# HydraRadio/hydra-pspec

Measured on NVIDIA B200. Metric: baseline-Gibbs-iterations/sec at Nfreq=384, Ntimes=1024, Nfg=32 on 1/8 B200, higher is better.
Workload: dtype f64 (complex128)

## Files before the change

### hydra_pspec_b200/_lib.py

```python
import ctypes as C
import os
from pathlib import Path

import numpy as np

_HERE = Path(__file__).resolve().parent
LIB_PATH = Path(os.environ.get("HP_LIB_PATH", _HERE / "csrc" / "libhydra_pspec_b200.so"))

HP_RNG_INJECTED, HP_RNG_PHILOX = 0, 1
HP_KEEP_CR, HP_KEEP_FG, HP_KEEP_CHISQ = 1, 2, 4
(HP_BUF_PS, HP_BUF_LNPOST, HP_BUF_CR, HP_BUF_FG, HP_BUF_CHISQ, HP_BUF_LAST_CR, HP_BUF_LAST_FG,
 HP_BUF_PS_CUR) = range(8)
HP_NUM_KERNEL_CLASSES = 6


class HPConfig(C.Structure):
    _fields_ = [
        ("device", C.c_int), ("nchains", C.c_int), ("ntimes", C.c_int), ("nfreqs", C.c_int),
        ("nmodes", C.c_int), ("rng_mode", C.c_int), ("cg_compat", C.c_int), ("refresh_omega", C.c_int),
        ("keep", C.c_int), ("max_iters", C.c_int), ("general_basis0", C.c_int), ("profile", C.c_int), ("substreams", C.c_int), ("dense_noise", C.c_int),
        ("force_dense_transforms", C.c_int), ("force_dense_solve", C.c_int), ("time_flags", C.c_int),
        ("ring_iters", C.c_int), ("seed", C.c_uint64), ("stream", C.c_void_p),
    ]


class HPHostSink(C.Structure):
    _fields_ = [("signal_ps", C.c_void_p), ("ln_post", C.c_void_p), ("signal_cr", C.c_void_p),
                ("fg_amps", C.c_void_p), ("chisq", C.c_void_p), ("iters", C.c_int), ("first_iter", C.c_int),
                ("iter_major", C.c_int), ("read_ahead", C.c_int)]


class HydraLibError(RuntimeError):
    pass


_lib = None

_dp = C.POINTER(C.c_double)
_SIGNATURES = {
    "hp_engine_create": (C.c_int, [C.POINTER(HPConfig), C.POINTER(C.c_void_p)]),
    "hp_engine_destroy": (C.c_int, [C.c_void_p]),
    "hp_engine_load_chain": (C.c_int, [C.c_void_p, C.c_int, C.c_void_p, C.c_void_p, C.c_void_p, C.c_void_p,
                                       C.c_void_p, C.c_void_p, C.c_void_p]),
    "hp_engine_load_chain_dense": (C.c_int, [C.c_void_p, C.c_int] + [C.c_void_p] * 9),
    "hp_engine_set_draws": (C.c_int, [C.c_void_p, C.c_int, C.c_void_p, C.c_void_p, C.c_void_p, C.c_int]),
    "hp_engine_run": (C.c_int, [C.c_void_p, C.c_int]),
    "hp_engine_run_to_host": (C.c_int, [C.c_void_p, C.c_int, C.POINTER(HPHostSink)]),
    "hp_engine_gcr": (C.c_int, [C.c_void_p]),
    "hp_engine_sync": (C.c_int, [C.c_void_p]),
    "hp_engine_iterations_done": (C.c_int, [C.c_void_p]),
    "hp_engine_rewind": (C.c_int, [C.c_void_p]),
    "hp_engine_read": (C.c_int, [C.c_void_p, C.c_int, C.c_int, C.c_int, C.c_int, C.c_void_p, C.c_size_t]),
    "hp_engine_read_signal_S": (C.c_int, [C.c_void_p, C.c_int, C.c_void_p]),
    "hp_engine_info": (C.c_int, [C.c_void_p, C.c_void_p]),
    "hp_engine_kernel_ms": (C.c_int, [C.c_void_p, C.c_void_p, C.c_void_p, C.c_int]),
    "hp_engine_set_substreams": (C.c_int, [C.c_void_p, C.c_int]),
    "hp_engine_set_chain_ids": (C.c_int, [C.c_void_p, C.c_void_p]),
    "hp_engine_set_profile": (C.c_int, [C.c_void_p, C.c_int]),
    "hp_engine_launch_count": (C.c_longlong, [C.c_void_p]),
    "hp_engine_pt_form": (C.c_int, [C.c_void_p, C.POINTER(C.c_int), C.POINTER(C.c_int)]),
    "hp_kernel_class_name": (C.c_char_p, [C.c_int]),
    "hp_sample_S": (C.c_int, [C.c_int, C.c_int, C.c_int, C.c_void_p, C.c_void_p, C.c_void_p, C.c_void_p]),
    "hp_fourier_operator": (C.c_int, [C.c_int, C.c_int, C.c_void_p]),
    "hp_eigh_batch": (C.c_int, [C.c_int, C.c_int, C.c_int, C.c_void_p, C.c_void_p, C.c_void_p, C.c_void_p]),
    "hp_test_zgemm": (C.c_int, [C.c_int, C.c_int, C.c_int, C.c_void_p, C.c_int, C.c_int, C.c_void_p, C.c_int,
                                C.c_int, C.c_void_p, C.c_void_p]),
    "hp_test_chol_solve": (C.c_int, [C.c_int, C.c_int, C.c_int, C.c_void_p, C.c_void_p, C.c_void_p, C.c_void_p,
                                     C.c_int, C.c_void_p, C.c_void_p, C.c_void_p]),
    "hp_test_solve2": (C.c_int, [C.c_int, C.c_int, C.c_int, C.c_int, C.c_void_p, C.c_void_p, C.c_void_p, C.c_void_p,
                                 C.c_int, C.c_int, C.c_int, C.c_void_p, C.c_void_p]),
    "hp_test_solve3_schedule": (C.c_int, [C.c_int, C.c_void_p, C.c_void_p, C.POINTER(C.c_int), C.POINTER(C.c_int)]),
    "hp_fp64_peak_tflops": (C.c_double, [C.c_int, C.c_double]),
    "hp_release_cached_memory": (None, []),
    "hp_pinned_alloc": (C.c_void_p, [C.c_size_t]),
    "hp_pinned_free": (None, [C.c_void_p]),
    "hp_last_error": (C.c_char_p, []),
    "hp_version": (C.c_char_p, []),
}
EXPORTED_SYMBOLS = tuple(_SIGNATURES)


def lib():
    global _lib
    if _lib is None:
        if not LIB_PATH.exists():
            raise HydraLibError(
                f"{LIB_PATH} not found: build it with hydra_pspec_b200/csrc/build.sh "
                "(hydra_pspec_b200 has no CPU fallback)")
        L = C.CDLL(os.fspath(LIB_PATH))
        for name, (res, args) in _SIGNATURES.items():
            fn = getattr(L, name)
            fn.restype = res
            fn.argtypes = args
        _lib = L
    return _lib


def check(rc):
    if rc != 0:
        raise HydraLibError(f"hydra_pspec_b200 error {rc}: {lib().hp_last_error().decode()}")


def ptr(a):
    if a is None:
        return None
    assert a.flags["C_CONTIGUOUS"]
    return a.ctypes.data_as(C.c_void_p)


def c128(a):
    return np.ascontiguousarray(a, dtype=np.complex128)


def f64(a):
    return np.ascontiguousarray(a, dtype=np.float64)


def pinned_empty(shape, dtype):
    dtype = np.dtype(dtype)
    nbytes = int(np.prod(shape)) * dtype.itemsize
    p = lib().hp_pinned_alloc(max(nbytes, 1))
    if not p:
        raise HydraLibError("cudaHostAlloc failed")
    buf = (C.c_char * max(nbytes, 1)).from_address(p)
    arr = np.frombuffer(buf, dtype=dtype, count=int(np.prod(shape))).reshape(shape)
    import weakref
    weakref.finalize(buf, lib().hp_pinned_free, p)
    return arr


def bind_to_device_numa(device, verbose=False):
    import os
    import subprocess
    if os.environ.get("HP_NO_NUMA_BIND") == "1":
        return None
    try:
        out = subprocess.run(["nvidia-smi", "--query-gpu=pci.bus_id", "--format=csv,noheader", "-i", str(int(device))],
                             capture_output=True, text=True, timeout=20).stdout.strip().splitlines()[0].strip().lower()
        dom, rest = out.split(":", 1)
        bus = f"{dom[-4:]}:{rest}"
        node = int(open(f"/sys/bus/pci/devices/{bus}/numa_node").read())
        if node < 0:
            return None
        cpus = set()
        for part in open(f"/sys/devices/system/node/node{node}/cpulist").read().strip().split(","):
            lo, _, hi = part.partition("-")
            cpus.update(range(int(lo), int(hi or lo) + 1))
        allowed = os.sched_getaffinity(0)
        use = cpus & allowed
        if verbose:
            import sys
            print(f"[numa] device {device} bus {bus} node {node}: {len(use)} of {len(allowed)} allowed CPUs on that node",
                  file=sys.stderr)
        if not use:
            return None
        os.sched_setaffinity(0, use)
        return node
    except Exception:
        return None
```

### hydra_pspec_b200/csrc/hp_diag.cuh

```cuda
#pragma once
#include "hp_kernels.cuh"
#include "hp_mma.cuh"

namespace hp {

__device__ __forceinline__ bool diag_chol_inverse8(double* Ar, double* Ai, double* Vr, double* Vi) {
    const int lane = threadIdx.x & 31;
    const int r = lane & 7;
    const bool act = lane < 8;
    bool bad = false;
    {
        double ar[8], ai[8];
#pragma unroll
        for (int c = 0; c < 8; ++c) { ar[c] = Ar[r * kLdBlk + c]; ai[c] = Ai[r * kLdBlk + c]; }
#pragma unroll
        for (int c = 0; c < 8; ++c) {
            const double piv = __shfl_sync(0xffffffffu, ar[c], c);
            if (!(piv > 0.0)) bad = true;
            const double inv = rsqrt(piv);
            double lr = ar[c] * inv, li = ai[c] * inv;
            if (r == c) { lr = piv * inv; li = 0.0; }
            if (r < c) { lr = 0.0; li = 0.0; }
            if (act) {
                Ar[r * kLdBlk + c] = lr; Ai[r * kLdBlk + c] = li;
                if (r == c) Vr[c * kLdBlk + c] = inv;
            }
#pragma unroll
            for (int c2 = c + 1; c2 < 8; ++c2) {
                const double yr = __shfl_sync(0xffffffffu, lr, c2), yi = __shfl_sync(0xffffffffu, li, c2);
                ar[c2] -= lr * yr + li * yi;
                ai[c2] -= li * yr - lr * yi;
            }
        }
    }
    __syncwarp();
    {
        double vr[8], vi[8];
#pragma unroll
        for (int q = 0; q < 8; ++q) {
            double sr = 0.0, si = 0.0;
#pragma unroll
            for (int p = 0; p < q; ++p) {
                const double lr = Ar[q * kLdBlk + p], li = Ai[q * kLdBlk + p];
                sr += lr * vr[p] - li * vi[p];
                si += lr * vi[p] + li * vr[p];
            }
            const double dinv = Vr[q * kLdBlk + q];
            vr[q] = r < q ? -sr * dinv : (r == q ? dinv : 0.0);
            vi[q] = r < q ? -si * dinv : 0.0;
        }
        __syncwarp();
        if (act) {
#pragma unroll
            for (int q = 0; q < 8; ++q) { Vr[q * kLdBlk + r] = vr[q]; Vi[q * kLdBlk + r] = vi[q]; }
        }
    }
    __syncwarp();
    return bad;
}

__device__ __forceinline__ bool diag_chol_inverse_block(double* Ar, double* Ai, double* Vr, double* Vi, int tid, int nthreads) {
    const int warp = tid >> 5, lane = tid & 31;
    const int g = lane >> 2, q = lane & 3;
    bool bad = false;
    auto sub = [](double* base, int R, int C) { return base + (8 * R) * kLdBlk + 8 * C; };
    for (int e = tid; e < kLBlkDoubles; e += nthreads) Vr[e] = 0.0;
    if (warp < 6) {
        const int R = warp < 3 ? 0 : (warp < 5 ? 1 : 2), C = warp < 3 ? warp + 1 : (warp < 5 ? warp - 1 : 3);
        for (int e = lane; e < 64; e += 32) { sub(Ar, R, C)[(e >> 3) * kLdBlk + (e & 7)] = 0.0; sub(Ai, R, C)[(e >> 3) * kLdBlk + (e & 7)] = 0.0; }
    }
    __syncthreads();
    for (int kk = 0; kk < 4; ++kk) {
        if (warp == 0) bad |= diag_chol_inverse8(sub(Ar, kk, kk), sub(Ai, kk, kk), sub(Vr, kk, kk), sub(Vi, kk, kk));
        if (kk == 3) break;
        __syncthreads();
        if (warp < 3 - kk) {
            const int R = kk + 1 + warp;
            double P[3][1][1][2], cr[1][1][2], ci[1][1][2];
            warp_zero3m<1, 1>(P);
            warp_zgemm3m<1, 1, false, false, true, true>(P, sub(Ar, R, kk), sub(Ai, R, kk), kLdBlk, sub(Vr, kk, kk), sub(Vi, kk, kk),
                                                         kLdBlk, 8);
            warp_zgemm3m_finish<1, 1, false, true>(P, cr, ci);
            __syncwarp();
            *reinterpret_cast<double2*>(sub(Ar, R, kk) + g * kLdBlk + 2 * q) = make_double2(cr[0][0][0], cr[0][0][1]);
            *reinterpret_cast<double2*>(sub(Ai, R, kk) + g * kLdBlk + 2 * q) = make_double2(ci[0][0][0], ci[0][0][1]);
        }
        __syncthreads();
        const int ntr = (3 - kk) * (4 - kk) / 2;
        if (warp < ntr) {
            int R = kk + 1, C = kk + 1, w = warp;
            while (w > R - (kk + 1)) { w -= R - kk; ++R; }
            C = kk + 1 + w;
            double P[3][1][1][2], cr[1][1][2], ci[1][1][2];
            warp_zero3m<1, 1>(P);
            warp_zgemm3m<1, 1, false, false, true, true>(P, sub(Ar, R, kk), sub(Ai, R, kk), kLdBlk, sub(Ar, C, kk), sub(Ai, C, kk),
                                                         kLdBlk, 8);
            warp_zgemm3m_finish<1, 1, false, true>(P, cr, ci);
            double2* dr = reinterpret_cast<double2*>(sub(Ar, R, C) + g * kLdBlk + 2 * q);
            double2* di = reinterpret_cast<double2*>(sub(Ai, R, C) + g * kLdBlk + 2 * q);
            double2 xr = *dr, xi = *di;
            xr.x -= cr[0][0][0]; xr.y -= cr[0][0][1]; xi.x -= ci[0][0][0]; xi.y -= ci[0][0][1];
            *dr = xr; *di = xi;
        }
        __syncthreads();
    }
    __syncthreads();
    for (int d = 1; d < 4; ++d) {
        if (warp < 4 - d) {
            const int C = warp, R = C + d;
            double P[3][1][1][2], cr[1][1][2], ci[1][1][2];
            warp_zero3m<1, 1>(P);
            warp_zgemm3m<1, 1, false, false, false, false>(P, sub(Ar, R, C), sub(Ai, R, C), kLdBlk, sub(Vr, C, C), sub(Vi, C, C),
                                                           kLdBlk, 8 * d);
            warp_zgemm3m_finish<1, 1, false, false>(P, cr, ci);
            *reinterpret_cast<double2*>(sub(Vr, R, C) + g * kLdBlk + 2 * q) = make_double2(cr[0][0][0], cr[0][0][1]);
            *reinterpret_cast<double2*>(sub(Vi, R, C) + g * kLdBlk + 2 * q) = make_double2(ci[0][0][0], ci[0][0][1]);
            __syncwarp();
            warp_zero3m<1, 1>(P);
            warp_zgemm3m<1, 1, false, false, false, false>(P, sub(Vr, R, R), sub(Vi, R, R), kLdBlk, sub(Vr, R, C), sub(Vi, R, C),
                                                           kLdBlk, 8);
            warp_zgemm3m_finish<1, 1, false, false>(P, cr, ci);
            __syncwarp();
            *reinterpret_cast<double2*>(sub(Vr, R, C) + g * kLdBlk + 2 * q) = make_double2(-cr[0][0][0], -cr[0][0][1]);
            *reinterpret_cast<double2*>(sub(Vi, R, C) + g * kLdBlk + 2 * q) = make_double2(-ci[0][0][0], -ci[0][0][1]);
        }
        __syncthreads();
    }
    return bad;
}

}
```

### hydra_pspec_b200/csrc/hp_engine.cu

```cuda
#include "../../include/hydra_pspec_b200.h"
#include "hp_kernels.cuh"
#include "hp_math.h"

#include <cmath>
#include <cstdio>
#include <cstdlib>
#include <cstring>
#include <mutex>
#include <string>
#include <vector>

namespace {

thread_local std::string g_err;

int fail(int code, const std::string& msg) {
    g_err = msg;
    return code;
}

#define CU_TRY(expr)                                                                              \
    do {                                                                                          \
        cudaError_t _e = (expr);                                                                  \
        if (_e != cudaSuccess)                                                                    \
// ... 78 lines not shown
    double* y = Y + 2 * (sys * (size_t)Tp * Np + (size_t)e);
    y[0] += n0 * 0.70710678118654752440; y[1] += n1 * 0.70710678118654752440;
}
__global__ void k_make_ssc(double* Ssc, const double* X, const double* lam, int n, int Np, int T, int Tp) {
    const size_t sys = blockIdx.y;
    long long e = blockIdx.x * (long long)blockDim.x + threadIdx.x;
    if (e >= (long long)T * n) return;
    const int t = (int)(e / n), k = (int)(e % n);
    const double l = lam[sys * Np + k];
    const double* x = X + 2 * ((sys * (size_t)Tp + t) * Np + k);
    double* o = Ssc + 2 * ((sys * (size_t)Tp + t) * n + k);
    o[0] = l * x[0]; o[1] = l * x[1];
}
__global__ void k_sqrt_vec(double* out, const double* in, int n) {
    int k = blockIdx.x * blockDim.x + threadIdx.x;
    if (k < n) out[k] = sqrt(in[k]);
}

__global__ void k_basis_fourier(double* Bmat, const double* U, int n, int Np) {
    long long e = blockIdx.x * (long long)blockDim.x + threadIdx.x;
    if (e >= (long long)n * n) return;
    int x = (int)(e / n), k = (int)(e % n);
    Bmat[2 * ((size_t)x * Np + k)] = U[2 * ((size_t)k * n + x)];
    Bmat[2 * ((size_t)x * Np + k) + 1] = -U[2 * ((size_t)k * n + x) + 1];
}
__global__ void k_basis_general(double* Bmat, const double* Q, int n, int Np) {
    long long e = blockIdx.x * (long long)blockDim.x + threadIdx.x;
    if (e >= (long long)n * n) return;
    int x = (int)(e / n), k = (int)(e % n);
    Bmat[2 * ((size_t)x * Np + k)] = Q[2 * e];
    Bmat[2 * ((size_t)x * Np + k) + 1] = Q[2 * e + 1];
}
__global__ void k_basis_fg(double* Bmat, double* Ft, const double* F, int n, int m, int Np) {
    long long e = blockIdx.x * (long long)blockDim.x + threadIdx.x;
    if (e >= (long long)n * m) return;
    int x = (int)(e / m), j = (int)(e % m);
    double fr = F[2 * e], fi = F[2 * e + 1];
    Bmat[2 * ((size_t)x * Np + n + j)] = fr;
    Bmat[2 * ((size_t)x * Np + n + j) + 1] = fi;
    if (Ft) { Ft[2 * ((size_t)j * n + x)] = fr; Ft[2 * ((size_t)j * n + x) + 1] = fi; }
}
__global__ void k_noise_vectors(const double* w, const double* ninv, double* ni, double* nu, int n) {
    int x = blockIdx.x * blockDim.x + threadIdx.x;
    if (x >= n) return;
    double v = w[x] * ninv[x];
    ni[x] = v;
    nu[x] = sqrt(v);
}
__global__ void k_init_lam(double* lam, double* ps, const double* lamsq, int n, int N, int Np) {
    int k = blockIdx.x * blockDim.x + threadIdx.x;
    if (k >= Np) return;
    if (k < n) { lam[k] = sqrt(lamsq[k]); if (ps) ps[k] = (double)n * lamsq[k]; }
    else lam[k] = k < N ? 1.0 : 0.0;
}
__global__ void k_scale_vec(double* out, const double* in, double s, int n) {
    int k = blockIdx.x * blockDim.x + threadIdx.x;
    if (k < n) out[k] = in[k] * s;
}

__global__ void k_mask_dense(double* NiD, const double* Ninv, const double* w, int n) {
    long long e = blockIdx.x * (long long)blockDim.x + threadIdx.x;
    if (e >= (long long)n * n) return;
    int x = (int)(e / n), y = (int)(e % n);
    double s = w[x] * w[y];
    NiD[2 * e] = s * Ninv[2 * e];
    NiD[2 * e + 1] = s * Ninv[2 * e + 1];
}
__global__ void k_lower_half(double* NiL, const double* NiD, int n) {
    long long e = blockIdx.x * (long long)blockDim.x + threadIdx.x;
    if (e >= (long long)n * n) return;
    int x = (int)(e / n), y = (int)(e % n);
    double re = 0.0, im = 0.0;
    if (y < x) {
        const long long f = (long long)y * n + x;
        re = 0.5 * (NiD[2 * e] + NiD[2 * f]);
        im = 0.5 * (NiD[2 * e + 1] - NiD[2 * f + 1]);
    } else if (y == x) {
        re = 0.5 * NiD[2 * e];
    }
    NiL[2 * e] = re; NiL[2 * e + 1] = im;
}
__global__ void k_rowdot(const double* A, const double* B, double* out, int T, int Tp, int n, double scale) {
    const int sys = blockIdx.y, t = blockIdx.x;
    const double* a = A + 2 * (((size_t)sys * Tp + t) * n);
    const double* b = B + 2 * (((size_t)sys * Tp + t) * n);
    double acc = 0.0;
    if (t < T)
        for (int x = threadIdx.x; x < n; x += blockDim.x) acc += a[2 * x] * b[2 * x] + a[2 * x + 1] * b[2 * x + 1];
    __shared__ double red[8];
    for (int o = 16; o > 0; o >>= 1) acc += __shfl_down_sync(0xffffffffu, acc, o);
    if ((threadIdx.x & 31) == 0) red[threadIdx.x >> 5] = acc;
    __syncthreads();
    if (threadIdx.x == 0) {
        double s2 = 0.0;
        for (int i = 0; i < (int)(blockDim.x >> 5); ++i) s2 += red[i];
        out[(size_t)sys * Tp + t] = scale * s2;
    }
}

inline unsigned nblocks(long long tot, int bs = 256) { return (unsigned)((tot + bs - 1) / bs); }

struct Basis {
    double* Bmat = nullptr;
    double* Gp = nullptr;
    double* Rfix = nullptr;
    double* wa = nullptr;
    double* Rt = nullptr;
};

enum { CLS_CHOL = 0, CLS_SOLVE = 1, CLS_TRANSFORM = 2, CLS_POST = 3, CLS_SAMPLE = 4, CLS_LOWRANK = 5 };

}

struct hp_engine {
    hp_config cfg;
    int C, T, n, m, N, nblk, Np, Tp, ntiles;
    cudaStream_t st = nullptr;
    cudaStream_t copy_st = nullptr;
    std::vector<cudaStream_t> sub_st;
    cudaEvent_t fork_ev = nullptr;
    int active_subs = 1 << 30;
    std::vector<cudaEvent_t> join_ev;
    bool own_stream = false;
    double *Fop = nullptr, *U = nullptr;
    Basis bF, b0;
    double *lam = nullptr, *ps = nullptr;
    double *wd = nullptr, *w = nullptr, *ninvd = nullptr, *ni = nullptr, *nu = nullptr, *Ft = nullptr, *prior = nullptr;
    double *Lp = nullptr, *Linvp = nullptr, *Wp = nullptr;
    double *wT = nullptr, *Hpt = nullptr, *niT = nullptr, *Bsel = nullptr, *ptScratch = nullptr;
    int* ptSame = nullptr;
    int pt_ctas = 0;
    bool pt_low = false;
    int Tp0 = 0;
    int pt_kcap = 0;
    double* Pm = nullptr;
    uint16_t* ptFidx = nullptr;
    int* ptFcnt = nullptr;
    std::vector<int> pt_kmax;
    std::vector<uint8_t> hpt_built;
    std::vector<uint8_t> pt_loaded;
    int gd_slots = 1;
    std::vector<uint8_t> pending;
    bool big_solve = false;
    bool solve2 = false;
    bool solve3 = false;
    double *Wf1 = nullptr, *Wf2 = nullptr;
    hp::Solve3Sched sched3{};
    int pp_tiles = 0;
    double* Wp1 = nullptr;
    double *Wd = nullptr, *Yb = nullptr;
    double *NiL = nullptr;
    double *NiD = nullptr, *NihD = nullptr, *Td = nullptr, *Rm = nullptr, *Yd = nullptr;
    int* info = nullptr;
    int* chain_ids = nullptr;
    double *X = nullptr, *Ssc = nullptr, *Ppart = nullptr, *Sf = nullptr, *Wm = nullptr, *Tmp = nullptr;
    double *Em = nullptr, *Eu = nullptr, *lnp1 = nullptr;
    double* sdraws = nullptr;
    double *ps_out = nullptr, *lnpost_out = nullptr, *cr_out = nullptr, *fg_out = nullptr, *chisq_out = nullptr;
    double *Gd = nullptr, *stage = nullptr, *vecn = nullptr;
    void* arena = nullptr;
    size_t arena_bytes = 0;
    hp::FftPlan plan{};
    hp::FftPlan plan2f{}, plan2r{};
    bool fft2_ok = false;
    bool fft_ok = false;
    int ntilesE = 0, ktp = 8;
    double *tw = nullptr, *tw2 = nullptr, *Empart = nullptr, *Eupart = nullptr;
    std::vector<uint8_t> flagged;
    std::vector<uint8_t> have_omega;
    bool any_flagged = false;
    int ring = 1;
    std::vector<cudaEvent_t> copy_done;
    std::vector<cudaEvent_t> sub_done;
    int iter = 0;
    int out_pos = 0;
    int ahead = 0;
    std::vector<cudaEvent_t> it_done;
    uint32_t draw_counter = 0;
    const double* last_sf = nullptr;
    long long last_sf_bs = 0;
    long long launches = 0;
    std::vector<cudaEvent_t> ev;
    std::vector<int> ev_cls;
    double ms_acc[HP_NUM_KERNEL_CLASSES] = {0};
    int launch_acc[HP_NUM_KERNEL_CLASSES] = {0};

    void prof_begin(int cls, cudaStream_t s) {
        if (!cfg.profile || ev_cls.size() >= 8192) return;
        cudaEvent_t a, b;
        cudaEventCreate(&a); cudaEventCreate(&b);
        cudaEventRecord(a, s);
        ev.push_back(a); ev.push_back(b); ev_cls.push_back(cls);
    }
    void prof_end(int cls, int nlaunch, cudaStream_t s) {
        launches += nlaunch;
        launch_acc[cls] += nlaunch;
        if (!cfg.profile || ev_cls.empty() || ev_cls.back() != cls) return;
        cudaEventRecord(ev.back(), s);
    }
};

namespace {
constexpr int kMaxDevices = 64;
struct CachedArena { void* p = nullptr; size_t bytes = 0; };
CachedArena g_arena_cache[kMaxDevices];
std::mutex g_arena_mutex;
bool arena_cache_enabled() {
    static int on = -1;
    if (on < 0) { const char* e = getenv("HP_NO_ARENA_CACHE"); on = (e && e[0] == '1') ? 0 : 1; }
    return on == 1;
}
cudaError_t arena_acquire(void** base, size_t* bytes, int device) {
    if (arena_cache_enabled() && device >= 0 && device < kMaxDevices) {
        std::lock_guard<std::mutex> lk(g_arena_mutex);
        CachedArena& c = g_arena_cache[device];
        if (c.p && c.bytes >= *bytes) { *base = c.p; *bytes = c.bytes; c.p = nullptr; c.bytes = 0; return cudaSuccess; }
        if (c.p) { cudaFree(c.p); c.p = nullptr; c.bytes = 0; }
    }
    return cudaMalloc(base, *bytes);
}
void arena_release(void* p, size_t bytes, int device) {
    if (!p) return;
    if (arena_cache_enabled() && device >= 0 && device < kMaxDevices) {
        std::lock_guard<std::mutex> lk(g_arena_mutex);
        CachedArena& c = g_arena_cache[device];
        if (!c.p || c.bytes < bytes) {
            if (c.p) cudaFree(c.p);
            c.p = p; c.bytes = bytes;
            return;
        }
    }
    cudaFree(p);
}

struct ArenaPlan {
    struct Req { void** p; size_t bytes; };
    std::vector<Req> reqs;
    template <typename T>
    void want(T** p, size_t count) { *p = nullptr; if (count) reqs.push_back({reinterpret_cast<void**>(p), count * sizeof(T)}); }
    cudaError_t commit(void** base, size_t* bytes_out, int device, cudaStream_t st) {
        size_t total = 0;
        for (auto& r : reqs) total += (r.bytes + 255) & ~size_t(255);
        if (!total) total = 256;
        *bytes_out = total;
        cudaError_t e = arena_acquire(base, bytes_out, device);
        if (e != cudaSuccess) return e;
        e = cudaMemsetAsync(*base, 0, total, st);
        if (e != cudaSuccess) return e;
        size_t off = 0;
        for (auto& r : reqs) { *r.p = static_cast<char*>(*base) + off; off += (r.bytes + 255) & ~size_t(255); }
        return cudaSuccess;
    }
};

void want_basis(hp_engine* e, ArenaPlan& ap, Basis& b) {
    size_t C = e->C;
    ap.want(&b.Bmat, 2 * C * e->n * e->Np);
    ap.want(&b.Gp, C * hp::tri_blocks(e->nblk) * hp::kBlkDoubles);
    ap.want(&b.Rfix, 2 * C * e->Tp * e->Np);
    if (e->cfg.rng_mode == HP_RNG_INJECTED) ap.want(&b.wa, 2 * C * e->Tp * e->Np);
    if (e->solve2 || e->solve3) ap.want(&b.Rt, 2 * C * e->Tp * e->Np);
}
}

static const char* kAheadMsg = "read-ahead iterations are pending (hp_host_sink.read_ahead): deliver them with hp_engine_run_to_host or "
                               "drop them with hp_engine_rewind first";

extern "C" {

const char* hp_last_error(void) { return g_err.c_str(); }
const char* hp_version(void) { return "hydra_pspec_b200 0.1 (sm_100a)"; }
void hp_release_cached_memory(void) {
    std::lock_guard<std::mutex> lk(g_arena_mutex);
    int cur = 0;
    cudaGetDevice(&cur);
    for (int d = 0; d < kMaxDevices; ++d)
        if (g_arena_cache[d].p) {
            cudaSetDevice(d);
            cudaFree(g_arena_cache[d].p);
            g_arena_cache[d] = CachedArena();
        }
    cudaSetDevice(cur);
}
const char* hp_kernel_class_name(int cls) {
    static const char* names[HP_NUM_KERNEL_CLASSES] = {"chol", "solve", "transform", "post", "sample", "lowrank"};
    return (cls >= 0 && cls < HP_NUM_KERNEL_CLASSES) ? names[cls] : "?";
}

int hp_engine_destroy(hp_engine* e) {
    if (!e) return HP_OK;
    cudaSetDevice(e->cfg.device);
    if (e->st) cudaStreamSynchronize(e->st);
    for (auto& x : e->ev) cudaEventDestroy(x);
    arena_release(e->arena, e->arena_bytes, e->cfg.device);
    if (e->copy_st) cudaStreamDestroy(e->copy_st);
    for (auto x : e->sub_st) cudaStreamDestroy(x);
    if (e->fork_ev) cudaEventDestroy(e->fork_ev);
    for (auto x : e->join_ev) cudaEventDestroy(x);
    for (auto x : e->copy_done) cudaEventDestroy(x);
    for (auto x : e->it_done) cudaEventDestroy(x);
    for (auto x : e->sub_done) cudaEventDestroy(x);
    if (e->own_stream) cudaStreamDestroy(e->st);
    delete e;
    return HP_OK;
}

int hp_engine_create(const hp_config* cfg, hp_engine** out) {
    if (!cfg || !out) return fail(HP_ERR_ARG, "null argument");
    if (cfg->nchains < 1 || cfg->ntimes < 2 || cfg->nfreqs < 2 || cfg->nmodes < 0 || cfg->max_iters < 1)
        return fail(HP_ERR_ARG, "hp_engine_create: bad dimensions");
    int ndev = 0;
    if (cudaGetDeviceCount(&ndev) != cudaSuccess || ndev == 0)
        return fail(HP_ERR_CUDA, "no CUDA device: hydra_pspec_b200 has no CPU fallback");
    CU_TRY(cudaSetDevice(cfg->device));
    hp_engine* e = new hp_engine();
    e->cfg = *cfg;
    e->C = cfg->nchains; e->T = cfg->ntimes; e->n = cfg->nfreqs; e->m = cfg->nmodes;
    e->N = e->n + e->m;
    e->nblk = (e->N + hp::kNB - 1) / hp::kNB;
    e->Np = e->nblk * hp::kNB;
    e->ntiles = (e->T + hp::kTT - 1) / hp::kTT;
    e->Tp = e->ntiles * hp::kTT;
    e->Tp0 = e->Tp;
    int max_smem = 0;
    cudaDeviceGetAttribute(&max_smem, cudaDevAttrMaxSharedMemoryPerBlockOptin, cfg->device);
    e->big_solve = cfg->force_dense_solve || !hp::solve_resident_ok(e->nblk, (size_t)max_smem);
    {
        const char* kv = getenv("HP_SOLVE_KERNEL");
        const int want = kv ? atoi(kv) : 3;
        const bool resident = !e->big_solve && !cfg->time_flags;
        e->solve3 = resident && want >= 3 && hp::solve3_ok(e->nblk, (size_t)max_smem);
        const char* pd = getenv("HP_PT_DIRECT");
        if (cfg->time_flags && !(pd && pd[0] == '1') && !cfg->force_dense_solve && hp::solve3_ok(e->nblk, (size_t)max_smem) &&
            e->n < 65536) {
            e->pt_low = true;
            e->solve3 = true;
            e->Tp0 = e->Tp;
            e->Tp += hp::kTT * ((e->n + hp::kTT - 1) / hp::kTT);
            e->ntiles = e->Tp / hp::kTT;
        }
        e->solve2 = resident && !e->solve3 && want >= 2 && hp::solve2_stages(e->nblk, (size_t)max_smem) >= 2;
        if (e->solve3) hp::solve3_make_schedule(e->nblk, &e->sched3, (e->N + 15) / 16);
    }
    if (cfg->time_flags && (cfg->dense_noise || cfg->cg_compat || cfg->force_dense_transforms || (cfg->general_basis0 && !e->pt_low))) {
        delete e;
        return fail(HP_ERR_ARG, "per-time flags need diagonal noise, the exact solver and an FFT-able Nfreqs (and a delay-diagonal "
                                "S_initial unless Nfreqs + Nmodes <= 448)");
    }
    if (cfg->time_flags && (hp::pt_smem_bytes(e->nblk, e->n) > (size_t)max_smem || !hp::make_fft_plan(e->n, &e->plan) ||
                            hp::postfft_ktp(e->n, e->m, (size_t)max_smem) == 0)) {
        delete e;
        return fail(HP_ERR_SIZE, "per-time flags: Nfreqs too large for the shared-memory working set, or without an FFT plan");
    }
    if (cfg->stream) e->st = (cudaStream_t)cfg->stream;
    else { CU_TRY(cudaStreamCreateWithFlags(&e->st, cudaStreamNonBlocking)); e->own_stream = true; }
    const size_t C = e->C, n = e->n, m = e->m, Np = e->Np, Tp = e->Tp, T = e->T, I = cfg->max_iters;
    e->ring = (cfg->ring_iters > 0 && cfg->ring_iters < cfg->max_iters) ? cfg->ring_iters : cfg->max_iters;
    const size_t R = e->ring;
    e->ktp = hp::postfft_ktp(e->n, e->m, (size_t)max_smem);
    e->fft_ok = hp::make_fft_plan(e->n, &e->plan) && e->ktp > 0 &&
                !cfg->force_dense_transforms;
    {
        const char* v1 = getenv("HP_POST_FFT_V1");
        e->fft2_ok = e->fft_ok && !(v1 && v1[0] == '1') && hp::make_fft2_plan(e->n, &e->plan2f, &e->plan2r) &&
                     hp::postfft2_smem_bytes(e->n, e->m) <= (size_t)max_smem / (e->n >= 512 ? 1 : 2);
        if (e->fft2_ok) e->ktp = 8;
    }
    e->ntilesE = hp::postfft_tiles(e->T, e->ktp > 0 ? e->ktp : 8);
    const bool dense = !e->fft_ok;
    const bool need_ssc = dense || cfg->general_basis0;
    ArenaPlan ap;
    ap.want(&e->Fop, 2 * n * n); ap.want(&e->U, 2 * n * n);
    want_basis(e, ap, e->bF);
    if (cfg->general_basis0) want_basis(e, ap, e->b0);
    ap.want(&e->lam, C * Np); ap.want(&e->ps, C * n);
    ap.want(&e->wd, 2 * C * Tp * n); ap.want(&e->w, C * n); ap.want(&e->ninvd, C * n);
    ap.want(&e->ni, C * n); ap.want(&e->nu, C * n); ap.want(&e->Ft, 2 * C * (m ? m : 1) * n);
    ap.want(&e->prior, C * 2 * n);
    ap.want(&e->Lp, C * hp::tri_blocks(e->nblk) * hp::kLBlkDoubles);
    ap.want(&e->Linvp, C * e->nblk * hp::kLBlkDoubles);
    ap.want(&e->Wp, C * hp::tri_blocks(e->nblk) * hp::kLBlkDoubles);
    if (e->solve2 && cfg->rng_mode == HP_RNG_PHILOX) ap.want(&e->Wp1, C * hp::tri_blocks(e->nblk) * hp::kLBlkDoubles);
    if (e->solve3) { ap.want(&e->Wf1, C * hp::solve3_frag_doubles(e->nblk)); ap.want(&e->Wf2, C * hp::solve3_frag_doubles(e->nblk)); }
    ap.want(&e->info, C);
    ap.want(&e->chain_ids, C);
    ap.want(&e->X, 2 * C * Tp * Np);
    if (need_ssc) ap.want(&e->Ssc, 2 * C * Tp * n);
    e->pp_tiles = (e->solve2 ? 2 : 1) * e->ntiles;
    ap.want(&e->Ppart, C * e->pp_tiles * n); ap.want(&e->Sf, 2 * C * Tp * n);
    if (dense) { ap.want(&e->Wm, 2 * C * Tp * n); ap.want(&e->Tmp, 2 * C * Tp * n); ap.want(&e->Em, C * n); ap.want(&e->Eu, C * n); }
    ap.want(&e->lnp1, C * Tp);
    if (e->big_solve && !cfg->time_flags) { ap.want(&e->Wd, 2 * C * Np * Np); ap.want(&e->Yb, 2 * C * Tp * Np); }
    if (cfg->time_flags) {
        e->pt_ctas = hp::pt_grid(e->C, e->T);
        ap.want(&e->wT, C * Tp * n);
        ap.want(&e->ptSame, C * Tp);
        ap.want(&e->Hpt, 2 * C * Tp * (1 + m) * Np);
        ap.want(&e->niT, Tp * n);
        ap.want(&e->Bsel, 2 * n * (1 + m));
        ap.want(&e->ptScratch, (size_t)e->pt_ctas * hp::pt_scratch_doubles_per_cta(e->nblk));
        if (e->pt_low) {
            ap.want(&e->Pm, 2 * C * n * n);
            ap.want(&e->ptFidx, C * T * hp::kPtLowMaxRank);
            ap.want(&e->ptFcnt, C * T);
        }
    }
    if (cfg->dense_noise) {
        ap.want(&e->NiD, 2 * C * n * n);
        ap.want(&e->NiL, 2 * C * n * n);
        if (cfg->rng_mode == HP_RNG_INJECTED) ap.want(&e->NihD, 2 * C * n * n);
        ap.want(&e->Td, 2 * n * Np); ap.want(&e->Rm, 2 * C * Tp * n); ap.want(&e->Yd, 2 * C * Tp * n);
    }
    if (cfg->rng_mode != HP_RNG_PHILOX) ap.want(&e->sdraws, C * I * n);
    ap.want(&e->ps_out, C * I * n); ap.want(&e->lnpost_out, C * I);
    if (cfg->keep & HP_KEEP_CR) ap.want(&e->cr_out, 2 * C * R * T * n);
    if (cfg->keep & HP_KEEP_FG) ap.want(&e->fg_out, 2 * C * R * T * (m ? m : 1));
    if (cfg->keep & HP_KEEP_CHISQ) ap.want(&e->chisq_out, C * R * T * n);
    e->gd_slots = (int)(C < 16 ? C : 16);
    ap.want(&e->Gd, 2 * (size_t)e->gd_slots * e->N * e->N);
    ap.want(&e->stage, 2 * (T * n > n * n ? T * n : n * n));
    ap.want(&e->vecn, 4 * n);
    ap.want(&e->tw, 2 * n);
    if (e->fft2_ok) ap.want(&e->tw2, 4 * n);
    ap.want(&e->Empart, C * e->ntilesE * n); ap.want(&e->Eupart, C * e->ntilesE * n);
    {
        cudaError_t ce = ap.commit(&e->arena, &e->arena_bytes, cfg->device, e->st);
        if (ce != cudaSuccess) {
            std::string msg = std::string("device allocation failed: ") + cudaGetErrorString(ce);
            hp_engine_destroy(e);
            return fail(HP_ERR_CUDA, msg);
        }
    }
    e->flagged.assign(C, 0);
    e->pt_kmax.assign(C, 0);
    e->hpt_built.assign(C, 0);
    e->pt_loaded.assign(C, 0);
    e->pending.assign(C, 0);
    e->have_omega.assign(C, 0);
    {
        int ns = cfg->substreams > 1 ? (cfg->substreams < (int)C ? cfg->substreams : (int)C) : 1;
        if (ns > 1) {
            for (int i = 0; i < ns; ++i) {
                cudaStream_t x; cudaEvent_t ev;
                cudaStreamCreateWithFlags(&x, cudaStreamNonBlocking); e->sub_st.push_back(x);
                cudaEventCreateWithFlags(&ev, cudaEventDisableTiming); e->join_ev.push_back(ev);
            }
            cudaEventCreateWithFlags(&e->fork_ev, cudaEventDisableTiming);
        }
    }
    {
        std::vector<int> ids(C);
        for (size_t c = 0; c < C; ++c) ids[c] = (int)c;
        cudaMemcpyAsync(e->chain_ids, ids.data(), C * sizeof(int), cudaMemcpyHostToDevice, e->st);
    }
    hp::launch_fourier_operator(e->Fop, e->n, 1.0, e->st);
    hp::launch_fourier_operator(e->U, e->n, 1.0 / std::sqrt((double)e->n), e->st);
    hp::launch_twiddles(e->tw, e->n, e->st);
    if (e->tw2 && !hp::launch_fft2_tables(e->tw2, e->tw, e->n, e->st)) e->tw2 = nullptr;
    if (cudaStreamSynchronize(e->st) != cudaSuccess || cudaGetLastError() != cudaSuccess) {
        hp_engine_destroy(e);
        return fail(HP_ERR_CUDA, "engine initialisation kernels failed");
    }
    *out = e;
    return HP_OK;
}

static int build_hpt(hp_engine* e, int c) {
    const int n = e->n, m = e->m, N = e->N, Np = e->Np, T = e->T;
    const double* Bm = e->bF.Bmat + 2 * (size_t)c * n * Np;
    k_rowscale<<<nblocks((long long)T * n), 256, 0, e->st>>>(e->niT, e->wT + (size_t)c * e->Tp * n, e->ninvd + (size_t)c * n, T, n);
    k_select_cols<<<nblocks((long long)n * (1 + m)), 256, 0, e->st>>>(e->Bsel, Bm, n, m, Np);
    hp::ZgemmArgs h{};
    h.A = Bm; h.sAi = 1; h.sAk = Np; h.bsA = 0; h.conjA = 1;
    h.B = e->Bsel; h.sBk = 1 + m; h.sBj = 1; h.bsB = 0;
    h.C = e->Hpt + 2 * (size_t)c * e->Tp * (1 + m) * Np; h.sCi = 1; h.sCj = Np; h.bsC = (long long)(1 + m) * Np;
    h.dk = e->niT; h.bsD = n;
    h.M = N; h.N = 1 + m; h.K = n; h.accumulate = 0; h.alpha = 1.0; h.batch = T;
    hp::launch_zgemm(h, e->st);
    CU_TRY(cudaGetLastError());
    e->hpt_built[c] = 1;
    return HP_OK;
}

static int build_basis_products(hp_engine* e, Basis& b, int c) {
    const int n = e->n, N = e->N, Np = e->Np, T = e->T;
    double* Bm = b.Bmat + 2 * (size_t)c * n * Np;
    const bool dn = e->cfg.dense_noise != 0;
    const double* NiD = dn ? e->NiD + 2 * (size_t)c * n * n : nullptr;
    hp::ZgemmArgs g{};
    g.A = Bm; g.sAi = 1; g.sAk = Np; g.bsA = 0; g.conjA = 1;
    g.C = e->Gd; g.sCi = N; g.sCj = 1; g.bsC = 0;
    g.M = N; g.N = N; g.K = n; g.accumulate = 0; g.alpha = 1.0; g.batch = 1;
    if (dn) {
        hp::ZgemmArgs t1{};
        t1.A = NiD; t1.sAi = n; t1.sAk = 1;
        t1.B = Bm; t1.sBk = Np; t1.sBj = 1;
        t1.C = e->Td; t1.sCi = Np; t1.sCj = 1;
        t1.M = n; t1.N = N; t1.K = n; t1.alpha = 1.0; t1.batch = 1;
        hp::launch_zgemm(t1, e->st);
        g.B = e->Td; g.sBk = Np; g.sBj = 1;
    } else {
        g.B = Bm; g.sBk = Np; g.sBj = 1; g.bsB = 0; g.conjB = 0;
        g.dk = e->ni + (size_t)c * n; g.bsD = 0;
    }
    hp::launch_zgemm(g, e->st);
    hp::launch_pack_lower(e->Gd, N, 0, b.Gp + (size_t)c * hp::tri_blocks(e->nblk) * hp::kBlkDoubles, N, e->nblk, 1, e->st);
    hp::ZgemmArgs r{};
    r.B = Bm; r.sBk = Np; r.sBj = 1; r.conjB = 1;
    r.C = b.Rfix + 2 * (size_t)c * e->Tp * Np; r.sCi = Np; r.sCj = 1;
    r.M = T; r.N = N; r.K = n; r.accumulate = 0; r.alpha = 1.0; r.batch = 1;
    if (dn) {
        hp::ZgemmArgs y{};
        y.A = e->wd + 2 * (size_t)c * e->Tp * n; y.sAi = n; y.sAk = 1;
        y.B = NiD; y.sBk = 1; y.sBj = n;
        y.C = e->Yd + 2 * (size_t)c * e->Tp * n; y.sCi = n; y.sCj = 1;
        y.M = T; y.N = n; y.K = n; y.alpha = 1.0; y.batch = 1;
        hp::launch_zgemm(y, e->st);
        r.A = e->Yd + 2 * (size_t)c * e->Tp * n; r.sAi = n; r.sAk = 1;
    } else {
        r.A = e->wd + 2 * (size_t)c * e->Tp * n; r.sAi = n; r.sAk = 1; r.conjA = 0;
        r.dk = e->cfg.time_flags ? e->ninvd + (size_t)c * n : e->ni + (size_t)c * n;
    }
    hp::launch_zgemm(r, e->st);
    if (e->ptFidx) hp::launch_pt_arows(b.Rfix + 2 * (size_t)c * e->Tp * Np, Bm, e->ni + (size_t)c * n, n, Np, e->Tp0, e->st);
    if (b.Rt && e->cfg.rng_mode == HP_RNG_PHILOX)
        hp::launch_rhs_tile(b.Rt + 2 * (size_t)c * e->Tp * Np, b.Rfix + 2 * (size_t)c * e->Tp * Np, nullptr, nullptr, e->nblk, e->n, e->N,
                            e->ptFidx ? e->Tp : e->T, e->Tp, e->ntiles, 1, e->st);
    if (e->cfg.time_flags && &b == &e->bF) {
        e->hpt_built[c] = 0;
        if (!e->pt_low) { const int rc = build_hpt(e, c); if (rc != HP_OK) return rc; }
    }
    CU_TRY(cudaGetLastError());
    return HP_OK;
}

static int build_basis_products_batch(hp_engine* e, Basis& b, int c0, int nc) {
    const int n = e->n, N = e->N, Np = e->Np, T = e->T;
    const size_t tri = hp::tri_blocks(e->nblk);
    for (int cc0 = c0; cc0 < c0 + nc; cc0 += e->gd_slots) {
        const int ncc = (c0 + nc - cc0) < e->gd_slots ? (c0 + nc - cc0) : e->gd_slots;
        double* Bm = b.Bmat + 2 * (size_t)cc0 * n * Np;
        hp::ZgemmArgs g{};
        g.A = Bm; g.sAi = 1; g.sAk = Np; g.bsA = (long long)n * Np; g.conjA = 1;
        g.B = Bm; g.sBk = Np; g.sBj = 1; g.bsB = (long long)n * Np;
        g.dk = e->ni + (size_t)cc0 * n; g.bsD = n;
        g.C = e->Gd; g.sCi = N; g.sCj = 1; g.bsC = (long long)N * N;
        g.M = N; g.N = N; g.K = n; g.accumulate = 0; g.alpha = 1.0; g.batch = ncc;
        hp::launch_zgemm(g, e->st);
        hp::launch_pack_lower(e->Gd, N, (long long)N * N, b.Gp + (size_t)cc0 * tri * hp::kBlkDoubles, N, e->nblk, ncc, e->st);
        hp::ZgemmArgs r{};
        r.A = e->wd + 2 * (size_t)cc0 * e->Tp * n; r.sAi = n; r.sAk = 1; r.bsA = (long long)e->Tp * n;
        r.dk = e->ni + (size_t)cc0 * n; r.bsD = n;
        r.B = Bm; r.sBk = Np; r.sBj = 1; r.bsB = (long long)n * Np; r.conjB = 1;
        r.C = b.Rfix + 2 * (size_t)cc0 * e->Tp * Np; r.sCi = Np; r.sCj = 1; r.bsC = (long long)e->Tp * Np;
        r.M = T; r.N = N; r.K = n; r.accumulate = 0; r.alpha = 1.0; r.batch = ncc;
        hp::launch_zgemm(r, e->st);
        if (b.Rt && e->cfg.rng_mode == HP_RNG_PHILOX)
            hp::launch_rhs_tile(b.Rt + 2 * (size_t)cc0 * e->Tp * Np, b.Rfix + 2 * (size_t)cc0 * e->Tp * Np, nullptr, nullptr, e->nblk,
                                e->n, e->N, e->T, e->Tp, e->ntiles, ncc, e->st);
    }
    CU_TRY(cudaGetLastError());
    return HP_OK;
}

static int flush_pending(hp_engine* e) {
    const int C = e->C;
    if (e->cfg.time_flags && !e->pt_low)
        for (int c = 0; c < C; ++c)
            if (e->pt_loaded[c] && !e->hpt_built[c]) { const int rc = build_hpt(e, c); if (rc != HP_OK) return rc; }
    for (int c = 0; c < C;) {
        if (!e->pending[c]) { ++c; continue; }
        int c1 = c;
        while (c1 < C && e->pending[c1]) ++c1;
        int rc;
        if ((rc = build_basis_products_batch(e, e->bF, c, c1 - c)) != HP_OK) return rc;
        if (e->cfg.general_basis0 && (rc = build_basis_products_batch(e, e->b0, c, c1 - c)) != HP_OK) return rc;
        for (int k = c; k < c1; ++k) e->pending[k] = 0;
// ... 105 lines not shown
    }
    CU_TRY(cudaMemcpyAsync(e->vecn, lam0sq, n * sizeof(double), cudaMemcpyHostToDevice, st));
    k_init_lam<<<nblocks(Np), 256, 0, st>>>(e->lam + (size_t)c * Np, e->ps + (size_t)c * n, e->vecn, n, N, Np);
    CU_TRY(cudaStreamSynchronize(st));
    CU_TRY(cudaGetLastError());
    e->iter = 0;
    e->out_pos = 0;
    e->draw_counter = 0;
    return HP_OK;
}

int hp_engine_load_chain(hp_engine* e, int c, const double* vis, const uint8_t* flags, const double* fgmodes,
                         const double* ninv_diag, const double* basis0, const double* lam0sq, const double* ps_prior) {
    return load_chain_impl(e, c, vis, flags, fgmodes, ninv_diag, nullptr, nullptr, basis0, lam0sq, ps_prior);
}

int hp_engine_load_chain_dense(hp_engine* e, int c, const double* vis, const uint8_t* flags, const double* fgmodes,
                               const double* ninv_diag, const double* ninv_dense, const double* nih_dense,
                               const double* basis0, const double* lam0sq, const double* ps_prior) {
    if (!ninv_dense) return fail(HP_ERR_ARG, "hp_engine_load_chain_dense: ninv_dense is NULL");
    return load_chain_impl(e, c, vis, flags, fgmodes, ninv_diag, ninv_dense, nih_dense, basis0, lam0sq, ps_prior);
}

int hp_engine_set_draws(hp_engine* e, int c, const double* omega_a, const double* omega_b, const double* s_draws,
                        int n_draw_iters) {
    if (!e) return fail(HP_ERR_ARG, "null engine");
    if (e->cfg.rng_mode != HP_RNG_INJECTED) return fail(HP_ERR_ARG, "hp_engine_set_draws: engine is not in injected-draw mode");
    if (e->ahead > 0) return fail(HP_ERR_ARG, kAheadMsg);
    if (c < 0 || c >= e->C) return fail(HP_ERR_ARG, "chain index out of range");
    if ((omega_a == nullptr) != (omega_b == nullptr)) return fail(HP_ERR_ARG, "omega_a and omega_b must both be given or both NULL");
    if (n_draw_iters > e->cfg.max_iters) return fail(HP_ERR_ARG, "more draw iterations than max_iters");
    CU_TRY(cudaSetDevice(e->cfg.device));
    { int rcf = flush_pending(e); if (rcf != HP_OK) return rcf; }
    const int n = e->n, Np = e->Np, T = e->T, Tp = e->Tp;
    cudaStream_t st = e->st;
    if (s_draws && n_draw_iters > 0)
        CU_TRY(cudaMemcpyAsync(e->sdraws + (size_t)c * e->cfg.max_iters * n, s_draws, (size_t)n_draw_iters * n * sizeof(double),
                               cudaMemcpyHostToDevice, st));
    if (omega_a) {
        for (int which = 0; which < (e->cfg.general_basis0 ? 2 : 1); ++which) {
            Basis& b = which ? e->b0 : e->bF;
            double* Bm = b.Bmat + 2 * (size_t)c * n * Np;
            CU_TRY(cudaMemcpyAsync(e->stage, omega_b, 2 * (size_t)T * n * sizeof(double), cudaMemcpyHostToDevice, st));
            hp::ZgemmArgs r{};
            r.A = e->stage; r.sAi = n; r.sAk = 1;
            r.B = Bm; r.sBk = Np; r.sBj = 1; r.conjB = 1;
            r.C = b.Rfix + 2 * (size_t)c * Tp * Np; r.sCi = Np; r.sCj = 1;
            if (e->cfg.dense_noise) {
                hp::ZgemmArgs y{};
                y.A = e->stage; y.sAi = n; y.sAk = 1;
                y.B = e->NihD + 2 * (size_t)c * n * n; y.sBk = 1; y.sBj = n;
                y.C = e->Yd + 2 * (size_t)c * Tp * n; y.sCi = n; y.sCj = 1;
                y.M = T; y.N = n; y.K = n; y.alpha = 1.0; y.batch = 1;
                hp::launch_zgemm(y, st);
                r.A = e->Yd + 2 * (size_t)c * Tp * n;
            } else if (e->cfg.time_flags) {
                k_mask_elem<<<nblocks((long long)T * n), 256, 0, st>>>(e->stage, e->wT + (size_t)c * Tp * n, (long long)T * n);
                k_sqrt_vec<<<nblocks(n), 256, 0, st>>>(e->vecn, e->ninvd + (size_t)c * n, n);
                r.dk = e->vecn;
            } else {
                r.dk = e->nu + (size_t)c * n;
            }
            r.M = T; r.N = e->N; r.K = n; r.accumulate = 1; r.alpha = 1.0; r.batch = 1;
            hp::launch_zgemm(r, st);
            CU_TRY(cudaStreamSynchronize(st));
            CU_TRY(cudaMemcpyAsync(e->stage, omega_a, 2 * (size_t)T * n * sizeof(double), cudaMemcpyHostToDevice, st));
            hp::ZgemmArgs a{};
            a.A = e->stage; a.sAi = n; a.sAk = 1;
            a.B = Bm; a.sBk = Np; a.sBj = 1; a.conjB = 1;
            a.C = b.wa + 2 * (size_t)c * Tp * Np; a.sCi = Np; a.sCj = 1;
            a.M = T; a.N = n; a.K = n; a.accumulate = 0; a.alpha = 1.0; a.batch = 1;
            hp::launch_zgemm(a, st);
            CU_TRY(cudaStreamSynchronize(st));
        }
        e->have_omega[c] = 1;
    }
    CU_TRY(cudaStreamSynchronize(st));
    CU_TRY(cudaGetLastError());
    return HP_OK;
}

static cudaError_t copy_rows_d2h(void* dst, size_t dpitch, const void* src, size_t spitch, size_t width, size_t rows,
                                 cudaStream_t st) {
    if (rows == 0 || width == 0) return cudaSuccess;
    if (dpitch < (size_t)0x7fffffff && spitch < (size_t)0x7fffffff)
        return cudaMemcpy2DAsync(dst, dpitch, src, spitch, width, rows, cudaMemcpyDeviceToHost, st);
    cudaError_t e = cudaSuccess;
    for (size_t r = 0; r < rows && e == cudaSuccess; ++r)
        e = cudaMemcpyAsync((char*)dst + r * dpitch, (const char*)src + r * spitch, width, cudaMemcpyDeviceToHost, st);
    return e;
}

struct IterOut {
    double* sf; long long sf_bs;
    double* fg; long long fg_bs;
    double* chisq; long long chisq_bs;
};

struct Sub { int c0, nc; cudaStream_t st; };
#define OFFS(ptr, per_chain) ((ptr) ? (ptr) + (size_t)sb.c0 * (size_t)(per_chain) : nullptr)

static void enqueue_dense_lnp1(hp_engine* e, const Sub& sb) {
    const size_t n = e->n, Tp = e->Tp;
    e->prof_begin(CLS_TRANSFORM, sb.st);
    hp::ZgemmArgs y{};
    y.A = OFFS(e->Rm, 2 * Tp * n); y.sAi = e->n; y.sAk = 1; y.bsA = (long long)e->Tp * e->n;
    y.B = OFFS(e->NiL, 2 * n * n); y.sBk = e->n; y.sBj = 1; y.conjB = 1; y.bsB = (long long)e->n * e->n;
    y.C = OFFS(e->Yd, 2 * Tp * n); y.sCi = e->n; y.sCj = 1; y.bsC = (long long)e->Tp * e->n;
    y.M = e->T; y.N = e->n; y.K = e->n; y.alpha = 1.0; y.batch = sb.nc;
    y.tri = 2;
    hp::launch_zgemm(y, sb.st);
    k_rowdot<<<dim3(e->Tp, sb.nc), 128, 0, sb.st>>>(OFFS(e->Rm, 2 * Tp * n), OFFS(e->Yd, 2 * Tp * n), OFFS(e->lnp1, Tp), e->T,
                                                   e->Tp, e->n, 2.0);
    e->prof_end(CLS_TRANSFORM, 2, sb.st);
}

static void enqueue_gcr(hp_engine* e, Basis& b, const IterOut& o, const Sub& sb, uint32_t draw_iter) {
    const bool philox = e->cfg.rng_mode == HP_RNG_PHILOX;
    const bool general = &b == &e->b0;
    const size_t n = e->n, m = e->m, Np = e->Np, Tp = e->Tp;
    const size_t tri = hp::tri_blocks(e->nblk);
    const bool fused_inverse = e->fft_ok && !general;
    const bool pt = e->cfg.time_flags != 0;
    bool any_omega = false;
    for (auto h : e->have_omega) any_omega |= (h != 0);
    const bool pt_low = pt && e->pt_low;
    if (pt && !pt_low) {
        const int nsub = e->C > 0 ? (e->C + sb.nc - 1) / sb.nc : 1;
        int grid = e->pt_ctas / (nsub > 0 ? nsub : 1);
        if (grid < 1) grid = 1;
        const int slot0 = (int)(((long long)sb.c0 * e->pt_ctas) / e->C);
        if (slot0 + grid > e->pt_ctas) grid = e->pt_ctas - slot0;
        e->prof_begin(CLS_SOLVE, sb.st);
        cudaMemsetAsync(e->info + sb.c0, 0, sizeof(int) * sb.nc, sb.st);
        hp::PtArgs pa{};
        pa.H = OFFS(e->Hpt, 2 * Tp * (1 + m) * Np); pa.lam = OFFS(e->lam, Np); pa.Rfix = OFFS(b.Rfix, 2 * Tp * Np);
        pa.wa = (!philox && any_omega) ? OFFS(b.wa, 2 * Tp * Np) : nullptr;
        pa.X = OFFS(e->X, 2 * Tp * Np);
        pa.same_prev = OFFS(e->ptSame, Tp);
        pa.scratch = e->ptScratch + (size_t)slot0 * hp::pt_scratch_doubles_per_cta(e->nblk);
        pa.info = e->info + sb.c0;
        pa.nblk = e->nblk; pa.n = e->n; pa.m = e->m; pa.N = e->N; pa.T = e->T; pa.Tp = e->Tp; pa.nsys = sb.nc;
        pa.philox_wa = philox ? 1 : 0;
        pa.key0 = (uint32_t)e->cfg.seed; pa.key1 = (uint32_t)(e->cfg.seed >> 32); pa.iter = draw_iter;
        pa.chain_ids = OFFS(e->chain_ids, 1); pa.chain0 = sb.c0;
        hp::launch_pt_cholsolve(pa, grid, sb.st);
        hp::launch_colsumsq(OFFS(e->X, 2 * Tp * Np), OFFS(e->Ppart, (size_t)e->pp_tiles * n), e->T, e->Tp, e->n, sb.nc, sb.st, e->Np);
        e->prof_end(CLS_SOLVE, 2, sb.st);
    } else {
    e->prof_begin(CLS_CHOL, sb.st);
    hp::CholArgs ca{};
    ca.Gp = OFFS(b.Gp, tri * hp::kBlkDoubles); ca.lam = OFFS(e->lam, Np); ca.Lp = OFFS(e->Lp, tri * hp::kLBlkDoubles);
    ca.Linvp = OFFS(e->Linvp, (size_t)e->nblk * hp::kLBlkDoubles); ca.info = e->info + sb.c0;
    ca.nblk = e->nblk; ca.n = e->n; ca.N = e->N; ca.nsys = sb.nc;
    const hp::TrinvExtra ex{OFFS(e->Wp1, tri * hp::kLBlkDoubles), OFFS(e->Wf1, hp::solve3_frag_doubles(e->nblk)),
                            OFFS(e->Wf2, hp::solve3_frag_doubles(e->nblk)), philox ? OFFS(e->lam, Np) : nullptr};
    const int nchol = hp::launch_chol_trinv(ca, OFFS(e->Wp, tri * hp::kLBlkDoubles), ex, sb.st);
    e->prof_end(CLS_CHOL, nchol, sb.st);

    if (e->big_solve) {
        e->prof_begin(CLS_SOLVE, sb.st);
        const long long NN = (long long)e->Np * e->Np, TN = (long long)e->Tp * e->Np;
        double* Wd = OFFS(e->Wd, 2 * Np * Np);
        double* Yb = OFFS(e->Yb, 2 * Tp * Np);
        double* X = OFFS(e->X, 2 * Tp * Np);
        k_unpack_lower<<<dim3(nblocks(NN), sb.nc), 256, 0, sb.st>>>(OFFS(e->Wp, tri * hp::kLBlkDoubles), Wd, e->nblk,
                                                                   tri * hp::kLBlkDoubles);
        k_build_rhs<<<dim3(nblocks(TN), sb.nc), 256, 0, sb.st>>>(X, OFFS(b.Rfix, 2 * Tp * Np),
                                                                (!philox && any_omega) ? OFFS(b.wa, 2 * Tp * Np) : nullptr,
                                                                OFFS(e->lam, Np), e->n, e->Np, e->T, e->Tp);
        hp::ZgemmArgs y{};
        y.A = X; y.sAi = e->Np; y.sAk = 1; y.bsA = TN;
        y.B = Wd; y.sBk = 1; y.sBj = e->Np; y.bsB = NN;
        y.C = Yb; y.sCi = e->Np; y.sCj = 1; y.bsC = TN;
        y.M = e->T; y.N = e->Np; y.K = e->Np; y.alpha = 1.0; y.batch = sb.nc;
        y.tri = 1;
        hp::launch_zgemm(y, sb.st);
        int nl = 4;
        if (philox) {
            k_add_noise<<<dim3(nblocks((long long)e->T * e->Np), sb.nc), 256, 0, sb.st>>>(
                Yb, e->N, e->Np, e->T, e->Tp, (uint32_t)e->cfg.seed, (uint32_t)(e->cfg.seed >> 32), draw_iter, OFFS(e->chain_ids, 1));
            ++nl;
        }
        hp::ZgemmArgs x{};
        x.A = Yb; x.sAi = e->Np; x.sAk = 1; x.bsA = TN;
        x.B = Wd; x.sBk = e->Np; x.sBj = 1; x.bsB = NN; x.conjB = 1;
        x.C = X; x.sCi = e->Np; x.sCj = 1; x.bsC = TN;
        x.M = e->T; x.N = e->Np; x.K = e->Np; x.alpha = 1.0; x.batch = sb.nc;
        x.tri = 2;
        hp::launch_zgemm(x, sb.st);
        if (e->cfg.cg_compat) {
            hp::launch_cg_scale(X, OFFS(b.Rfix, 2 * Tp * Np), (!philox && any_omega) ? OFFS(b.wa, 2 * Tp * Np) : nullptr, OFFS(e->lam, Np),
                                e->n, e->N, e->Np, e->T, e->Tp, sb.nc, sb.st);
            ++nl;
        }
        hp::launch_colsumsq(X, OFFS(e->Ppart, (size_t)e->pp_tiles * n), e->T, e->Tp, e->n, sb.nc, sb.st, e->Np);
        ++nl;
        if (!fused_inverse) {
            k_make_ssc<<<dim3(nblocks((long long)e->T * e->n), sb.nc), 256, 0, sb.st>>>(OFFS(e->Ssc, 2 * Tp * n), X, OFFS(e->lam, Np),
                                                                                       e->n, e->Np, e->T, e->Tp);
            ++nl;
        }
        e->prof_end(CLS_SOLVE, nl, sb.st);
    } else if (e->solve3) {
        e->prof_begin(CLS_SOLVE, sb.st);
        int nl = 1;
        const double* wa_sb = (!philox && any_omega) ? OFFS(b.wa, 2 * Tp * Np) : nullptr;
        if (!philox) {
            hp::launch_rhs_tile(OFFS(b.Rt, 2 * Tp * Np), OFFS(b.Rfix, 2 * Tp * Np), wa_sb, OFFS(e->lam, Np), e->nblk, e->n, e->N,
                                pt_low ? e->Tp : e->T, e->Tp, e->ntiles, sb.nc, sb.st);
            ++nl;
        }
        hp::Solve3Args sa{};
        sa.Wf1 = OFFS(e->Wf1, hp::solve3_frag_doubles(e->nblk)); sa.Wf2 = OFFS(e->Wf2, hp::solve3_frag_doubles(e->nblk));
        sa.Rt = OFFS(b.Rt, 2 * Tp * Np);
        sa.X = OFFS(e->X, 2 * Tp * Np);
        sa.Ppart = OFFS(e->Ppart, (size_t)e->pp_tiles * n);
        sa.nblk = e->nblk; sa.n = e->n; sa.N = e->N; sa.Tp = e->Tp; sa.ntiles = e->ntiles; sa.nsys = sb.nc; sa.T = e->T;
        sa.philox = philox ? 1 : 0;
        sa.key0 = (uint32_t)e->cfg.seed; sa.key1 = (uint32_t)(e->cfg.seed >> 32); sa.iter = draw_iter;
        sa.chain_ids = OFFS(e->chain_ids, 1); sa.chain0 = sb.c0;
        sa.sched = e->sched3; sa.nstrip = (e->N + 15) / 16;
        hp::launch_solve3(sa, sb.st);
        if (pt_low) {
            e->prof_end(CLS_SOLVE, nl, sb.st);
            nl = 0;
            e->prof_begin(CLS_LOWRANK, sb.st);
            hp::ZgemmArgs pz{};
            pz.A = OFFS(b.Rfix, 2 * Tp * Np) + 2 * (size_t)e->Tp0 * Np; pz.sAi = e->Np; pz.sAk = 1; pz.bsA = (long long)e->Tp * e->Np;
            pz.conjA = 1; pz.dk = OFFS(e->lam, Np); pz.bsD = e->Np;
            pz.B = sa.X + 2 * (size_t)e->Tp0 * Np; pz.sBk = 1; pz.sBj = e->Np; pz.bsB = (long long)e->Tp * e->Np;
            pz.C = OFFS(e->Pm, 2 * n * n); pz.sCi = e->n; pz.sCj = 1; pz.bsC = (long long)e->n * e->n;
            pz.M = e->n; pz.N = e->n; pz.K = e->N; pz.alpha = 1.0; pz.batch = sb.nc;
            pz.lower_out = 1;
            hp::launch_zgemm(pz, sb.st);
            hp::PtLowArgs la{};
            la.Rfix = OFFS(b.Rfix, 2 * Tp * Np); la.wa = wa_sb; la.lam = OFFS(e->lam, Np); la.X = sa.X; la.Pm = OFFS(e->Pm, 2 * n * n);
            la.fidx = e->ptFidx + (size_t)sb.c0 * e->T * hp::kPtLowMaxRank; la.fcnt = e->ptFcnt + (size_t)sb.c0 * e->T;
            la.info = e->info + sb.c0;
            la.n = e->n; la.N = e->N; la.Np = e->Np; la.T = e->T; la.Tp = e->Tp; la.Tp0 = e->Tp0; la.nsys = sb.nc; la.nblk = e->nblk;
            la.kcap = e->pt_kcap; la.philox = philox ? 1 : 0;
            la.key0 = (uint32_t)e->cfg.seed; la.key1 = (uint32_t)(e->cfg.seed >> 32); la.iter = draw_iter;
            la.chain_ids = OFFS(e->chain_ids, 1); la.chain0 = sb.c0;
            hp::launch_pt_lowrank(la, sb.st);
            hp::launch_colsumsq(sa.X, OFFS(e->Ppart, (size_t)e->pp_tiles * n), e->T, e->Tp, e->n, sb.nc, sb.st, e->Np);
            e->prof_end(CLS_LOWRANK, 3, sb.st);
            e->prof_begin(CLS_SOLVE, sb.st);
        }
        if (e->cfg.cg_compat) {
            hp::launch_cg_scale(sa.X, OFFS(b.Rfix, 2 * Tp * Np), wa_sb, OFFS(e->lam, Np), e->n, e->N, e->Np, e->T, e->Tp, sb.nc, sb.st);
            hp::launch_colsumsq(sa.X, OFFS(e->Ppart, (size_t)e->pp_tiles * n), e->T, e->Tp, e->n, sb.nc, sb.st, e->Np);
            nl += 2;
        }
        if (!fused_inverse) {
            k_make_ssc<<<dim3(nblocks((long long)e->T * e->n), sb.nc), 256, 0, sb.st>>>(OFFS(e->Ssc, 2 * Tp * n), sa.X, OFFS(e->lam, Np),
                                                                                       e->n, e->Np, e->T, e->Tp);
            ++nl;
        }
        e->prof_end(CLS_SOLVE, nl, sb.st);
    } else if (e->solve2) {
        e->prof_begin(CLS_SOLVE, sb.st);
        int nl = 1;
        const double* wa_sb = (!philox && any_omega) ? OFFS(b.wa, 2 * Tp * Np) : nullptr;
        if (!philox) {
            hp::launch_rhs_tile(OFFS(b.Rt, 2 * Tp * Np), OFFS(b.Rfix, 2 * Tp * Np), wa_sb, OFFS(e->lam, Np), e->nblk, e->n, e->N, e->T,
                                e->Tp, e->ntiles, sb.nc, sb.st);
            ++nl;
        }
        hp::Solve2Args sa{};
        sa.W1 = philox ? OFFS(e->Wp1, tri * hp::kLBlkDoubles) : OFFS(e->Wp, tri * hp::kLBlkDoubles);
        sa.W2 = OFFS(e->Wp, tri * hp::kLBlkDoubles);
        sa.Rt = OFFS(b.Rt, 2 * Tp * Np);
        sa.X = OFFS(e->X, 2 * Tp * Np);
        sa.Ppart = OFFS(e->Ppart, (size_t)e->pp_tiles * n);
        sa.nblk = e->nblk; sa.n = e->n; sa.N = e->N; sa.Tp = e->Tp; sa.ntiles = e->ntiles; sa.nsys = sb.nc; sa.T = e->T;
        sa.philox = philox ? 1 : 0;
        sa.key0 = (uint32_t)e->cfg.seed; sa.key1 = (uint32_t)(e->cfg.seed >> 32); sa.iter = draw_iter;
        sa.chain_ids = OFFS(e->chain_ids, 1); sa.chain0 = sb.c0;
        hp::launch_solve2(sa, sb.st);
        if (e->cfg.cg_compat) {
            hp::launch_cg_scale(sa.X, OFFS(b.Rfix, 2 * Tp * Np), wa_sb, OFFS(e->lam, Np), e->n, e->N, e->Np, e->T, e->Tp, sb.nc, sb.st);
            hp::launch_colsumsq(sa.X, OFFS(e->Ppart, (size_t)e->pp_tiles * n), e->T, e->Tp, e->n, sb.nc, sb.st, e->Np);
            nl += 2;
        }
        if (!fused_inverse) {
            k_make_ssc<<<dim3(nblocks((long long)e->T * e->n), sb.nc), 256, 0, sb.st>>>(OFFS(e->Ssc, 2 * Tp * n), sa.X, OFFS(e->lam, Np),
                                                                                       e->n, e->Np, e->T, e->Tp);
            ++nl;
        }
        e->prof_end(CLS_SOLVE, nl, sb.st);
    } else {
    e->prof_begin(CLS_SOLVE, sb.st);
    hp::SolveArgs sa{};
    sa.Wp = OFFS(e->Wp, tri * hp::kLBlkDoubles); sa.lam = OFFS(e->lam, Np);
    sa.Rfix = OFFS(b.Rfix, 2 * Tp * Np);
    sa.wa = (!philox && any_omega) ? OFFS(b.wa, 2 * Tp * Np) : nullptr;
    sa.X = OFFS(e->X, 2 * Tp * Np); sa.Ssc = fused_inverse ? nullptr : OFFS(e->Ssc, 2 * Tp * n);
    sa.Ppart = OFFS(e->Ppart, (size_t)e->pp_tiles * n);
    sa.nblk = e->nblk; sa.n = e->n; sa.N = e->N; sa.Tp = e->Tp; sa.ntiles = e->ntiles; sa.nsys = sb.nc; sa.T = e->T;
    sa.philox_wa = philox ? 1 : 0;
    sa.cg_compat = e->cfg.cg_compat;
    sa.key0 = (uint32_t)e->cfg.seed; sa.key1 = (uint32_t)(e->cfg.seed >> 32); sa.iter = draw_iter;
    sa.chain_ids = OFFS(e->chain_ids, 1); sa.chain0 = sb.c0;
    hp::launch_solve(sa, sb.st);
    e->prof_end(CLS_SOLVE, 1, sb.st);
    }
// ... 246 lines not shown
                                     e->copy_st);
        }
        cudaEventRecord(e->copy_done[slot], e->copy_st);
    }
    if (big && cerr == cudaSuccess && sink->read_ahead > 0) {
        int want = sink->read_ahead < (int)R - 1 ? sink->read_ahead : (int)R - 1;
        while (e->ahead < want && e->out_pos + e->ahead < e->cfg.max_iters) {
            compute_next((size_t)(e->out_pos + e->ahead));
            ++e->ahead;
        }
    }
    join_subs(e, subs);
    if (cerr != cudaSuccess) return fail(HP_ERR_CUDA, std::string("hp_engine_run_to_host: ") + cudaGetErrorString(cerr));
    {
        cudaEvent_t ev;
        CU_TRY(cudaEventCreateWithFlags(&ev, cudaEventDisableTiming));
        CU_TRY(cudaEventRecord(ev, e->st));
        CU_TRY(cudaStreamWaitEvent(e->copy_st, ev, 0));
        cudaEventDestroy(ev);
    }
    if (niter > 0) {
        const size_t h0 = (size_t)(first - sink->first_iter);
        if (sink->signal_ps)
            CU_TRY(copy_rows_d2h(sink->signal_ps + h0 * n, HI * n * 8, e->ps_out + first * n, I * n * 8, (size_t)niter * n * 8, C,
                                 e->copy_st));
        if (sink->ln_post)
            CU_TRY(copy_rows_d2h(sink->ln_post + h0, HI * 8, e->lnpost_out + first, I * 8, (size_t)niter * 8, C, e->copy_st));
    }
    CU_TRY(cudaStreamSynchronize(e->copy_st));
    CU_TRY(cudaStreamSynchronize(e->st));
    CU_TRY(cudaGetLastError());
    return HP_OK;
}

int hp_engine_set_chain_ids(hp_engine* e, const int* ids) {
    if (!e || !ids) return fail(HP_ERR_ARG, "null argument");
    CU_TRY(cudaSetDevice(e->cfg.device));
    CU_TRY(cudaMemcpyAsync(e->chain_ids, ids, (size_t)e->C * sizeof(int), cudaMemcpyHostToDevice, e->st));
    CU_TRY(cudaStreamSynchronize(e->st));
    return HP_OK;
}

int hp_engine_set_substreams(hp_engine* e, int n) {
    if (!e) return fail(HP_ERR_ARG, "null engine");
    if (e->ahead > 0) return fail(HP_ERR_ARG, kAheadMsg);
    e->active_subs = n < 1 ? 1 : n;
    return HP_OK;
}

int hp_engine_set_profile(hp_engine* e, int on) {
    if (!e) return fail(HP_ERR_ARG, "null engine");
    e->cfg.profile = on ? 1 : 0;
    return HP_OK;
}

int hp_engine_sync(hp_engine* e) {
    if (!e) return fail(HP_ERR_ARG, "null engine");
    CU_TRY(cudaSetDevice(e->cfg.device));
    CU_TRY(cudaStreamSynchronize(e->st));
    CU_TRY(cudaGetLastError());
    return HP_OK;
}
int hp_engine_iterations_done(const hp_engine* e) { return e ? e->iter : -1; }
int hp_engine_rewind(hp_engine* e) {
    if (!e) return fail(HP_ERR_ARG, "null engine");
    e->out_pos = 0;
    e->ahead = 0;
    return HP_OK;
}
long long hp_engine_launch_count(const hp_engine* e) { return e ? e->launches : -1; }
int hp_engine_pt_form(const hp_engine* e, int* low_rank, int* max_rank) {
    if (!e) return fail(HP_ERR_ARG, "null engine");
    if (low_rank) *low_rank = (e->cfg.time_flags && e->pt_low) ? 1 : 0;
    if (max_rank) *max_rank = e->pt_kcap;
    return HP_OK;
}

int hp_engine_read(hp_engine* e, int c, int buffer, int iter0, int niter, void* dst, size_t dst_bytes) {
    if (!e || !dst) return fail(HP_ERR_ARG, "null argument");
    if (c < 0 || c >= e->C) return fail(HP_ERR_ARG, "chain index out of range");
    CU_TRY(cudaSetDevice(e->cfg.device));
    CU_TRY(cudaStreamSynchronize(e->st));
    const size_t n = e->n, m = e->m, T = e->T, Tp = e->Tp, Np = e->Np, I = e->cfg.max_iters;
    const bool per_iter = buffer <= HP_BUF_CHISQ;
    if (per_iter && (iter0 < 0 || niter < 0 || (size_t)(iter0 + niter) > I)) return fail(HP_ERR_ARG, "iteration range out of bounds");
    const double* src = nullptr;
    size_t bytes = 0;
    switch (buffer) {
        case HP_BUF_PS: src = e->ps_out + ((size_t)c * I + iter0) * n; bytes = (size_t)niter * n * 8; break;
        case HP_BUF_LNPOST: src = e->lnpost_out + (size_t)c * I + iter0; bytes = (size_t)niter * 8; break;
        case HP_BUF_CR:
        case HP_BUF_FG:
        case HP_BUF_CHISQ: {
            const double* base = buffer == HP_BUF_CR ? e->cr_out : (buffer == HP_BUF_FG ? e->fg_out : e->chisq_out);
            if (!base) return fail(HP_ERR_ARG, "this output was not kept (cfg.keep)");
            const size_t R = e->ring;
            const size_t per = buffer == HP_BUF_CR ? 2 * T * n : (buffer == HP_BUF_FG ? 2 * T * m : T * n);
            bytes = (size_t)niter * per * 8;
            if (dst_bytes < bytes) return fail(HP_ERR_ARG, "destination too small");
            if (niter > 0 && (size_t)iter0 + R < (size_t)(e->out_pos + e->ahead))
                return fail(HP_ERR_ARG, "iteration no longer in the device ring (cfg.ring_iters): stream it with hp_engine_run_to_host");
            for (int k = 0; k < niter; ++k) {
                const size_t slot = (size_t)(iter0 + k) % R;
                if (per) CU_TRY(cudaMemcpy((char*)dst + (size_t)k * per * 8, base + (slot * (size_t)e->C + (size_t)c) * per, per * 8, cudaMemcpyDeviceToHost));
            }
            return HP_OK;
        }
        case HP_BUF_LAST_CR:
            if (e->ahead > 0) return fail(HP_ERR_ARG, kAheadMsg);
            if (!e->last_sf) return fail(HP_ERR_ARG, "no GCR solve has run yet");
            src = e->last_sf + 2 * (size_t)c * e->last_sf_bs; bytes = T * n * 16; break;
        case HP_BUF_PS_CUR:
            if (e->ahead > 0) return fail(HP_ERR_ARG, kAheadMsg);
            src = e->ps + (size_t)c * n; bytes = n * 8; break;
        case HP_BUF_LAST_FG: {
            if (e->ahead > 0) return fail(HP_ERR_ARG, kAheadMsg);
            bytes = T * m * 16;
            if (dst_bytes < bytes) return fail(HP_ERR_ARG, "destination too small");
            if (m == 0) return HP_OK;
            CU_TRY(cudaMemcpy2D(dst, m * 16, e->X + 2 * ((size_t)c * Tp * Np + n), Np * 16, m * 16, T, cudaMemcpyDeviceToHost));
            return HP_OK;
        }
        default: return fail(HP_ERR_ARG, "unknown buffer id");
    }
    if (dst_bytes < bytes) return fail(HP_ERR_ARG, "destination too small");
    if (bytes) CU_TRY(cudaMemcpy(dst, src, bytes, cudaMemcpyDeviceToHost));
    return HP_OK;
}

int hp_engine_read_signal_S(hp_engine* e, int c, double* dst) {
    if (!e || !dst) return fail(HP_ERR_ARG, "null argument");
    if (c < 0 || c >= e->C) return fail(HP_ERR_ARG, "chain index out of range");
    if (e->ahead > 0) return fail(HP_ERR_ARG, kAheadMsg);
    CU_TRY(cudaSetDevice(e->cfg.device));
    const int n = e->n;
    k_scale_vec<<<nblocks(n), 256, 0, e->st>>>(e->vecn + n, e->ps + (size_t)c * n, 1.0 / ((double)n * n), n);
    hp::ZgemmArgs g{};
    g.A = e->Fop; g.sAi = 1; g.sAk = n; g.conjA = 1;
    g.B = e->Fop; g.sBk = n; g.sBj = 1;
    g.C = e->stage; g.sCi = n; g.sCj = 1;
    g.dk = e->vecn + n;
    g.M = n; g.N = n; g.K = n; g.alpha = 1.0; g.batch = 1;
    hp::launch_zgemm(g, e->st);
    CU_TRY(cudaStreamSynchronize(e->st));
    CU_TRY(cudaMemcpy(dst, e->stage, 2 * (size_t)n * n * sizeof(double), cudaMemcpyDeviceToHost));
    return HP_OK;
}

int hp_engine_info(hp_engine* e, int* info_host) {
    if (!e || !info_host) return fail(HP_ERR_ARG, "null argument");
    CU_TRY(cudaSetDevice(e->cfg.device));
    CU_TRY(cudaStreamSynchronize(e->st));
    CU_TRY(cudaMemcpy(info_host, e->info, e->C * sizeof(int), cudaMemcpyDeviceToHost));
    return HP_OK;
}

int hp_engine_kernel_ms(hp_engine* e, double* ms, int* launches, int reset) {
    if (!e) return fail(HP_ERR_ARG, "null engine");
    CU_TRY(cudaSetDevice(e->cfg.device));
    CU_TRY(cudaStreamSynchronize(e->st));
    for (size_t i = 0; i < e->ev_cls.size(); ++i) {
        float t = 0.f;
        if (cudaEventElapsedTime(&t, e->ev[2 * i], e->ev[2 * i + 1]) == cudaSuccess) e->ms_acc[e->ev_cls[i]] += t;
        cudaEventDestroy(e->ev[2 * i]); cudaEventDestroy(e->ev[2 * i + 1]);
    }
    e->ev.clear(); e->ev_cls.clear();
    for (int i = 0; i < HP_NUM_KERNEL_CLASSES; ++i) {
        if (ms) ms[i] = e->ms_acc[i];
        if (launches) launches[i] = e->launch_acc[i];
        if (reset) { e->ms_acc[i] = 0; e->launch_acc[i] = 0; }
    }
    return HP_OK;
}

int hp_sample_S(int device, int T, int n, const double* s, const double* prior, const double* draws, double* out) {
    if (!s || !draws || !out || T < 2 || n < 1) return fail(HP_ERR_ARG, "hp_sample_S: bad argument");
    int ndev = 0;
    if (cudaGetDeviceCount(&ndev) != cudaSuccess || ndev == 0) return fail(HP_ERR_CUDA, "no CUDA device: hydra_pspec_b200 has no CPU fallback");
    CU_TRY(cudaSetDevice(device));
    double *U, *S, *Sk, *Eu, *pr, *dr, *ps, *lam, *lnp1, *psout, *lnp;
    CU_TRY(dalloc(&U, 2 * (size_t)n * n)); CU_TRY(dalloc(&S, 2 * (size_t)T * n)); CU_TRY(dalloc(&Sk, 2 * (size_t)T * n));
    CU_TRY(dalloc(&Eu, n)); CU_TRY(dalloc(&pr, 2 * (size_t)n)); CU_TRY(dalloc(&dr, n)); CU_TRY(dalloc(&ps, n));
    CU_TRY(dalloc(&lam, n + 64)); CU_TRY(dalloc(&lnp1, T)); CU_TRY(dalloc(&psout, n)); CU_TRY(dalloc(&lnp, 1));
    hp::launch_fourier_operator(U, n, 1.0 / std::sqrt((double)n), 0);
    CU_TRY(cudaMemcpy(S, s, 2 * (size_t)T * n * sizeof(double), cudaMemcpyHostToDevice));
    if (prior) CU_TRY(cudaMemcpy(pr, prior, 2 * (size_t)n * sizeof(double), cudaMemcpyHostToDevice));
    CU_TRY(cudaMemcpy(dr, draws, n * sizeof(double), cudaMemcpyHostToDevice));
    hp::ZgemmArgs t{};
    t.A = S; t.sAi = n; t.sAk = 1;
    t.B = U; t.sBk = 1; t.sBj = n;
    t.C = Sk; t.sCi = n; t.sCj = 1;
    t.M = T; t.N = n; t.K = n; t.alpha = 1.0; t.batch = 1;
    hp::launch_zgemm(t, 0);
    hp::launch_colsumsq(Sk, Eu, T, T, n, 1, 0);
    hp::SampleArgs sp{};
    sp.Eu = Eu; sp.lnp1 = lnp1; sp.prior = pr; sp.draws = dr; sp.draws_bs = n;
    sp.ps = ps; sp.lam = lam; sp.ps_out = psout; sp.ps_bs = n; sp.lnpost_out = lnp; sp.lnpost_bs = 1;
    sp.n = n; sp.Np = n; sp.T = T; sp.Tp = T; sp.ntiles = 0; sp.nsys = 1; sp.beta_mode = 1; sp.philox = 0;
    hp::launch_sample(sp, 0);
    CU_TRY(cudaDeviceSynchronize());
    CU_TRY(cudaGetLastError());
    CU_TRY(cudaMemcpy(out, psout, n * sizeof(double), cudaMemcpyDeviceToHost));
    double* ptrs[] = {U, S, Sk, Eu, pr, dr, ps, lam, lnp1, psout, lnp};
    for (double* p : ptrs) cudaFree(p);
    return HP_OK;
}

int hp_fourier_operator(int device, int n, double* out) {
    if (!out || n < 1) return fail(HP_ERR_ARG, "hp_fourier_operator: bad argument");
    int ndev = 0;
    if (cudaGetDeviceCount(&ndev) != cudaSuccess || ndev == 0) return fail(HP_ERR_CUDA, "no CUDA device: hydra_pspec_b200 has no CPU fallback");
    CU_TRY(cudaSetDevice(device));
    double* d;
    CU_TRY(dalloc(&d, 2 * (size_t)n * n));
    hp::launch_fourier_operator(d, n, 1.0, 0);
    CU_TRY(cudaDeviceSynchronize());
    CU_TRY(cudaMemcpy(out, d, 2 * (size_t)n * n * sizeof(double), cudaMemcpyDeviceToHost));
    cudaFree(d);
    return HP_OK;
}

}
```

### hydra_pspec_b200/csrc/hp_kernels.cu

```cuda
#include "hp_kernels.cuh"
#include "hp_math.h"
#include "hp_mma.cuh"
#include "hp_diag.cuh"

namespace hp {

__device__ __forceinline__ void cp_async16(void* smem_dst, const void* gmem_src) {
    unsigned s = (unsigned)__cvta_generic_to_shared(smem_dst);
    asm volatile("cp.async.cg.shared.global [%0], [%1], 16;" ::"r"(s), "l"(gmem_src) : "memory");
}
__device__ __forceinline__ void cp_async_commit() { asm volatile("cp.async.commit_group;" ::: "memory"); }
template <int N>
__device__ __forceinline__ void cp_async_wait() { asm volatile("cp.async.wait_group %0;" ::"n"(N) : "memory"); }

__global__ void k_fourier_operator(double* out, int n, double scale) {
    long long e = blockIdx.x * (long long)blockDim.x + threadIdx.x;
    if (e >= (long long)n * n) return;
    int k = (int)(e / n), x = (int)(e % n);
    long long a = (long long)(k - n / 2) * (long long)(x - n / 2);
    long long r = a % n;
    if (r < 0) r += n;
    double s, c;
    sincospi(-2.0 * (double)r / (double)n, &s, &c);
    out[2 * e] = c * scale;
    out[2 * e + 1] = s * scale;
}
void launch_fourier_operator(double* out, int n, double scale, cudaStream_t st) {
    long long tot = (long long)n * n;
    k_fourier_operator<<<(unsigned)((tot + 255) / 256), 256, 0, st>>>(out, n, scale);
}

__global__ void k_pack_lower(const double* dense, long long ld, long long bs, double* packed, int N, int nblk) {
    const int bi = blockIdx.y, bj = blockIdx.x;
    if (bj > bi) return;
    const double* D = dense + 2 * bs * blockIdx.z;
    double* P = packed + ((size_t)blockIdx.z * tri_blocks(nblk) + blk_index(bi, bj)) * kBlkDoubles;
    for (int e = threadIdx.x; e < 1024; e += blockDim.x) {
        int r = e >> 5, c = e & 31;
        int gi = bi * 32 + r, gj = bj * 32 + c;
        double xr = 0.0, xi = 0.0;
        if (gi < N && gj < N) { xr = D[2 * (gi * ld + gj)]; xi = D[2 * (gi * ld + gj) + 1]; }
        P[e] = xr; P[1024 + e] = xi;
    }
}
void launch_pack_lower(const double* dense, long long ld, long long bs, double* packed, int N, int nblk, int batch,
                       cudaStream_t st) {
    k_pack_lower<<<dim3(nblk, nblk, batch), 256, 0, st>>>(dense, ld, bs, packed, N, nblk);
}

constexpr int kCT = 512;

__device__ __forceinline__ void load_block_async_ct(double* s, const double* g) {
    for (int c = threadIdx.x; c < kLBlkDoubles / 2; c += kCT) cp_async16(s + 2 * c, g + 2 * c);
}

struct CholWSmem {
    double A[2][kLBlkDoubles];
    double B[2][kLBlkDoubles];
    double V[kLBlkDoubles];
};
__device__ __forceinline__ void store_frag1(double* Wf1, int R, int C, double re, double im) {
    const int s = R >> 4, t = C >> 2;
    double* d = Wf1 + ((size_t)(2 * s * (s + 1) + t) * 128 + 64 * ((R >> 3) & 1) + (4 * (R & 7) + (C & 3)) * 2);
    *reinterpret_cast<double2*>(d) = make_double2(re, im);
}
__device__ __forceinline__ void store_frag2(double* Wf2, int nblk, int R, int C, double re, double im) {
    const int s = C >> 4, t = R >> 2;
    double* d = Wf2 + ((size_t)(8 * nblk * s - 2 * s * (s - 1) + t - 4 * s) * 128 + 64 * ((C >> 3) & 1) + (4 * (C & 7) + (R & 3)) * 2);
    *reinterpret_cast<double2*>(d) = make_double2(re, im);
}

__global__ void __launch_bounds__(kCT, 2) k_chol_w(CholArgs a, TrinvExtra ex, double* Wp_all, int k, int first) {
    extern __shared__ __align__(16) unsigned char smem_raw[];
    CholWSmem& s = *reinterpret_cast<CholWSmem*>(smem_raw);
    const int sys = blockIdx.x;
    const int nblk = a.nblk, Np = nblk * 32;
    const int npanel = nblk - k - 1;
    const bool wrow = !first && (int)blockIdx.y >= npanel;
    const int jp = wrow ? (int)blockIdx.y - npanel : 0;
    const double* Gp = a.Gp + (size_t)sys * tri_blocks(nblk) * kBlkDoubles;
    double* Lp = a.Lp + (size_t)sys * tri_blocks(nblk) * kLBlkDoubles;
    double* Linvp = a.Linvp + (size_t)sys * nblk * kLBlkDoubles;
    double* Wp = Wp_all + (size_t)sys * tri_blocks(nblk) * kLBlkDoubles;
    const double* lam = a.lam + (size_t)sys * Np;
    double* Wp1 = (ex.Wp1 && ex.lam) ? ex.Wp1 + (size_t)sys * tri_blocks(nblk) * kLBlkDoubles : nullptr;
    const size_t wf = (size_t)4 * nblk * (2 * nblk + 1) * 128;
    double* Wf1 = ex.Wf1 ? ex.Wf1 + (size_t)sys * wf : nullptr;
    double* Wf2 = ex.Wf2 ? ex.Wf2 + (size_t)sys * wf : nullptr;
    const int tid = threadIdx.x, warp = tid >> 5, lane = tid & 31;
    const int g = lane >> 2, q = lane & 3;
    const int ti = warp >> 2, tj = warp & 3;
    double* Ar = s.A[0];
    double* Ai = s.A[0] + kLPlane;
    double* Vr = s.V;
    double* Vi = s.V + kLPlane;

    if (wrow) {
        const double* lamj = ex.lam ? ex.lam + (size_t)sys * Np + 32 * jp : nullptr;
        double P3m[3][1][1][2], cr[1][1][2], ci[1][1][2];
        warp_zero3m<1, 1>(P3m);
        load_block_async_ct(s.V, Linvp + (size_t)k * kLBlkDoubles);
        load_block_async_ct(s.A[0], Lp + blk_index(k, jp) * kLBlkDoubles);
        load_block_async_ct(s.B[0], Wp + blk_index(jp, jp) * kLBlkDoubles);
        cp_async_commit();
        for (int j = jp; j < k; ++j) {
            const int st = (j - jp) & 1;
            cp_async_wait<0>();
            __syncthreads();
            if (j + 1 < k) {
                load_block_async_ct(s.A[st ^ 1], Lp + blk_index(k, j + 1) * kLBlkDoubles);
                load_block_async_ct(s.B[st ^ 1], Wp + blk_index(j + 1, jp) * kLBlkDoubles);
                cp_async_commit();
            }
            warp_zgemm3m<1, 1, false, false, false, false>(P3m, s.A[st] + 8 * ti * kLdBlk, s.A[st] + kLPlane + 8 * ti * kLdBlk, kLdBlk,
                                                           s.B[st] + 8 * tj, s.B[st] + kLPlane + 8 * tj, kLdBlk, 32);
        }
        __syncthreads();
        warp_zgemm3m_finish<1, 1, false, false>(P3m, cr, ci);
#pragma unroll
        for (int e = 0; e < 2; ++e) {
            const int r = 8 * ti + g, c = 8 * tj + 2 * q + e;
            s.A[0][r * kLdBlk + c] = -cr[0][0][e];
            s.A[0][kLPlane + r * kLdBlk + c] = -ci[0][0][e];
        }
        __syncthreads();
        double dr[1][1][2], di[1][1][2], Q3m[3][1][1][2];
        warp_zero3m<1, 1>(Q3m);
        warp_zgemm3m<1, 1, false, false, false, false>(Q3m, s.V + 8 * ti * kLdBlk, s.V + kLPlane + 8 * ti * kLdBlk, kLdBlk,
                                                       s.A[0] + 8 * tj, s.A[0] + kLPlane + 8 * tj, kLdBlk, 8 * (ti + 1));
        warp_zgemm3m_finish<1, 1, false, false>(Q3m, dr, di);
        double* Wb = Wp + blk_index(k, jp) * kLBlkDoubles;
        const int r = 8 * ti + g, c = 8 * tj + 2 * q;
        *reinterpret_cast<double2*>(Wb + r * kLdBlk + c) = make_double2(dr[0][0][0], dr[0][0][1]);
        *reinterpret_cast<double2*>(Wb + kLPlane + r * kLdBlk + c) = make_double2(di[0][0][0], di[0][0][1]);
        if (Wp1) {
            double* Wb1 = Wp1 + blk_index(k, jp) * kLBlkDoubles;
            const double l0 = lamj[c], l1 = lamj[c + 1];
            *reinterpret_cast<double2*>(Wb1 + r * kLdBlk + c) = make_double2(l0 * dr[0][0][0], l1 * dr[0][0][1]);
            *reinterpret_cast<double2*>(Wb1 + kLPlane + r * kLdBlk + c) = make_double2(l0 * di[0][0][0], l1 * di[0][0][1]);
        }
        if (Wf1 || Wf2) {
#pragma unroll
            for (int e = 0; e < 2; ++e) {
                const int R = 32 * k + r, C = 32 * jp + c + e;
                if (Wf1) {
                    const double l = lamj ? lamj[c + e] : 1.0;
                    store_frag1(Wf1, R, C, l * dr[0][0][e], l * di[0][0][e]);
                }
                if (Wf2) store_frag2(Wf2, nblk, R, C, dr[0][0][e], di[0][0][e]);
            }
        }
        return;
    }

    auto chol_block = [&](int i, int kc, bool diag) {
        double cr[1][1][2], ci[1][1][2], P3m[3][1][1][2];
        warp_zero<1, 1>(cr, ci);
        warp_zero3m<1, 1>(P3m);
        double mr_[2], mi_[2];
        {
            const double* Gb = Gp + blk_index(i, kc) * kBlkDoubles;
#pragma unroll
            for (int e = 0; e < 2; ++e) {
                const int r = 8 * ti + g, c = 8 * tj + 2 * q + e;
                const int gi = 32 * i + r, gj = 32 * kc + c;
                const double sc = lam[gi] * lam[gj];
                mr_[e] = sc * Gb[r * 32 + c];
                mi_[e] = sc * Gb[1024 + r * 32 + c];
                if (gi == gj && (gi < a.n || gi >= a.N)) mr_[e] += 1.0;
            }
        }
        if (!diag) load_block_async_ct(s.V, Linvp + (size_t)kc * kLBlkDoubles);
        if (kc > 0) {
            load_block_async_ct(s.A[0], Lp + blk_index(i, 0) * kLBlkDoubles);
            if (!diag) load_block_async_ct(s.B[0], Lp + blk_index(kc, 0) * kLBlkDoubles);
        }
        cp_async_commit();
        for (int j = 0; j < kc; ++j) {
            const int st = j & 1;
            cp_async_wait<0>();
            __syncthreads();
            if (j + 1 < kc) {
                load_block_async_ct(s.A[st ^ 1], Lp + blk_index(i, j + 1) * kLBlkDoubles);
                if (!diag) load_block_async_ct(s.B[st ^ 1], Lp + blk_index(kc, j + 1) * kLBlkDoubles);
                cp_async_commit();
            }
            const double* ar = s.A[st];
            const double* br = diag ? s.A[st] : s.B[st];
            warp_zgemm3m<1, 1, false, false, true, true>(P3m, ar + 8 * ti * kLdBlk, ar + kLPlane + 8 * ti * kLdBlk, kLdBlk,
                                                         br + 8 * tj * kLdBlk, br + kLPlane + 8 * tj * kLdBlk, kLdBlk, 32);
        }
        cp_async_wait<0>();
        __syncthreads();
        warp_zgemm3m_finish<1, 1, false, true>(P3m, cr, ci);
#pragma unroll
        for (int e = 0; e < 2; ++e) {
            int r = 8 * ti + g, c = 8 * tj + 2 * q + e;
            Ar[r * kLdBlk + c] = mr_[e] - cr[0][0][e];
            Ai[r * kLdBlk + c] = mi_[e] - ci[0][0][e];
        }
        __syncthreads();
        if (diag) {
            const bool bad = diag_chol_inverse_block(Ar, Ai, Vr, Vi, tid, kCT);
            __syncthreads();
            double* Lb = Lp + blk_index(kc, kc) * kLBlkDoubles;
            double* Vb = Linvp + (size_t)kc * kLBlkDoubles;
            double* Wb = Wp + blk_index(kc, kc) * kLBlkDoubles;
            const double* lamk = ex.lam ? ex.lam + (size_t)sys * Np + 32 * kc : nullptr;
            for (int e = tid; e < kLBlkDoubles; e += kCT) {
                const double v = s.V[e];
                Lb[e] = s.A[0][e];
                Vb[e] = v;
                Wb[e] = v;
                if (Wp1) {
                    const int c = (e % kLPlane) % kLdBlk;
                    Wp1[blk_index(kc, kc) * kLBlkDoubles + e] = c < 32 ? v * lamk[c] : 0.0;
                }
            }
            if (Wf1 || Wf2) {
                for (int e = tid; e < 1024; e += kCT) {
                    const int r = e >> 5, c = e & 31;
                    const double re = Vr[r * kLdBlk + c], im = Vi[r * kLdBlk + c];
                    if (Wf1 && c < 16 * ((r >> 4) + 1)) {
                        const double l = lamk ? lamk[c] : 1.0;
                        store_frag1(Wf1, 32 * kc + r, 32 * kc + c, l * re, l * im);
                    }
                    if (Wf2 && r >= 16 * (c >> 4)) store_frag2(Wf2, nblk, 32 * kc + r, 32 * kc + c, re, im);
                }
            }
            if (bad && tid == 0 && a.info) atomicMax(a.info + sys, kc + 1);
        } else {
            double dr[1][1][2], di[1][1][2], Q3m[3][1][1][2];
            warp_zero3m<1, 1>(Q3m);
            warp_zgemm3m<1, 1, false, false, true, true>(Q3m, Ar + 8 * ti * kLdBlk, Ai + 8 * ti * kLdBlk, kLdBlk, Vr + 8 * tj * kLdBlk,
                                                         Vi + 8 * tj * kLdBlk, kLdBlk, 32);
            warp_zgemm3m_finish<1, 1, false, true>(Q3m, dr, di);
            double* Lb = Lp + blk_index(i, kc) * kLBlkDoubles;
            int r = 8 * ti + g, c = 8 * tj + 2 * q;
            *reinterpret_cast<double2*>(Lb + r * kLdBlk + c) = make_double2(dr[0][0][0], dr[0][0][1]);
            *reinterpret_cast<double2*>(Lb + kLPlane + r * kLdBlk + c) = make_double2(di[0][0][0], di[0][0][1]);
        }
    };
    if (first) { chol_block(0, 0, true); return; }
    chol_block(k + 1 + (int)blockIdx.y, k, false);
    if (blockIdx.y == 0) {
        __syncthreads();
        chol_block(k + 1, k + 1, true);
    }
}

int launch_chol_trinv(const CholArgs& a, double* Wp, const TrinvExtra& ex, cudaStream_t st) {
    static bool attr_dev[kMaxDev] = {false};
    bool& attr_set = attr_dev[current_device_slot()];
    if (!attr_set) {
        cudaFuncSetAttribute(k_chol_w, cudaFuncAttributeMaxDynamicSharedMemorySize, (int)sizeof(CholWSmem));
        attr_set = true;
    }
    if (a.info) cudaMemsetAsync(a.info, 0, sizeof(int) * a.nsys, st);
    k_chol_w<<<dim3(a.nsys, 1), kCT, sizeof(CholWSmem), st>>>(a, ex, Wp, 0, 1);
    if (a.nblk == 1) return 1;
    for (int k = 0; k < a.nblk; ++k) k_chol_w<<<dim3(a.nsys, a.nblk - 1), kCT, sizeof(CholWSmem), st>>>(a, ex, Wp, k, 0);
    return a.nblk + 1;
}

__global__ void __launch_bounds__(128) k_post(PostArgs a) {
    extern __shared__ double fsh[];
    const int sys = blockIdx.y, t = blockIdx.x;
    const double* X = a.X + 2 * ((size_t)sys * a.Tp + t) * a.Np;
    for (int j = threadIdx.x; j < 2 * a.m; j += blockDim.x) fsh[j] = X[2 * a.n + j];
    __syncthreads();
    if (a.fg_out && t < a.T)
        for (int j = threadIdx.x; j < 2 * a.m; j += blockDim.x) a.fg_out[(size_t)sys * a.fg_bs + (size_t)t * 2 * a.m + j] = fsh[j];
    const double* Sf = a.Sf + 2 * ((size_t)sys * a.sf_bs + (size_t)t * a.n);
    const double* wd = a.wd + 2 * ((size_t)sys * a.Tp + t) * a.n;
    const double* Ft = a.Ft + 2 * (size_t)sys * a.m * a.n;
    const double* w = a.w + (size_t)sys * a.n;
    const double* nd = a.ninvd + (size_t)sys * a.n;
    double part = 0.0;
    for (int x = threadIdx.x; x < a.n; x += blockDim.x) {
        double sr = 0.0, si = 0.0;
        if (t < a.T) { sr = Sf[2 * x]; si = Sf[2 * x + 1]; }
        double mr = sr, mi = si;
        for (int j = 0; j < a.m; ++j) {
            double fr = Ft[2 * ((size_t)j * a.n + x)], fi = Ft[2 * ((size_t)j * a.n + x) + 1];
            double ar = fsh[2 * j], ai = fsh[2 * j + 1];
            mr += ar * fr - ai * fi;
            mi += ar * fi + ai * fr;
        }
        double rr = wd[2 * x] - mr, ri = wd[2 * x + 1] - mi;
        double r2 = rr * rr + ri * ri;
        if (t < a.T) {
            if (a.chisq_out) a.chisq_out[(size_t)sys * a.chisq_bs + (size_t)t * a.n + x] = r2 * nd[x];
            part += w[x] * nd[x] * r2;
            if (a.Rm) {
                double* p = a.Rm + 2 * (((size_t)sys * a.Tp + t) * a.n + x);
                p[0] = w[x] * rr; p[1] = w[x] * ri;
            }
        }
        if (a.Wm) {
            double* p = a.Wm + 2 * (((size_t)sys * a.Tp + t) * a.n + x);
            p[0] = w[x] * sr; p[1] = w[x] * si;
        }
    }
    __shared__ double redp[4];
    for (int o = 16; o > 0; o >>= 1) part += __shfl_down_sync(0xffffffffu, part, o);
    if ((threadIdx.x & 31) == 0) redp[threadIdx.x >> 5] = part;
    __syncthreads();
    if (threadIdx.x == 0) {
        double s = 0.0;
        for (int i = 0; i < (int)(blockDim.x >> 5); ++i) s += redp[i];
        a.lnp1[(size_t)sys * a.Tp + t] = t < a.T ? s : 0.0;
    }
}
void launch_post(const PostArgs& a, cudaStream_t st) {
    k_post<<<dim3(a.Tp, a.nsys), 128, 2 * a.m * sizeof(double), st>>>(a);
}

__global__ void __launch_bounds__(256) k_colsumsq(const double* A, double* out, int T, int Tp, int n, int ld) {
    __shared__ double red[8][33];
    const int sys = blockIdx.y;
    const int k = blockIdx.x * 32 + (threadIdx.x & 31), tg = threadIdx.x >> 5;
    double acc = 0.0;
    if (k < n)
        for (int t = tg; t < T; t += 8) {
            const double* p = A + 2 * (((size_t)sys * Tp + t) * ld + k);
            acc += p[0] * p[0] + p[1] * p[1];
        }
    red[tg][threadIdx.x & 31] = acc;
    __syncthreads();
    if (tg == 0 && k < n) {
        double s = 0.0;
#pragma unroll
        for (int i = 0; i < 8; ++i) s += red[i][threadIdx.x & 31];
        out[(size_t)sys * n + k] = s;
    }
}
void launch_colsumsq(const double* A, double* out, int T, int Tp, int n, int nsys, cudaStream_t st, int ld) {
    k_colsumsq<<<dim3((n + 31) / 32, nsys), 256, 0, st>>>(A, out, T, Tp, n, ld > 0 ? ld : n);
}

__device__ __forceinline__ double block_reduce(double v, double* sh, int op) {
    for (int o = 16; o > 0; o >>= 1) {
        double w = __shfl_xor_sync(0xffffffffu, v, o);
        v = op == 0 ? v + w : (op == 1 ? fmin(v, w) : fmax(v, w));
    }
    __syncthreads();
    if ((threadIdx.x & 31) == 0) sh[threadIdx.x >> 5] = v;
    __syncthreads();
    if (threadIdx.x < 32) {
        double x = sh[threadIdx.x];
        for (int o = 16; o > 0; o >>= 1) {
            double w = __shfl_xor_sync(0xffffffffu, x, o);
            x = op == 0 ? x + w : (op == 1 ? fmin(x, w) : fmax(x, w));
        }
        if (threadIdx.x == 0) sh[32] = x;
    }
    __syncthreads();
    return sh[32];
}

__global__ void __launch_bounds__(1024) k_sample(SampleArgs a) {
    __shared__ double sh[40];
    __shared__ double cdf[kInvGrid + 24];
    __shared__ double pmx[kInvGrid + 24];
    __shared__ double wmax[33];
    __shared__ double beta_s;
    const int sys = blockIdx.x, tid = threadIdx.x;
    const int n = a.n;
    double* ps = a.ps + (size_t)sys * n;
    double* lam = a.lam + (size_t)sys * a.Np;
    const double* prior = a.prior + (size_t)sys * 2 * n;
    const double* draws = a.draws ? a.draws + (size_t)sys * a.draws_bs : nullptr;
    const double alpha = (double)a.T - 1.0;
    const uint32_t chain = a.chain_ids ? (uint32_t)a.chain_ids[sys] : (uint32_t)(a.chain0 + sys);

    double lp2 = 0.0;
    for (int k0 = 0; k0 < n; k0 += 1024) {
        int k = k0 + tid;
        double beta = 0.0, newps = 0.0;
        bool has_prior = false;
        if (k < n) {
            if (a.beta_mode == 0) {
                double s = 0.0;
                for (int tl = 0; tl < a.ntiles; ++tl) s += a.Ppart[((size_t)sys * a.ntiles + tl) * n + k];
                beta = ps[k] * s;
            } else if (a.ntilesE > 0) {
                double s = 0.0;
                for (int tl = 0; tl < a.ntilesE; ++tl) s += a.Eu[((size_t)sys * a.ntilesE + tl) * n + k];
                beta = (double)n * s;
            } else {
                beta = (double)n * a.Eu[(size_t)sys * n + k];
            }
            has_prior = prior[k] > 0.0 || prior[n + k] > 0.0;
            if (!has_prior) {
                if (!a.philox) newps = draws[k] * beta;
                else newps = beta / gamma_mt(alpha, (uint32_t)k, a.iter, chain, a.key0, a.key1 ^ 0x5A5A5A5Au);
            }
        }
        for (int kk = k0; kk < min(k0 + 1024, n); ++kk) {
            bool hp_ = prior[kk] > 0.0 || prior[n + kk] > 0.0;
            if (!hp_) continue;
            if (tid == kk - k0) beta_s = beta;
            __syncthreads();
            const double b = beta_s;
            const double l0 = log10(prior[n + kk]), l1 = log10(prior[kk]);
            double xj = 0.0, cj = 0.0;
            if (tid < kInvGrid) {
                xj = invsamp_grid_x(l0, l1, tid, kInvGrid);
                cj = igamc(alpha + 1.0, b / xj);
            }
            double mn = block_reduce(tid < kInvGrid ? cj : INFINITY, sh, 1);
            cj -= mn;
            double mx = block_reduce(tid < kInvGrid ? cj : -INFINITY, sh, 2);
            cj /= mx;
// ... 70 lines not shown
```

### hydra_pspec_b200/csrc/hp_kernels.cuh

```cuda
#pragma once
#include <cuda_runtime.h>
#include <stdint.h>

namespace hp {

constexpr int kNB = 32;
constexpr int kBlkDoubles = 2 * 32 * 32;
constexpr int kLdBlk = 36;
constexpr int kLPlane = 32 * kLdBlk;
constexpr int kLBlkDoubles = 2 * kLPlane;
constexpr int kTT = 16;
constexpr int kInvGrid = 1000;

constexpr int kMaxDev = 64;
inline int current_device_slot() {
    int d = 0;
    cudaGetDevice(&d);
    return (d < 0 || d >= kMaxDev) ? 0 : d;
}

__host__ __device__ inline size_t tri_blocks(int nblk) { return (size_t)nblk * (nblk + 1) / 2; }
__host__ __device__ inline size_t blk_index(int i, int j) { return (size_t)i * (i + 1) / 2 + j; }

struct ZgemmArgs {
    const double* A; long long sAi, sAk, bsA;
    const double* B; long long sBk, sBj, bsB;
    double* C;       long long sCi, sCj, bsC;
    const double* dk; long long bsD;
    int M, N, K;
    int conjA, conjB, accumulate;
    double alpha;
    int batch;
    int tri;
    int lower_out;
};
void launch_zgemm(const ZgemmArgs& a, cudaStream_t st);

void launch_fourier_operator(double* out, int n, double scale, cudaStream_t st);

void launch_pack_lower(const double* dense, long long ld, long long bs, double* packed, int N, int nblk,
                       int batch, cudaStream_t st);

struct CholArgs {
    const double* Gp;
    const double* lam;
    double* Lp;
    double* Linvp;
    int* info;
    int nblk, n, N, nsys;
};
struct TrinvExtra { double* Wp1; double* Wf1; double* Wf2; const double* lam; };
int launch_chol_trinv(const CholArgs& a, double* Wp, const TrinvExtra& ex, cudaStream_t st);

struct SolveArgs {
    const double* Wp;
    const double* lam;
    const double* Rfix;
    const double* wa;
    double* X;
    double* Ssc;
    double* Ppart;
    int nblk, n, N, Tp, ntiles, nsys;
    int T;
    int philox_wa;
    int stages;
    int rows_per_round;
    int cg_compat;
    uint32_t key0, key1, iter;
    const int* chain_ids;
    int chain0;
};
void launch_solve(const SolveArgs& a, cudaStream_t st);
size_t solve_smem_bytes(int nblk);
bool solve_resident_ok(int nblk, size_t max_smem);

struct Solve2Args {
    const double* W1;
    const double* W2;
    const double* Rt;
    double* X;
    double* Ppart;
    int nblk, n, N, Tp, ntiles, nsys, T;
    int philox;
    uint32_t key0, key1, iter;
    const int* chain_ids;
    int chain0;
    int stages;
    int grid_limit;
};
void launch_solve2(const Solve2Args& a, cudaStream_t st);
int solve2_stages(int nblk, size_t max_smem);
void launch_rhs_tile(double* Rt, const double* Rfix, const double* wa, const double* lam, int nblk, int n, int N, int T, int Tp,
                     int ntiles, int nsys, cudaStream_t st);
void launch_cg_scale(double* X, const double* Rfix, const double* wa, const double* lam, int n, int N, int Np, int T, int Tp,
                     int nsys, cudaStream_t st);

constexpr int kS3Warps = 16;
constexpr int kS3MaxStrips = 28;
constexpr int kS3MaxPerWarp = 8;
struct Solve3Sched {
    uint8_t n[2][kS3Warps];
    uint8_t strip[2][kS3Warps][kS3MaxPerWarp];
};
struct Solve3Args {
    const double* Wf1;
    const double* Wf2;
    const double* Rt;
    double* X;
    double* Ppart;
    int nblk, n, N, Tp, ntiles, nsys, T;
    int philox;
    uint32_t key0, key1, iter;
    const int* chain_ids;
    int chain0;
    int grid_limit;
    int nstrip;
    Solve3Sched sched;
};
void launch_solve3(const Solve3Args& a, cudaStream_t st);
bool solve3_ok(int nblk, size_t max_smem);
size_t solve3_frag_doubles(int nblk);
void solve3_make_schedule(int nblk, Solve3Sched* sc, int nstrip = 0);

struct PostArgs {
    const double* Sf;
    long long sf_bs;
    const double* X;
    const double* Ft;
    const double* wd;
    const double* w;
    const double* ninvd;
    double* fg_out;
    double* chisq_out;
    double* Wm;
    double* Rm;
    double* lnp1;
    int n, m, Np, T, Tp, nsys;
    long long fg_bs, chisq_bs;
};
void launch_post(const PostArgs& a, cudaStream_t st);

void launch_colsumsq(const double* A, double* out, int T, int Tp, int n, int nsys, cudaStream_t st, int ld = 0);

struct PtArgs {
    const double* H;
    const double* lam;
    const double* Rfix;
    const double* wa;
    double* X;
    double* scratch;
    const int* same_prev;
    int* info;
    int nblk, n, m, N, T, Tp, nsys;
    int philox_wa;
    uint32_t key0, key1, iter;
    const int* chain_ids;
    int chain0;
};
size_t pt_smem_bytes(int nblk, int n);
size_t pt_scratch_doubles_per_cta(int nblk);
int pt_grid(int nsys, int T);
void launch_pt_cholsolve(const PtArgs& a, int grid, cudaStream_t st);

constexpr int kPtLowMaxRank = 64;
struct PtLowArgs {
    const double* Rfix;
    const double* wa;
    const double* lam;
    double* X;
    const double* Pm;
    const uint16_t* fidx;
    const int* fcnt;
    int* info;
    int n, N, Np, T, Tp, Tp0, nsys, nblk, kcap;
    int philox;
    uint32_t key0, key1, iter;
    const int* chain_ids;
    int chain0;
};
size_t pt_lowrank_smem_bytes(int kcap, int warps);
void launch_pt_lowrank(const PtLowArgs& a, cudaStream_t st);
void launch_pt_arows(double* Rfix_sys, const double* Bmat_sys, const double* ni_sys, int n, int Np, int Tp0, cudaStream_t st);

struct SampleArgs {
    const double* Ppart;
    const double* Eu;
    const double* Em;
    const double* lnp1;
    const double* lnp1_dense;
    const double* prior;
    const double* draws;
    double* ps;
    double* lam;
    double* ps_out;
    double* lnpost_out;
    int n, Np, T, Tp, ntiles, nsys;
    int beta_mode, philox;
    int ntilesE;
    uint32_t key0, key1, iter;
    const int* chain_ids;
    int chain0;
    long long ps_bs, lnpost_bs, draws_bs;
};
void launch_sample(const SampleArgs& a, cudaStream_t st);
// ... 35 lines not shown
```

### hydra_pspec_b200/csrc/hp_pertime.cu

```cuda
#include "hp_kernels.cuh"
#include "hp_math.h"
#include "hp_mma.cuh"
#include "hp_diag.cuh"

namespace hp {
#ifdef HP_PT_TIMERS
__device__ unsigned long long g_pt_cycles[8];
#define PT_T(idx) do { if (tid == 0) { long long _n = clock64(); tacc[idx] += _n - tlast; tlast = _n; } } while (0)
#else
#define PT_T(idx) do { } while (0)
#endif
namespace {

constexpr int kPT = 512;

__device__ __forceinline__ void pt_cp_async16(void* smem_dst, const void* gmem_src) {
    unsigned s = (unsigned)__cvta_generic_to_shared(smem_dst);
    asm volatile("cp.async.cg.shared.global [%0], [%1], 16;" ::"r"(s), "l"(gmem_src) : "memory");
}
__device__ __forceinline__ void pt_commit() { asm volatile("cp.async.commit_group;" ::: "memory"); }
template <int N>
__device__ __forceinline__ void pt_wait() { asm volatile("cp.async.wait_group %0;" ::"n"(N) : "memory"); }
__device__ __forceinline__ void pt_load_block(double* s, const double* g) {
    for (int c = threadIdx.x; c < kLBlkDoubles / 2; c += kPT) pt_cp_async16(s + 2 * c, g + 2 * c);
// ... 15 lines not shown
    double* lamS = yi + Np;
    double* chr = lamS + Np;
    double* chi = chr + n;
    const int tid = threadIdx.x, warp = tid >> 5, lane = tid & 31;
    const int g = lane >> 2, q = lane & 3;
    const int ti = warp >> 2, tj = warp & 3;
    const int mr = tid >> 4, ms = tid & 15;
    double* Ar = s.A[0];
    double* Ai = s.A[0] + kLPlane;
    double* Vr = s.V;
    double* Vi = s.V + kLPlane;
    double* redr = s.B[0];
    double* redi = s.B[0] + 16 * 32;
    const size_t tri = tri_blocks(nblk);
    double* Lp = a.scratch + (size_t)blockIdx.x * (tri + nblk) * kLBlkDoubles;
    double* Vp = Lp + tri * kLBlkDoubles;
    const long long nitems = (long long)a.nsys * a.T;
#ifdef HP_PT_TIMERS
    long long tacc[8] = {0, 0, 0, 0, 0, 0, 0, 0}, tlast = clock64();
#endif

    const long long chunk = (nitems + gridDim.x - 1) / gridDim.x;
    const long long item_begin = (long long)blockIdx.x * chunk;
    const long long item_end = item_begin + chunk < nitems ? item_begin + chunk : nitems;
    for (long long item = item_begin; item < item_end; ++item) {
        const int sys = (int)(item / a.T), t = (int)(item % a.T);
        const bool reuse = item > item_begin && t > 0 && a.same_prev && a.same_prev[(size_t)sys * a.Tp + t] != 0;
        const double2* H = reinterpret_cast<const double2*>(a.H) + ((size_t)sys * a.Tp + t) * (size_t)(1 + m) * Np;
        const double* lam = a.lam + (size_t)sys * Np;
        const double2* R = reinterpret_cast<const double2*>(a.Rfix) + ((size_t)sys * a.Tp + t) * Np;
        const double2* WA = a.wa ? reinterpret_cast<const double2*>(a.wa) + ((size_t)sys * a.Tp + t) * Np : nullptr;
        __syncthreads();
        for (int e = tid; e < Np; e += kPT) {
            const double l = lam[e];
            double2 r = R[e];
            r.x *= l; r.y *= l;
            if (WA) { double2 w = WA[e]; r.x += w.x; r.y += w.y; }
            lamS[e] = l; yr[e] = r.x; yi[e] = r.y;
        }
        for (int e = tid; e < n; e += kPT) { double2 c = H[e]; chr[e] = c.x; chi[e] = c.y; }
        __syncthreads();
        int bad = 0;
        PT_T(0);

        if (reuse) {
            {
                const char* base = reinterpret_cast<const char*>(Lp);
                const size_t bytes = (tri + nblk) * (size_t)kLBlkDoubles * 8;
                for (size_t off = (size_t)tid * 128; off < bytes; off += (size_t)kPT * 128)
                    asm volatile("prefetch.global.L2 [%0];" ::"l"(base + off));
            }
            for (int k = 0; k < nblk; ++k) {
                double f0r = 0.0, f0i = 0.0, f1r = 0.0, f1i = 0.0;
                for (int j = 0; j < k; ++j) {
                    const double* Lb = Lp + blk_index(k, j) * kLBlkDoubles + mr * kLdBlk + 2 * ms;
                    const double lr0 = __ldcg(Lb), lr1 = __ldcg(Lb + 1), li0 = __ldcg(Lb + kLPlane), li1 = __ldcg(Lb + kLPlane + 1);
                    const double2 vr = *reinterpret_cast<const double2*>(yr + 32 * j + 2 * ms);
                    const double2 vi = *reinterpret_cast<const double2*>(yi + 32 * j + 2 * ms);
                    f0r += lr0 * vr.x - li0 * vi.x; f0i += lr0 * vi.x + li0 * vr.x;
                    f1r += lr1 * vr.y - li1 * vi.y; f1i += lr1 * vi.y + li1 * vr.y;
                }
                double fr = f0r + f1r, fi = f0i + f1i;
                for (int o = 8; o > 0; o >>= 1) {
                    fr += __shfl_xor_sync(0xffffffffu, fr, o);
                    fi += __shfl_xor_sync(0xffffffffu, fi, o);
                }
                if (ms == 0) { s.tv[mr] = yr[32 * k + mr] - fr; s.tv[32 + mr] = yi[32 * k + mr] - fi; }
                __syncthreads();
                {
                    const double* Vb = Vp + (size_t)k * kLBlkDoubles + mr * kLdBlk + 2 * ms;
                    const double vr0 = __ldcg(Vb), vr1 = __ldcg(Vb + 1), vi0 = __ldcg(Vb + kLPlane), vi1 = __ldcg(Vb + kLPlane + 1);
                    const double2 xr = *reinterpret_cast<const double2*>(s.tv + 2 * ms);
                    const double2 xi = *reinterpret_cast<const double2*>(s.tv + 32 + 2 * ms);
                    double pr = vr0 * xr.x - vi0 * xi.x + vr1 * xr.y - vi1 * xi.y;
                    double pi = vr0 * xi.x + vi0 * xr.x + vr1 * xi.y + vi1 * xr.y;
                    for (int o = 8; o > 0; o >>= 1) {
                        pr += __shfl_xor_sync(0xffffffffu, pr, o);
                        pi += __shfl_xor_sync(0xffffffffu, pi, o);
                    }
                    if (ms == 0) { yr[32 * k + mr] = pr; yi[32 * k + mr] = pi; }
                }
                __syncthreads();
            }
        } else
        for (int k = 0; k < nblk; ++k) {
            double fr = 0.0, fi = 0.0;
            for (int i = k; i < nblk; ++i) {
                double cr[1][1][2], ci[1][1][2];
                warp_zero<1, 1>(cr, ci);
                double P3m[3][1][1][2];
                warp_zero3m<1, 1>(P3m);
                __syncthreads();
                if (k > 0) {
                    pt_load_block(s.A[0], Lp + blk_index(i, 0) * kLBlkDoubles);
                    if (i != k) pt_load_block(s.B[0], Lp + blk_index(k, 0) * kLBlkDoubles);
                    pt_commit();
                }
                for (int j = 0; j < k; ++j) {
                    const int st = j & 1;
                    if (j + 1 < k) {
                        pt_load_block(s.A[st ^ 1], Lp + blk_index(i, j + 1) * kLBlkDoubles);
                        if (i != k) pt_load_block(s.B[st ^ 1], Lp + blk_index(k, j + 1) * kLBlkDoubles);
                        pt_commit();
                        pt_wait<1>();
                    } else {
                        pt_wait<0>();
                    }
                    __syncthreads();
                    const double* ar = s.A[st];
                    const double* br = (i != k) ? s.B[st] : s.A[st];
                    warp_zgemm3m<1, 1, false, false, true, true>(P3m, ar + 8 * ti * kLdBlk, ar + kLPlane + 8 * ti * kLdBlk,
                                                               kLdBlk, br + 8 * tj * kLdBlk, br + kLPlane + 8 * tj * kLdBlk,
                                                               kLdBlk, 32);
                    if (i == k) {
                        const double2 lr = *reinterpret_cast<const double2*>(ar + mr * kLdBlk + 2 * ms);
                        const double2 li = *reinterpret_cast<const double2*>(ar + kLPlane + mr * kLdBlk + 2 * ms);
                        const double2 vr = *reinterpret_cast<const double2*>(yr + 32 * j + 2 * ms);
                        const double2 vi = *reinterpret_cast<const double2*>(yi + 32 * j + 2 * ms);
                        fr += lr.x * vr.x - li.x * vi.x + lr.y * vr.y - li.y * vi.y;
                        fi += lr.x * vi.x + li.x * vr.x + lr.y * vi.y + li.y * vr.y;
                    }
                    __syncthreads();
                }
                PT_T(1);
                warp_zgemm3m_finish<1, 1, false, true>(P3m, cr, ci);
#pragma unroll
                for (int e = 0; e < 2; ++e) {
                    const int r = 8 * ti + g, c = 8 * tj + 2 * q + e;
                    const int gi = 32 * i + r, gj = 32 * k + c;
                    double vr, vi;
                    if (gi >= N || gj >= N) {
                        vr = gi == gj ? 1.0 : 0.0; vi = 0.0;
                    } else if (gi < n && gj < n) {
                        int d = gi - gj;
                        if (d < 0) d += n;
                        const double sc = lamS[gi] * lamS[gj];
                        vr = sc * chr[d]; vi = sc * chi[d];
                        if (gi == gj) vr += 1.0;
                    } else if (gj >= n) {
                        const double2 h = H[(size_t)(1 + gj - n) * Np + gi];
                        const double sc = lamS[gi];
                        vr = sc * h.x; vi = sc * h.y;
                    } else {
                        const double2 h = H[(size_t)(1 + gi - n) * Np + gj];
                        const double sc = lamS[gj];
                        vr = sc * h.x; vi = -sc * h.y;
                    }
                    Ar[r * kLdBlk + c] = vr - cr[0][0][e];
                    Ai[r * kLdBlk + c] = vi - ci[0][0][e];
                }
                __syncthreads();
                PT_T(2);
                if (i == k) {
                    if (diag_chol_inverse_block(Ar, Ai, Vr, Vi, tid, kPT)) bad = k + 1;
                    __syncthreads();
                    PT_T(3);
                    for (int o = 8; o > 0; o >>= 1) {
                        fr += __shfl_xor_sync(0xffffffffu, fr, o);
                        fi += __shfl_xor_sync(0xffffffffu, fi, o);
                    }
                    if (ms == 0) { s.tv[mr] = yr[32 * k + mr] - fr; s.tv[32 + mr] = yi[32 * k + mr] - fi; }
                    __syncthreads();
                    {
                        const double2 vr = *reinterpret_cast<const double2*>(Vr + mr * kLdBlk + 2 * ms);
                        const double2 vi = *reinterpret_cast<const double2*>(Vi + mr * kLdBlk + 2 * ms);
                        const double2 xr = *reinterpret_cast<const double2*>(s.tv + 2 * ms);
                        const double2 xi = *reinterpret_cast<const double2*>(s.tv + 32 + 2 * ms);
                        double pr = vr.x * xr.x - vi.x * xi.x + vr.y * xr.y - vi.y * xi.y;
                        double pi = vr.x * xi.x + vi.x * xr.x + vr.y * xi.y + vi.y * xr.y;
                        for (int o = 8; o > 0; o >>= 1) {
                            pr += __shfl_xor_sync(0xffffffffu, pr, o);
                            pi += __shfl_xor_sync(0xffffffffu, pi, o);
                        }
                        if (ms == 0) { yr[32 * k + mr] = pr; yi[32 * k + mr] = pi; }
                    }
                    double* Lb = Lp + blk_index(k, k) * kLBlkDoubles;
                    double* Vb = Vp + (size_t)k * kLBlkDoubles;
                    for (int e = tid; e < kLBlkDoubles; e += kPT) {
                        Lb[e] = s.A[0][e];
                        Vb[e] = s.V[e];
                    }
                    PT_T(4);
                } else {
                    double dr[1][1][2], di[1][1][2];
                    warp_zero<1, 1>(dr, di);
                    double Q3m[3][1][1][2];
                    warp_zero3m<1, 1>(Q3m);
                    warp_zgemm3m<1, 1, false, false, true, true>(Q3m, Ar + 8 * ti * kLdBlk, Ai + 8 * ti * kLdBlk, kLdBlk,
                                                               Vr + 8 * tj * kLdBlk, Vi + 8 * tj * kLdBlk, kLdBlk, 32);
                    warp_zgemm3m_finish<1, 1, false, true>(Q3m, dr, di);
                    double* Lb = Lp + blk_index(i, k) * kLBlkDoubles;
                    const int r = 8 * ti + g, c = 8 * tj + 2 * q;
                    *reinterpret_cast<double2*>(Lb + r * kLdBlk + c) = make_double2(dr[0][0][0], dr[0][0][1]);
                    *reinterpret_cast<double2*>(Lb + kLPlane + r * kLdBlk + c) = make_double2(di[0][0][0], di[0][0][1]);
                    PT_T(5);
                }
            }
        }
        __syncthreads();
        if (bad && tid == 0 && a.info) atomicMax(a.info + sys, bad);

        if (a.philox_wa) {
            const uint32_t chain = a.chain_ids ? (uint32_t)a.chain_ids[sys] : (uint32_t)(a.chain0 + sys);
            for (int row = tid; row < N; row += kPT) {
                u32x4 ctr; ctr.x = (uint32_t)row; ctr.y = (uint32_t)t; ctr.z = a.iter; ctr.w = chain;
                double n0, n1;
                normal_pair_fast(philox4x32_10(ctr, a.key0, a.key1 ^ 0xA5A5A5A5u), n0, n1);
                yr[row] += n0 * 0.70710678118654752440;
                yi[row] += n1 * 0.70710678118654752440;
            }
        }
        __syncthreads();

        auto prefetch_row = [&](int i) {
            const char* vb = reinterpret_cast<const char*>(Vp + (size_t)i * kLBlkDoubles);
            for (int off = tid * 128; off < (int)(kLBlkDoubles * 8); off += kPT * 128)
                asm volatile("prefetch.global.L2 [%0];" ::"l"(vb + off));
            for (int j = i + 1; j < nblk; ++j) {
                const char* lb = reinterpret_cast<const char*>(Lp + blk_index(j, i) * kLBlkDoubles);
                for (int off = tid * 128; off < (int)(kLBlkDoubles * 8); off += kPT * 128)
                    asm volatile("prefetch.global.L2 [%0];" ::"l"(lb + off));
            }
        };
        prefetch_row(nblk - 1);
        for (int i = nblk - 1; i >= 0; --i) {
            if (i > 0) prefetch_row(i - 1);
            double pr = 0.0, pi = 0.0;
            for (int j = i + 1 + warp; j < nblk; j += 16) {
                const double* Lr = Lp + blk_index(j, i) * kLBlkDoubles + lane;
                const double* Li = Lr + kLPlane;
                const double* xr = yr + 32 * j;
                const double* xi = yi + 32 * j;
#pragma unroll 8
                for (int r = 0; r < 32; ++r) {
                    const double lr = __ldcg(Lr + r * kLdBlk), li = __ldcg(Li + r * kLdBlk);
                    pr += lr * xr[r] + li * xi[r];
                    pi += lr * xi[r] - li * xr[r];
                }
            }
            redr[warp * 32 + lane] = pr; redi[warp * 32 + lane] = pi;
            __syncthreads();
            if (tid < 32) {
                double tr = 0.0, tim = 0.0;
#pragma unroll
                for (int pp = 0; pp < 16; ++pp) { tr += redr[pp * 32 + lane]; tim += redi[pp * 32 + lane]; }
                s.tv[lane] = yr[32 * i + lane] - tr;
                s.tv[32 + lane] = yi[32 * i + lane] - tim;
            }
            __syncthreads();
            {
                const double* Vg = Vp + (size_t)i * kLBlkDoubles + lane;
                pr = 0.0; pi = 0.0;
#pragma unroll
                for (int rr = 0; rr < 2; ++rr) {
                    const int r = 2 * warp + rr;
                    const double vr = __ldcg(Vg + r * kLdBlk), vi = __ldcg(Vg + kLPlane + r * kLdBlk);
                    pr += vr * s.tv[r] + vi * s.tv[32 + r];
                    pi += vr * s.tv[32 + r] - vi * s.tv[r];
                }
                redr[warp * 32 + lane] = pr; redi[warp * 32 + lane] = pi;
            }
            __syncthreads();
            if (tid < 32) {
                double tr = 0.0, tim = 0.0;
#pragma unroll
                for (int pp = 0; pp < 16; ++pp) { tr += redr[pp * 32 + lane]; tim += redi[pp * 32 + lane]; }
                yr[32 * i + lane] = tr;
                yi[32 * i + lane] = tim;
            }
            __syncthreads();
        }
        PT_T(6);
        double2* X = reinterpret_cast<double2*>(a.X) + ((size_t)sys * a.Tp + t) * Np;
        for (int e = tid; e < Np; e += kPT) X[e] = make_double2(yr[e], yi[e]);
        PT_T(7);
    }
#ifdef HP_PT_TIMERS
    if (tid == 0) for (int i = 0; i < 8; ++i) atomicAdd(&g_pt_cycles[i], (unsigned long long)tacc[i]);
#endif
}

}

size_t pt_smem_bytes(int nblk, int n) { return sizeof(PtSmem) + sizeof(double) * ((size_t)3 * nblk * 32 + 2 * n); }
size_t pt_scratch_doubles_per_cta(int nblk) { return (tri_blocks(nblk) + nblk) * (size_t)kLBlkDoubles; }

int pt_grid(int nsys, int T) {
    static int ctas = 0;
    if (!ctas) {
        int dev = 0, sms = 0;
        cudaGetDevice(&dev);
        cudaDeviceGetAttribute(&sms, cudaDevAttrMultiProcessorCount, dev);
        ctas = 2 * (sms > 0 ? sms : 148);
    }
    long long items = (long long)nsys * T;
    return (int)(items < ctas ? items : ctas);
}

#ifdef HP_PT_TIMERS
extern "C" void hp_pt_timers(unsigned long long* out, int reset) {
    cudaDeviceSynchronize();
    cudaMemcpyFromSymbol(out, g_pt_cycles, sizeof(unsigned long long) * 8);
    if (reset) { unsigned long long z[8] = {0}; cudaMemcpyToSymbol(g_pt_cycles, z, sizeof(z)); }
}
#endif
void launch_pt_cholsolve(const PtArgs& a, int grid, cudaStream_t st) {
    const size_t smem = pt_smem_bytes(a.nblk, a.n);
// ... 11 lines not shown
```

### hydra_pspec_b200/csrc/hp_testhooks.cu

```cuda
#include "../../include/hydra_pspec_b200.h"
#include "hp_kernels.cuh"

#include <string>
#include <vector>

extern "C" {

int hp_test_zgemm(int M, int N, int K, const double* A, int transA, int conjA, const double* B, int transB, int conjB,
                  const double* dk, double* C) {
    double *dA, *dB, *dC, *dD = nullptr;
    if (cudaMalloc(&dA, 16ull * M * K) || cudaMalloc(&dB, 16ull * K * N) || cudaMalloc(&dC, 16ull * M * N)) return HP_ERR_CUDA;
    cudaMemcpy(dA, A, 16ull * M * K, cudaMemcpyHostToDevice);
    cudaMemcpy(dB, B, 16ull * K * N, cudaMemcpyHostToDevice);
    if (dk) { cudaMalloc(&dD, 8ull * K); cudaMemcpy(dD, dk, 8ull * K, cudaMemcpyHostToDevice); }
    hp::ZgemmArgs g{};
    g.A = dA; g.sAi = transA ? 1 : K; g.sAk = transA ? M : 1; g.conjA = conjA;
    g.B = dB; g.sBk = transB ? 1 : N; g.sBj = transB ? K : 1; g.conjB = conjB;
    g.C = dC; g.sCi = N; g.sCj = 1; g.dk = dD;
    g.M = M; g.N = N; g.K = K; g.alpha = 1.0; g.batch = 1;
    hp::launch_zgemm(g, 0);
    cudaError_t e = cudaDeviceSynchronize();
    cudaMemcpy(C, dC, 16ull * M * N, cudaMemcpyDeviceToHost);
    cudaFree(dA); cudaFree(dB); cudaFree(dC); cudaFree(dD);
    return e == cudaSuccess ? HP_OK : HP_ERR_CUDA;
}

int hp_test_chol_solve(int n, int m, int T, const double* G, const double* lam, const double* Rfix, const double* wa,
                       int cg_compat, double* Ldense, double* X, int* info) {
    const int N = n + m, nblk = (N + 31) / 32, Np = nblk * 32, ntiles = (T + 15) / 16, Tp = ntiles * 16;
    double *dG, *dGp, *dlam, *dLp, *dLinv, *dWp, *dR, *dW = nullptr, *dX, *dS, *dP;
    int* dinfo;
    size_t tri = hp::tri_blocks(nblk) * hp::kLBlkDoubles, trig = hp::tri_blocks(nblk) * hp::kBlkDoubles;
    cudaMalloc(&dG, 16ull * N * N); cudaMalloc(&dGp, 8 * trig); cudaMalloc(&dlam, 8ull * Np); cudaMalloc(&dLp, 8 * tri);
    cudaMalloc(&dLinv, 8ull * nblk * hp::kLBlkDoubles); cudaMalloc(&dWp, 8 * tri); cudaMalloc(&dR, 16ull * Tp * Np); cudaMalloc(&dX, 16ull * Tp * Np);
    cudaMalloc(&dS, 16ull * Tp * n); cudaMalloc(&dP, 8ull * ntiles * n); cudaMalloc(&dinfo, 4);
    cudaMemset(dR, 0, 16ull * Tp * Np); cudaMemset(dlam, 0, 8ull * Np);
    cudaMemcpy(dG, G, 16ull * N * N, cudaMemcpyHostToDevice);
    cudaMemcpy(dlam, lam, 8ull * N, cudaMemcpyHostToDevice);
    cudaMemcpy2D(dR, 16ull * Np, Rfix, 16ull * N, 16ull * N, T, cudaMemcpyHostToDevice);
    if (wa) {
        cudaMalloc(&dW, 16ull * Tp * Np); cudaMemset(dW, 0, 16ull * Tp * Np);
        cudaMemcpy2D(dW, 16ull * Np, wa, 16ull * n, 16ull * n, T, cudaMemcpyHostToDevice);
    }
    hp::launch_pack_lower(dG, N, 0, dGp, N, nblk, 1, 0);
    hp::CholArgs ca{};
    ca.Gp = dGp; ca.lam = dlam; ca.Lp = dLp; ca.Linvp = dLinv; ca.info = dinfo; ca.nblk = nblk; ca.n = n; ca.N = N; ca.nsys = 1;
    hp::launch_chol_trinv(ca, dWp, hp::TrinvExtra{nullptr, nullptr, nullptr, nullptr}, 0);
    hp::SolveArgs sa{};
    sa.Wp = dWp; sa.lam = dlam; sa.Rfix = dR; sa.wa = dW; sa.X = dX; sa.Ssc = dS; sa.Ppart = dP;
    sa.nblk = nblk; sa.n = n; sa.N = N; sa.Tp = Tp; sa.ntiles = ntiles; sa.nsys = 1; sa.T = T; sa.cg_compat = cg_compat;
    hp::launch_solve(sa, 0);
    cudaError_t e = cudaDeviceSynchronize();
    if (e == cudaSuccess) {
        cudaMemcpy2D(X, 16ull * N, dX, 16ull * Np, 16ull * N, T, cudaMemcpyDeviceToHost);
        cudaMemcpy(info, dinfo, 4, cudaMemcpyDeviceToHost);
        if (Ldense) {
            std::vector<double> lp(tri);
            cudaMemcpy(lp.data(), dLp, 8 * tri, cudaMemcpyDeviceToHost);
            for (int i = 0; i < N; ++i)
                for (int j = 0; j < N; ++j) {
                    double re = 0, im = 0;
                    if (j <= i) {
                        const double* b = lp.data() + hp::blk_index(i / 32, j / 32) * hp::kLBlkDoubles;
                        re = b[(i % 32) * hp::kLdBlk + (j % 32)]; im = b[hp::kLPlane + (i % 32) * hp::kLdBlk + (j % 32)];
                    }
                    Ldense[2 * ((size_t)i * N + j)] = re; Ldense[2 * ((size_t)i * N + j) + 1] = im;
                }
        }
    }
    cudaFree(dG); cudaFree(dGp); cudaFree(dlam); cudaFree(dLp); cudaFree(dLinv); cudaFree(dWp); cudaFree(dR); cudaFree(dW); cudaFree(dX);
    cudaFree(dS); cudaFree(dP); cudaFree(dinfo);
    return e == cudaSuccess ? HP_OK : HP_ERR_CUDA;
}


int hp_test_solve2(int n, int m, int T, int nsys, const double* G, const double* lam, const double* Rfix, const double* wa,
                   int cg_compat, int grid_limit, int variant, double* X, double* psum) {
    const int N = n + m, nblk = (N + 31) / 32, Np = nblk * 32, ntiles = (T + 15) / 16, Tp = ntiles * 16;
    int max_smem = 0, dev = 0;
    cudaGetDevice(&dev);
    cudaDeviceGetAttribute(&max_smem, cudaDevAttrMaxSharedMemoryPerBlockOptin, dev);
    if (variant == 3 ? !hp::solve3_ok(nblk, (size_t)max_smem) : hp::solve2_stages(nblk, (size_t)max_smem) == 0) return HP_ERR_SIZE;
    const int ppt = variant == 3 ? ntiles : 2 * ntiles;
    const size_t wf = hp::solve3_frag_doubles(nblk);
    double *dWf1 = nullptr, *dWf2 = nullptr;
    double *dG, *dGp, *dlam, *dLp, *dLinv, *dWp, *dWp1, *dR, *dW = nullptr, *dX, *dP, *dRt;
    int* dinfo;
    const size_t tri = hp::tri_blocks(nblk) * hp::kLBlkDoubles, trig = hp::tri_blocks(nblk) * hp::kBlkDoubles;
    const size_t rt_doubles = (size_t)nsys * ntiles * nblk * 2 * 32 * hp::kTT;
    cudaMalloc(&dG, 16ull * N * N); cudaMalloc(&dGp, 8 * trig); cudaMalloc(&dlam, 8ull * Np); cudaMalloc(&dLp, 8 * tri);
    cudaMalloc(&dLinv, 8ull * nblk * hp::kLBlkDoubles); cudaMalloc(&dWp, 8 * tri); cudaMalloc(&dWp1, 8 * tri);
    cudaMalloc(&dR, 16ull * nsys * Tp * Np); cudaMalloc(&dX, 16ull * nsys * Tp * Np);
    cudaMalloc(&dP, 8ull * nsys * 2 * ntiles * n); cudaMalloc(&dinfo, 4); cudaMalloc(&dRt, 8 * rt_doubles);
    cudaMemset(dR, 0, 16ull * nsys * Tp * Np); cudaMemset(dlam, 0, 8ull * Np); cudaMemset(dX, 0xff, 16ull * nsys * Tp * Np);
    cudaMemcpy(dG, G, 16ull * N * N, cudaMemcpyHostToDevice);
    cudaMemcpy(dlam, lam, 8ull * N, cudaMemcpyHostToDevice);
    for (int s = 0; s < nsys; ++s)
        cudaMemcpy2D(dR + 2ull * s * Tp * Np, 16ull * Np, Rfix + 2ull * s * T * N, 16ull * N, 16ull * N, T, cudaMemcpyHostToDevice);
    if (wa) {
        cudaMalloc(&dW, 16ull * nsys * Tp * Np); cudaMemset(dW, 0, 16ull * nsys * Tp * Np);
        for (int s = 0; s < nsys; ++s)
            cudaMemcpy2D(dW + 2ull * s * Tp * Np, 16ull * Np, wa + 2ull * s * T * n, 16ull * n, 16ull * n, T, cudaMemcpyHostToDevice);
    }
    hp::launch_pack_lower(dG, N, 0, dGp, N, nblk, 1, 0);
    hp::CholArgs ca{};
    ca.Gp = dGp; ca.lam = dlam; ca.Lp = dLp; ca.Linvp = dLinv; ca.info = dinfo; ca.nblk = nblk; ca.n = n; ca.N = N; ca.nsys = 1;
    if (variant == 3) {
        cudaMalloc(&dWf1, 8 * wf * nsys); cudaMalloc(&dWf2, 8 * wf * nsys);
        cudaMemset(dWf1, 0xff, 8 * wf * nsys); cudaMemset(dWf2, 0xff, 8 * wf * nsys);
    }
    hp::launch_chol_trinv(ca, dWp, hp::TrinvExtra{dWp1, dWf1, dWf2, wa ? nullptr : dlam}, 0);
    if (variant != 3 && wa) cudaMemcpy(dWp1, dWp, 8 * tri, cudaMemcpyDeviceToDevice);
    for (int s = 0; s < nsys; ++s) {
        hp::launch_rhs_tile(dRt + (size_t)s * ntiles * nblk * 2 * 32 * hp::kTT, dR + 2ull * s * Tp * Np,
                            dW ? dW + 2ull * s * Tp * Np : nullptr, wa ? dlam : nullptr, nblk, n, N, T, Tp, ntiles, 1, 0);
    }
    double *dWall, *dW1all;
    cudaMalloc(&dWall, 8 * tri * nsys); cudaMalloc(&dW1all, 8 * tri * nsys);
    for (int s = 0; s < nsys; ++s) {
        cudaMemcpy(dWall + tri * s, dWp, 8 * tri, cudaMemcpyDeviceToDevice);
        cudaMemcpy(dW1all + tri * s, dWp1, 8 * tri, cudaMemcpyDeviceToDevice);
        if (variant == 3 && s > 0) {
            cudaMemcpy(dWf1 + wf * s, dWf1, 8 * wf, cudaMemcpyDeviceToDevice);
            cudaMemcpy(dWf2 + wf * s, dWf2, 8 * wf, cudaMemcpyDeviceToDevice);
        }
    }
    if (variant == 3) {
        hp::Solve3Args s3{};
        s3.Wf1 = dWf1; s3.Wf2 = dWf2; s3.Rt = dRt; s3.X = dX; s3.Ppart = dP;
        s3.nblk = nblk; s3.n = n; s3.N = N; s3.Tp = Tp; s3.ntiles = ntiles; s3.nsys = nsys; s3.T = T;
        s3.philox = 0; s3.grid_limit = grid_limit;
        s3.nstrip = (N + 15) / 16;
        hp::solve3_make_schedule(nblk, &s3.sched, s3.nstrip);
        hp::launch_solve3(s3, 0);
    } else {
    hp::Solve2Args sa{};
    sa.W1 = dW1all; sa.W2 = dWall; sa.Rt = dRt; sa.X = dX; sa.Ppart = dP;
    sa.nblk = nblk; sa.n = n; sa.N = N; sa.Tp = Tp; sa.ntiles = ntiles; sa.nsys = nsys; sa.T = T;
    sa.philox = 0; sa.grid_limit = grid_limit;
    hp::launch_solve2(sa, 0);
    }
    if (cg_compat)
        for (int s = 0; s < nsys; ++s)
            hp::launch_cg_scale(dX + 2ull * s * Tp * Np, dR + 2ull * s * Tp * Np, dW ? dW + 2ull * s * Tp * Np : nullptr, dlam, n, N,
                                Np, T, Tp, 1, 0);
    cudaError_t e = cudaDeviceSynchronize();
    if (e == cudaSuccess) {
        for (int s = 0; s < nsys; ++s)
            cudaMemcpy2D(X + 2ull * s * T * N, 16ull * N, dX + 2ull * s * Tp * Np, 16ull * Np, 16ull * N, T, cudaMemcpyDeviceToHost);
        if (psum) {
            std::vector<double> pp((size_t)nsys * ppt * n);
            cudaMemcpy(pp.data(), dP, 8 * pp.size(), cudaMemcpyDeviceToHost);
            for (int s = 0; s < nsys; ++s)
                for (int k = 0; k < n; ++k) {
                    double acc = 0.0;
                    for (int tl = 0; tl < ppt; ++tl) acc += pp[((size_t)s * ppt + tl) * n + k];
                    psum[(size_t)s * n + k] = acc;
                }
        }
    }
    cudaFree(dG); cudaFree(dGp); cudaFree(dlam); cudaFree(dLp); cudaFree(dLinv); cudaFree(dWp); cudaFree(dWp1); cudaFree(dR);
    cudaFree(dW); cudaFree(dX); cudaFree(dP); cudaFree(dinfo); cudaFree(dRt); cudaFree(dWall); cudaFree(dW1all); cudaFree(dWf1); cudaFree(dWf2);
    return e == cudaSuccess ? HP_OK : HP_ERR_CUDA;
}

int hp_test_solve3_schedule(int nblk, unsigned char* n, unsigned char* strips, int* nwarps, int* max_per_warp) {
    if (nblk < 1 || 2 * nblk > hp::kS3MaxStrips) return HP_ERR_SIZE;
    hp::Solve3Sched sc{};
    hp::solve3_make_schedule(nblk, &sc);
    for (int p = 0; p < 2; ++p)
        for (int w = 0; w < hp::kS3Warps; ++w) {
            n[p * hp::kS3Warps + w] = sc.n[p][w];
            for (int e = 0; e < hp::kS3MaxPerWarp; ++e) strips[(p * hp::kS3Warps + w) * hp::kS3MaxPerWarp + e] = sc.strip[p][w][e];
        }
    *nwarps = hp::kS3Warps;
    *max_per_warp = hp::kS3MaxPerWarp;
    return HP_OK;
}

namespace {
__global__ void __launch_bounds__(256) k_fp64_peak(double* out, int iters, double a, double b) {
    double c[8][2];
#pragma unroll
    for (int i = 0; i < 8; ++i) { c[i][0] = threadIdx.x; c[i][1] = i; }
    for (int it = 0; it < iters; ++it) {
#pragma unroll
        for (int i = 0; i < 8; ++i)
            asm volatile("mma.sync.aligned.m8n8k4.row.col.f64.f64.f64.f64 {%0,%1}, {%2}, {%3}, {%0,%1};"
                         : "+d"(c[i][0]), "+d"(c[i][1]) : "d"(a), "d"(b));
    }
    double s = 0;
#pragma unroll
    for (int i = 0; i < 8; ++i) s += c[i][0] + c[i][1];
    if (s == 12345.678) out[0] = s;
}
}

double hp_fp64_peak_tflops(int device, double seconds) {
    if (cudaSetDevice(device) != cudaSuccess) return -1.0;
    int nsm = 0;
    cudaDeviceGetAttribute(&nsm, cudaDevAttrMultiProcessorCount, device);
    double* out;
    if (cudaMalloc(&out, 8) != cudaSuccess) return -1.0;
    cudaEvent_t e0, e1;
    cudaEventCreate(&e0); cudaEventCreate(&e1);
    const int iters = 20000, bps = 4;
    k_fp64_peak<<<nsm * bps, 256>>>(out, iters / 10, 1.0000001, 1e-9);
    cudaDeviceSynchronize();
    double best = 0.0, spent = 0.0;
    while (spent < seconds * 1e3) {
        cudaEventRecord(e0);
        k_fp64_peak<<<nsm * bps, 256>>>(out, iters, 1.0000001, 1e-9);
        cudaEventRecord(e1);
        if (cudaEventSynchronize(e1) != cudaSuccess) { best = -1.0; break; }
        float ms;
        cudaEventElapsedTime(&ms, e0, e1);
        double tf = 2.0 * 8 * 256 / 32.0 * iters * 256.0 * nsm * bps / ms * 1e-9;
        if (tf > best) best = tf;
        spent += ms;
    }
    cudaEventDestroy(e0); cudaEventDestroy(e1); cudaFree(out);
    return best;
}

void* hp_pinned_alloc(size_t bytes) {
    void* p = nullptr;
    if (cudaHostAlloc(&p, bytes, cudaHostAllocDefault) != cudaSuccess) return nullptr;
    return p;
}
void hp_pinned_free(void* p) { if (p) cudaFreeHost(p); }

}
```

### include/hydra_pspec_b200.h

```cpp
#ifndef HYDRA_PSPEC_B200_H
#define HYDRA_PSPEC_B200_H

#include <stddef.h>
#include <stdint.h>

#ifdef __cplusplus
extern "C" {
#endif

typedef struct hp_engine hp_engine;

enum hp_status { HP_OK = 0, HP_ERR_ARG = -1, HP_ERR_CUDA = -2, HP_ERR_SIZE = -3, HP_ERR_NUMERIC = -4 };

enum hp_rng_mode {
    HP_RNG_INJECTED = 0,
    HP_RNG_PHILOX = 1
};

enum hp_keep { HP_KEEP_CR = 1, HP_KEEP_FG = 2, HP_KEEP_CHISQ = 4 };

enum hp_buffer {
    HP_BUF_PS = 0,
    HP_BUF_LNPOST = 1,
    HP_BUF_CR = 2,
    HP_BUF_FG = 3,
    HP_BUF_CHISQ = 4,
    HP_BUF_LAST_CR = 5,
    HP_BUF_LAST_FG = 6,
    HP_BUF_PS_CUR = 7
};

typedef struct hp_config {
    int device;
    int nchains;
    int ntimes, nfreqs, nmodes;
    int rng_mode;
    int cg_compat;
    int refresh_omega;
    int keep;
    int max_iters;
    int general_basis0;
    int profile;
    int substreams;
    int dense_noise;
    int force_dense_transforms;
    int force_dense_solve;
    int time_flags;
    int ring_iters;
    uint64_t seed;
    void* stream;
} hp_config;

#define HP_NUM_KERNEL_CLASSES 6
const char* hp_kernel_class_name(int cls);

int hp_engine_create(const hp_config* cfg, hp_engine** out);
int hp_engine_destroy(hp_engine* e);

int hp_engine_load_chain(hp_engine* e, int chain, const double* vis, const uint8_t* flags, const double* fgmodes,
                         const double* ninv_diag, const double* basis0, const double* lam0sq,
                         const double* ps_prior);

int hp_engine_load_chain_dense(hp_engine* e, int chain, const double* vis, const uint8_t* flags, const double* fgmodes,
                               const double* ninv_diag, const double* ninv_dense, const double* nih_dense,
                               const double* basis0, const double* lam0sq, const double* ps_prior);

int hp_engine_set_draws(hp_engine* e, int chain, const double* omega_a, const double* omega_b,
                        const double* s_draws, int n_draw_iters);

int hp_engine_run(hp_engine* e, int niter);
typedef struct hp_host_sink {
    double* signal_ps; double* ln_post; double* signal_cr; double* fg_amps; double* chisq;
    int iters;
    int first_iter;
    int iter_major;
    int read_ahead;
} hp_host_sink;
int hp_engine_run_to_host(hp_engine* e, int niter, const hp_host_sink* sink);
int hp_engine_gcr(hp_engine* e);
int hp_engine_sync(hp_engine* e);
int hp_engine_iterations_done(const hp_engine* e);
int hp_engine_rewind(hp_engine* e);

int hp_engine_read(hp_engine* e, int chain, int buffer, int iter0, int niter, void* dst, size_t dst_bytes);
int hp_engine_read_signal_S(hp_engine* e, int chain, double* dst);
int hp_engine_info(hp_engine* e, int* info_host);

int hp_engine_kernel_ms(hp_engine* e, double* ms, int* launches, int reset);
int hp_engine_set_chain_ids(hp_engine* e, const int* ids);
int hp_engine_set_substreams(hp_engine* e, int n);
int hp_engine_set_profile(hp_engine* e, int on);
int hp_engine_pt_form(const hp_engine* e, int* low_rank, int* max_rank);
long long hp_engine_launch_count(const hp_engine* e);

int hp_sample_S(int device, int ntimes, int nfreqs, const double* s, const double* prior, const double* draws,
                double* out);

int hp_fourier_operator(int device, int n, double* out);
int hp_eigh_batch(int device, int n, int batch, const double* S, double* V, double* w, int* sweeps);

int hp_test_zgemm(int M, int N, int K, const double* A, int transA, int conjA, const double* B, int transB, int conjB,
                  const double* dk, double* C);
int hp_test_chol_solve(int n, int m, int T, const double* G, const double* lam, const double* Rfix, const double* wa,
                       int cg_compat, double* Ldense, double* X, int* info);
int hp_test_solve2(int n, int m, int T, int nsys, const double* G, const double* lam, const double* Rfix, const double* wa,
                   int cg_compat, int grid_limit, int variant, double* X, double* psum);

int hp_test_solve3_schedule(int nblk, unsigned char* n, unsigned char* strips, int* nwarps, int* max_per_warp);

double hp_fp64_peak_tflops(int device, double seconds);
void hp_release_cached_memory(void);
void* hp_pinned_alloc(size_t bytes);
void hp_pinned_free(void* p);

const char* hp_last_error(void);
const char* hp_version(void);

#ifdef __cplusplus
}
#endif
#endif
```

Before: 16680.

## Replace blocked Cholesky/inverse with dataflow task kernel using per-block ready flags

Introduces a persistent task kernel for the blocked Cholesky factorisation and triangular inverse. CTAs pull tasks from an atomic counter and wait on per-block acquire/release flags with a timeout abort. This lets diagonal, panel and inverse blocks across systems overlap instead of being serialised by per-step launches or block-wide barriers. It adds spin-wait overhead, a sync-word arena, and a timeout error path in the info check.

```diff
diff --git a/hydra_pspec_b200/_lib.py b/hydra_pspec_b200/_lib.py
--- a/hydra_pspec_b200/_lib.py
+++ b/hydra_pspec_b200/_lib.py
@@ -69,6 +69,7 @@
                                      C.c_int, C.c_void_p, C.c_void_p, C.c_void_p]),
     "hp_test_solve2": (C.c_int, [C.c_int, C.c_int, C.c_int, C.c_int, C.c_void_p, C.c_void_p, C.c_void_p, C.c_void_p,
                                  C.c_int, C.c_int, C.c_int, C.c_void_p, C.c_void_p]),
+    "hp_test_chol_batch": (C.c_int, [C.c_int, C.c_int, C.c_int] + [C.c_void_p] * 7),
     "hp_test_solve3_schedule": (C.c_int, [C.c_int, C.c_void_p, C.c_void_p, C.POINTER(C.c_int), C.POINTER(C.c_int)]),
     "hp_fp64_peak_tflops": (C.c_double, [C.c_int, C.c_double]),
     "hp_release_cached_memory": (None, []),
diff --git a/hydra_pspec_b200/csrc/hp_diag.cuh b/hydra_pspec_b200/csrc/hp_diag.cuh
--- a/hydra_pspec_b200/csrc/hp_diag.cuh
+++ b/hydra_pspec_b200/csrc/hp_diag.cuh
@@ -59,23 +59,32 @@
     return bad;
 }
 
-__device__ __forceinline__ bool diag_chol_inverse_block(double* Ar, double* Ai, double* Vr, double* Vi, int tid, int nthreads) {
+template <int nthreads>
+__device__ __forceinline__ bool diag_chol_inverse_block(double* Ar, double* Ai, double* Vr, double* Vi, int tid) {
     const int warp = tid >> 5, lane = tid & 31;
+    constexpr int nwarps = nthreads >> 5;
     const int g = lane >> 2, q = lane & 3;
     bool bad = false;
     auto sub = [](double* base, int R, int C) { return base + (8 * R) * kLdBlk + 8 * C; };
+    auto on_warps = [&](int n, auto&& body) {
+        if constexpr (nwarps >= 6) {
+            if (warp < n) body(warp);
+        } else {
+            for (int w = warp; w < n; w += nwarps) body(w);
+        }
+    };
     for (int e = tid; e < kLBlkDoubles; e += nthreads) Vr[e] = 0.0;
-    if (warp < 6) {
-        const int R = warp < 3 ? 0 : (warp < 5 ? 1 : 2), C = warp < 3 ? warp + 1 : (warp < 5 ? warp - 1 : 3);
+    on_warps(6, [&](int w) {
+        const int R = w < 3 ? 0 : (w < 5 ? 1 : 2), C = w < 3 ? w + 1 : (w < 5 ? w - 1 : 3);
         for (int e = lane; e < 64; e += 32) { sub(Ar, R, C)[(e >> 3) * kLdBlk + (e & 7)] = 0.0; sub(Ai, R, C)[(e >> 3) * kLdBlk + (e & 7)] = 0.0; }
-    }
+    });
     __syncthreads();
     for (int kk = 0; kk < 4; ++kk) {
         if (warp == 0) bad |= diag_chol_inverse8(sub(Ar, kk, kk), sub(Ai, kk, kk), sub(Vr, kk, kk), sub(Vi, kk, kk));
         if (kk == 3) break;
         __syncthreads();
-        if (warp < 3 - kk) {
-            const int R = kk + 1 + warp;
+        on_warps(3 - kk, [&](int w) {
+            const int R = kk + 1 + w;
             double P[3][1][1][2], cr[1][1][2], ci[1][1][2];
             warp_zero3m<1, 1>(P);
             warp_zgemm3m<1, 1, false, false, true, true>(P, sub(Ar, R, kk), sub(Ai, R, kk), kLdBlk, sub(Vr, kk, kk), sub(Vi, kk, kk),
@@ -84,11 +93,11 @@
             __syncwarp();
             *reinterpret_cast<double2*>(sub(Ar, R, kk) + g * kLdBlk + 2 * q) = make_double2(cr[0][0][0], cr[0][0][1]);
             *reinterpret_cast<double2*>(sub(Ai, R, kk) + g * kLdBlk + 2 * q) = make_double2(ci[0][0][0], ci[0][0][1]);
-        }
+        });
         __syncthreads();
         const int ntr = (3 - kk) * (4 - kk) / 2;
-        if (warp < ntr) {
-            int R = kk + 1, C = kk + 1, w = warp;
+        on_warps(ntr, [&](int w0) {
+            int R = kk + 1, C = kk + 1, w = w0;
             while (w > R - (kk + 1)) { w -= R - kk; ++R; }
             C = kk + 1 + w;
             double P[3][1][1][2], cr[1][1][2], ci[1][1][2];
@@ -101,13 +110,13 @@
             double2 xr = *dr, xi = *di;
             xr.x -= cr[0][0][0]; xr.y -= cr[0][0][1]; xi.x -= ci[0][0][0]; xi.y -= ci[0][0][1];
             *dr = xr; *di = xi;
-        }
+        });
         __syncthreads();
     }
     __syncthreads();
     for (int d = 1; d < 4; ++d) {
-        if (warp < 4 - d) {
-            const int C = warp, R = C + d;
+        on_warps(4 - d, [&](int w) {
+            const int C = w, R = C + d;
             double P[3][1][1][2], cr[1][1][2], ci[1][1][2];
             warp_zero3m<1, 1>(P);
             warp_zgemm3m<1, 1, false, false, false, false>(P, sub(Ar, R, C), sub(Ai, R, C), kLdBlk, sub(Vr, C, C), sub(Vi, C, C),
@@ -123,7 +132,7 @@
             __syncwarp();
             *reinterpret_cast<double2*>(sub(Vr, R, C) + g * kLdBlk + 2 * q) = make_double2(-cr[0][0][0], -cr[0][0][1]);
             *reinterpret_cast<double2*>(sub(Vi, R, C) + g * kLdBlk + 2 * q) = make_double2(-ci[0][0][0], -ci[0][0][1]);
-        }
+        });
         __syncthreads();
     }
     return bad;
diff --git a/hydra_pspec_b200/csrc/hp_engine.cu b/hydra_pspec_b200/csrc/hp_engine.cu
--- a/hydra_pspec_b200/csrc/hp_engine.cu
+++ b/hydra_pspec_b200/csrc/hp_engine.cu
@@ -254,6 +254,7 @@
     double *NiL = nullptr;
     double *NiD = nullptr, *NihD = nullptr, *Td = nullptr, *Rm = nullptr, *Yd = nullptr;
     int* info = nullptr;
+    unsigned* chol_sync = nullptr;
     int* chain_ids = nullptr;
     double *X = nullptr, *Ssc = nullptr, *Ppart = nullptr, *Sf = nullptr, *Wm = nullptr, *Tmp = nullptr;
     double *Em = nullptr, *Eu = nullptr, *lnp1 = nullptr;
@@ -525,6 +526,7 @@
     ap.want(&e->tw, 2 * n);
     if (e->fft2_ok) ap.want(&e->tw2, 4 * n);
     ap.want(&e->Empart, C * e->ntilesE * n); ap.want(&e->Eupart, C * e->ntilesE * n);
+    ap.want(&e->chol_sync, C * hp::chol_sync_words(e->nblk, 1));
     {
         cudaError_t ce = ap.commit(&e->arena, &e->arena_bytes, cfg->device, e->st);
         if (ce != cudaSuccess) {
@@ -936,6 +938,7 @@
     hp::CholArgs ca{};
     ca.Gp = OFFS(b.Gp, tri * hp::kBlkDoubles); ca.lam = OFFS(e->lam, Np); ca.Lp = OFFS(e->Lp, tri * hp::kLBlkDoubles);
     ca.Linvp = OFFS(e->Linvp, (size_t)e->nblk * hp::kLBlkDoubles); ca.info = e->info + sb.c0;
+    ca.sync = OFFS(e->chol_sync, hp::chol_sync_words(e->nblk, 1));
     ca.nblk = e->nblk; ca.n = e->n; ca.N = e->N; ca.nsys = sb.nc;
     const hp::TrinvExtra ex{OFFS(e->Wp1, tri * hp::kLBlkDoubles), OFFS(e->Wf1, hp::solve3_frag_doubles(e->nblk)),
                             OFFS(e->Wf2, hp::solve3_frag_doubles(e->nblk)), philox ? OFFS(e->lam, Np) : nullptr};
@@ -1488,6 +1491,9 @@
     CU_TRY(cudaSetDevice(e->cfg.device));
     CU_TRY(cudaStreamSynchronize(e->st));
     CU_TRY(cudaMemcpy(info_host, e->info, e->C * sizeof(int), cudaMemcpyDeviceToHost));
+    for (int c = 0; c < e->C; ++c)
+        if (info_host[c] == hp::kCholTimeout)
+            return fail(HP_ERR_CUDA, "k_chol_tasks gave up waiting for a block of the factorisation (chain " + std::to_string(c) + ")");
     return HP_OK;
 }
 
diff --git a/hydra_pspec_b200/csrc/hp_kernels.cu b/hydra_pspec_b200/csrc/hp_kernels.cu
--- a/hydra_pspec_b200/csrc/hp_kernels.cu
+++ b/hydra_pspec_b200/csrc/hp_kernels.cu
@@ -48,29 +48,316 @@
     k_pack_lower<<<dim3(nblk, nblk, batch), 256, 0, st>>>(dense, ld, bs, packed, N, nblk);
 }
 
+constexpr int kTaskCT = 128;
+constexpr int kCholGroup = 32;
+constexpr long long kCholSpinCycles = 2000000000LL;
+
+__device__ __forceinline__ void load_block_async_task(double* s, const double* g) {
+    for (int c = threadIdx.x; c < kLBlkDoubles / 2; c += kTaskCT) cp_async16(s + 2 * c, g + 2 * c);
+}
+
+struct CholTaskSmem {
+    double A[2][kLBlkDoubles];
+    double B[2][kLBlkDoubles];
+};
+__device__ __forceinline__ void store_frag1(double* Wf1, int R, int C, double re, double im) {
+    *reinterpret_cast<double2*>(Wf1 + frag1_offset(R, C)) = make_double2(re, im);
+}
+__device__ __forceinline__ void store_frag2(double* Wf2, int nblk, int R, int C, double re, double im) {
+    *reinterpret_cast<double2*>(Wf2 + frag2_offset(nblk, R, C)) = make_double2(re, im);
+}
+
+__device__ __forceinline__ unsigned ld_acquire(const unsigned* p) {
+    unsigned v;
+    asm volatile("ld.acquire.gpu.global.u32 %0, [%1];" : "=r"(v) : "l"(p) : "memory");
+    return v;
+}
+__device__ __forceinline__ void st_release(unsigned* p, unsigned v) {
+    asm volatile("st.release.gpu.global.u32 [%0], %1;" ::"l"(p), "r"(v) : "memory");
+}
+__device__ __noinline__ bool chol_wait(const unsigned* flag, unsigned* abort_word, int* info, bool block) {
+    if (ld_acquire(flag)) return true;
+    if (!block) return false;
+    const long long t0 = clock64();
+    unsigned ns = 32;
+    for (;;) {
+        __nanosleep(ns);
+        if (ns < 256) ns *= 2;
+        if (ld_acquire(flag)) return true;
+        if (*(volatile unsigned*)abort_word) return false;
+        if (clock64() - t0 > kCholSpinCycles) {
+            atomicExch(abort_word, 1u);
+            if (info) atomicMax(info, kCholTimeout);
+            return false;
+        }
+    }
+}
+
+template <int MODE>
+__device__ __forceinline__ bool chol_accumulate(double (&P)[3][2][2][2], CholTaskSmem& s, const double* Lp, const double* Wp,
+                                                const double* Vg, const unsigned* flags, size_t tri, int ia, int kb, int kv,
+                                                int j0, int j1, unsigned* abort_word, int* info) {
+    const int tid = threadIdx.x, warp = tid >> 5, ti = warp >> 1, tj = warp & 1;
+    auto ready = [&](int j, bool block) -> bool {
+        if (j == j1) return MODE == 0 || chol_wait(flags + blk_index(kv, kv), abort_word, info, block);
+        if (!chol_wait(flags + blk_index(ia, j), abort_word, info, block)) return false;
+        if (MODE == 1) return chol_wait(flags + blk_index(kb, j), abort_word, info, block);
+        if (MODE == 2) return chol_wait(flags + (j == kb ? blk_index(kb, kb) : tri + blk_index(j, kb)), abort_word, info, block);
+        return true;
+    };
+    auto load = [&](int j, int b) {
+        if (j == j1) {
+            if (MODE != 0) load_block_async_task(s.B[b], Vg);
+        } else {
+            load_block_async_task(s.A[b], Lp + blk_index(ia, j) * kLBlkDoubles);
+            if (MODE == 1) load_block_async_task(s.B[b], Lp + blk_index(kb, j) * kLBlkDoubles);
+            if (MODE == 2) load_block_async_task(s.B[b], Wp + blk_index(j, kb) * kLBlkDoubles);
+        }
+        cp_async_commit();
+    };
+    if (__syncthreads_or(tid == 0 && !ready(j0, true))) return false;
+    load(j0, 0);
+    for (int j = j0; j < j1; ++j) {
+        const int st = (j - j0) & 1;
+        const bool later = tid == 0 && !ready(j + 1, false);
+        cp_async_wait<0>();
+        const bool late = __syncthreads_or(later);
+        if (!late) load(j + 1, st ^ 1);
+        const double* ar = s.A[st];
+        const double* br = MODE == 0 ? s.A[st] : s.B[st];
+        if (MODE == 2)
+            warp_zgemm3m<2, 2, false, false, false, false>(P, ar + 16 * ti * kLdBlk, ar + kLPlane + 16 * ti * kLdBlk, kLdBlk,
+                                                           br + 16 * tj, br + kLPlane + 16 * tj, kLdBlk, 32);
+        else
+            warp_zgemm3m<2, 2, false, false, true, true>(P, ar + 16 * ti * kLdBlk, ar + kLPlane + 16 * ti * kLdBlk, kLdBlk,
+                                                         br + 16 * tj * kLdBlk, br + kLPlane + 16 * tj * kLdBlk, kLdBlk, 32);
+        if (late) {
+            if (__syncthreads_or(tid == 0 && !ready(j + 1, true))) return false;
+            load(j + 1, st ^ 1);
+        }
+    }
+    cp_async_wait<0>();
+    __syncthreads();
+    return true;
+}
+
+__global__ void __launch_bounds__(kTaskCT, 3) k_chol_tasks(CholArgs a, TrinvExtra ex, double* Wp_all) {
+    extern __shared__ __align__(16) unsigned char smem_raw[];
+    CholTaskSmem& s = *reinterpret_cast<CholTaskSmem*>(smem_raw);
+    __shared__ int s_task;
+    const int nblk = a.nblk, Np = nblk * 32;
+    const size_t tri = tri_blocks(nblk);
+    const int per_sys = nblk * nblk, ntask = a.nsys * per_sys;
+    unsigned* counter = a.sync;
+    unsigned* abort_word = a.sync + 1;
+    const size_t wf = (size_t)4 * nblk * (2 * nblk + 1) * 128;
+    const int tid = threadIdx.x, warp = tid >> 5, lane = tid & 31;
+    const int g = lane >> 2, q = lane & 3;
+    const int ti = warp >> 1, tj = warp & 1;
+    double* Ar = s.A[0];
+    double* Ai = s.A[0] + kLPlane;
+
+    for (;;) {
+        if (tid == 0) s_task = *(volatile unsigned*)abort_word ? ntask : (int)atomicAdd(counter, 1u);
+        __syncthreads();
+        const int task = s_task;
+        if (task >= ntask) return;
+        const int grp = task / (kCholGroup * per_sys);
+        const int sys0 = grp * kCholGroup, gs = min(kCholGroup, a.nsys - sys0);
+        int rem = task - grp * kCholGroup * per_sys;
+        const int k = rem / (gs * nblk);
+        rem -= k * gs * nblk;
+        const int npanel = nblk - k - 1;
+        int kind, row, sys;
+        if (rem < gs) { kind = 0; row = k; sys = sys0 + rem; }
+        else if ((rem -= gs) < gs * npanel) { kind = 1; row = k + 1 + rem / gs; sys = sys0 + rem % gs; }
+        else { rem -= gs * npanel; kind = 2; row = rem / gs; sys = sys0 + rem % gs; }
+
+        const double* Gp = a.Gp + (size_t)sys * tri * kBlkDoubles;
+        double* Lp = a.Lp + (size_t)sys * tri * kLBlkDoubles;
+        double* Linvp = a.Linvp + (size_t)sys * nblk * kLBlkDoubles;
+        double* Wp = Wp_all + (size_t)sys * tri * kLBlkDoubles;
+        const double* lam = a.lam + (size_t)sys * Np;
+        double* Wp1 = (ex.Wp1 && ex.lam) ? ex.Wp1 + (size_t)sys * tri * kLBlkDoubles : nullptr;
+        double* Wf1 = ex.Wf1 ? ex.Wf1 + (size_t)sys * wf : nullptr;
+        double* Wf2 = ex.Wf2 ? ex.Wf2 + (size_t)sys * wf : nullptr;
+        int* info = a.info ? a.info + sys : nullptr;
+        unsigned* flags = a.sync + 2 + (size_t)sys * 2 * tri;
+        unsigned* done;
+        double P3m[3][2][2][2];
+        warp_zero3m<2, 2>(P3m);
+
+        if (kind == 2) {
+            const int jp = row;
+            if (!chol_accumulate<2>(P3m, s, Lp, Wp, Linvp + (size_t)k * kLBlkDoubles, flags, tri, k, jp, k, jp, k, abort_word, info)) {
+                cp_async_wait<0>();
+                return;
+            }
+            const double* V = s.B[(k - jp) & 1];
+            double cr[2][2][2], ci[2][2][2];
+            warp_zgemm3m_finish<2, 2, false, false>(P3m, cr, ci);
+#pragma unroll
+            for (int i = 0; i < 2; ++i)
+#pragma unroll
+                for (int j = 0; j < 2; ++j)
+#pragma unroll
+                    for (int e = 0; e < 2; ++e) {
+                        const int r = 16 * ti + 8 * i + g, c = 16 * tj + 8 * j + 2 * q + e;
+                        Ar[r * kLdBlk + c] = -cr[i][j][e];
+                        Ai[r * kLdBlk + c] = -ci[i][j][e];
+                    }
+            __syncthreads();
+            double dr[2][2][2], di[2][2][2], Q3m[3][2][2][2];
+            warp_zero3m<2, 2>(Q3m);
+            warp_zgemm3m<2, 2, false, false, false, false>(Q3m, V + 16 * ti * kLdBlk, V + kLPlane + 16 * ti * kLdBlk, kLdBlk,
+                                                           Ar + 16 * tj, Ai + 16 * tj, kLdBlk, 16 * (ti + 1));
+            warp_zgemm3m_finish<2, 2, false, false>(Q3m, dr, di);
+            const double* lamj = ex.lam ? ex.lam + (size_t)sys * Np + 32 * jp : nullptr;
+            double* Wb = Wp + blk_index(k, jp) * kLBlkDoubles;
+            double* Wb1 = Wp1 ? Wp1 + blk_index(k, jp) * kLBlkDoubles : nullptr;
+#pragma unroll
+            for (int i = 0; i < 2; ++i)
+#pragma unroll
+                for (int j = 0; j < 2; ++j) {
+                    const int r = 16 * ti + 8 * i + g, c = 16 * tj + 8 * j + 2 * q;
+                    *reinterpret_cast<double2*>(Wb + r * kLdBlk + c) = make_double2(dr[i][j][0], dr[i][j][1]);
+                    *reinterpret_cast<double2*>(Wb + kLPlane + r * kLdBlk + c) = make_double2(di[i][j][0], di[i][j][1]);
+                    if (Wb1) {
+                        const double l0 = lamj[c], l1 = lamj[c + 1];
+                        *reinterpret_cast<double2*>(Wb1 + r * kLdBlk + c) = make_double2(l0 * dr[i][j][0], l1 * dr[i][j][1]);
+                        *reinterpret_cast<double2*>(Wb1 + kLPlane + r * kLdBlk + c) = make_double2(l0 * di[i][j][0], l1 * di[i][j][1]);
+                    }
+#pragma unroll
+                    for (int e = 0; e < 2; ++e) {
+                        const int R = 32 * k + r, C = 32 * jp + c + e;
+                        if (Wf1) {
+                            const double l = lamj ? lamj[c + e] : 1.0;
+                            store_frag1(Wf1, R, C, l * dr[i][j][e], l * di[i][j][e]);
+                        }
+                        if (Wf2) store_frag2(Wf2, nblk, R, C, dr[i][j][e], di[i][j][e]);
+                    }
+                }
+            done = flags + tri + blk_index(k, jp);
+        } else {
+            const int i = row;
+            const bool diag = kind == 0;
+            double mr_[2][2][2], mi_[2][2][2];
+            {
+                const double* Gb = Gp + blk_index(i, k) * kBlkDoubles;
+#pragma unroll
+                for (int ii = 0; ii < 2; ++ii)
+#pragma unroll
+                    for (int j = 0; j < 2; ++j)
+#pragma unroll
+                        for (int e = 0; e < 2; ++e) {
+                            const int r = 16 * ti + 8 * ii + g, c = 16 * tj + 8 * j + 2 * q + e;
+                            const int gi = 32 * i + r, gj = 32 * k + c;
+                            const double sc = lam[gi] * lam[gj];
+                            mr_[ii][j][e] = sc * Gb[r * 32 + c];
+                            mi_[ii][j][e] = sc * Gb[1024 + r * 32 + c];
+                            if (gi == gj && (gi < a.n || gi >= a.N)) mr_[ii][j][e] += 1.0;
+                        }
+            }
+            const bool ok = diag ? chol_accumulate<0>(P3m, s, Lp, Wp, nullptr, flags, tri, k, 0, 0, 0, k, abort_word, info)
+                                 : chol_accumulate<1>(P3m, s, Lp, Wp, Linvp + (size_t)k * kLBlkDoubles, flags, tri, i, k, k, 0, k,
+                                                      abort_word, info);
+            if (!ok) {
+                cp_async_wait<0>();
+                return;
+            }
+            double cr[2][2][2], ci[2][2][2];
+            warp_zgemm3m_finish<2, 2, false, true>(P3m, cr, ci);
+#pragma unroll
+            for (int ii = 0; ii < 2; ++ii)
+#pragma unroll
+                for (int j = 0; j < 2; ++j)
+#pragma unroll
+                    for (int e = 0; e < 2; ++e) {
+                        const int r = 16 * ti + 8 * ii + g, c = 16 * tj + 8 * j + 2 * q + e;
+                        Ar[r * kLdBlk + c] = mr_[ii][j][e] - cr[ii][j][e];
+                        Ai[r * kLdBlk + c] = mi_[ii][j][e] - ci[ii][j][e];
+                    }
+            __syncthreads();
+            if (diag) {
+                double* Vr = s.B[0];
+                double* Vi = s.B[0] + kLPlane;
+                const bool bad = diag_chol_inverse_block<kTaskCT>(Ar, Ai, Vr, Vi, tid);
+                __syncthreads();
+                double* Lb = Lp + blk_index(k, k) * kLBlkDoubles;
+                double* Vb = Linvp + (size_t)k * kLBlkDoubles;
+                double* Wb = Wp + blk_index(k, k) * kLBlkDoubles;
+                const double* lamk = ex.lam ? ex.lam + (size_t)sys * Np + 32 * k : nullptr;
+                for (int e = tid; e < kLBlkDoubles; e += kTaskCT) {
+                    const double v = Vr[e];
+                    Lb[e] = Ar[e];
+                    Vb[e] = v;
+                    Wb[e] = v;
+                }
+                __syncthreads();
+                if (tid == 0) {
+                    __threadfence();
+                    st_release(flags + blk_index(k, k), 1u);
+                }
+                if (Wp1)
+                    for (int e = tid; e < kLBlkDoubles; e += kTaskCT) {
+                        const int c = (e % kLPlane) % kLdBlk;
+                        Wp1[blk_index(k, k) * kLBlkDoubles + e] = c < 32 ? Vr[e] * lamk[c] : 0.0;
+                    }
+                if (Wf1 || Wf2) {
+                    for (int e = tid; e < 1024; e += kTaskCT) {
+                        const int r = e >> 5, c = e & 31;
+                        const double re = Vr[r * kLdBlk + c], im = Vi[r * kLdBlk + c];
+                        if (Wf1 && c < 16 * ((r >> 4) + 1)) {
+                            const double l = lamk ? lamk[c] : 1.0;
+                            store_frag1(Wf1, 32 * k + r, 32 * k + c, l * re, l * im);
+                        }
+                        if (Wf2 && r >= 16 * (c >> 4)) store_frag2(Wf2, nblk, 32 * k + r, 32 * k + c, re, im);
+                    }
+                }
+                if (bad && tid == 0 && info) atomicMax(info, k + 1);
+            } else {
+                const double* V = s.B[k & 1];
+                double dr[2][2][2], di[2][2][2], Q3m[3][2][2][2];
+                warp_zero3m<2, 2>(Q3m);
+                warp_zgemm3m<2, 2, false, false, true, true>(Q3m, Ar + 16 * ti * kLdBlk, Ai + 16 * ti * kLdBlk, kLdBlk,
+                                                             V + 16 * tj * kLdBlk, V + kLPlane + 16 * tj * kLdBlk, kLdBlk, 32);
+                warp_zgemm3m_finish<2, 2, false, true>(Q3m, dr, di);
+                double* Lb = Lp + blk_index(i, k) * kLBlkDoubles;
+#pragma unroll
+                for (int ii = 0; ii < 2; ++ii)
+#pragma unroll
+                    for (int j = 0; j < 2; ++j) {
+                        const int r = 16 * ti + 8 * ii + g, c = 16 * tj + 8 * j + 2 * q;
+                        *reinterpret_cast<double2*>(Lb + r * kLdBlk + c) = make_double2(dr[ii][j][0], dr[ii][j][1]);
+                        *reinterpret_cast<double2*>(Lb + kLPlane + r * kLdBlk + c) = make_double2(di[ii][j][0], di[ii][j][1]);
+                    }
+            }
+            done = diag ? nullptr : flags + blk_index(i, k);
+        }
+        __syncthreads();
+        if (tid == 0 && done) {
+            __threadfence();
+            st_release(done, 1u);
+        }
+    }
+}
+
 constexpr int kCT = 512;
 
 __device__ __forceinline__ void load_block_async_ct(double* s, const double* g) {
     for (int c = threadIdx.x; c < kLBlkDoubles / 2; c += kCT) cp_async16(s + 2 * c, g + 2 * c);
 }
 
+struct CholColArgs {
+    const double* Gp; const double* lam; double* Lp; double* Linvp; int* info;
+    int nblk, n, N, nsys;
+};
 struct CholWSmem {
     double A[2][kLBlkDoubles];
     double B[2][kLBlkDoubles];
     double V[kLBlkDoubles];
 };
-__device__ __forceinline__ void store_frag1(double* Wf1, int R, int C, double re, double im) {
-    const int s = R >> 4, t = C >> 2;
-    double* d = Wf1 + ((size_t)(2 * s * (s + 1) + t) * 128 + 64 * ((R >> 3) & 1) + (4 * (R & 7) + (C & 3)) * 2);
-    *reinterpret_cast<double2*>(d) = make_double2(re, im);
-}
-__device__ __forceinline__ void store_frag2(double* Wf2, int nblk, int R, int C, double re, double im) {
-    const int s = C >> 4, t = R >> 2;
-    double* d = Wf2 + ((size_t)(8 * nblk * s - 2 * s * (s - 1) + t - 4 * s) * 128 + 64 * ((C >> 3) & 1) + (4 * (C & 7) + (R & 3)) * 2);
-    *reinterpret_cast<double2*>(d) = make_double2(re, im);
-}
-
-__global__ void __launch_bounds__(kCT, 2) k_chol_w(CholArgs a, TrinvExtra ex, double* Wp_all, int k, int first) {
+__global__ void __launch_bounds__(kCT, 2) k_chol_w(CholColArgs a, TrinvExtra ex, double* Wp_all, int k, int first) {
     extern __shared__ __align__(16) unsigned char smem_raw[];
     CholWSmem& s = *reinterpret_cast<CholWSmem*>(smem_raw);
     const int sys = blockIdx.x;
@@ -201,7 +488,7 @@
         }
         __syncthreads();
         if (diag) {
-            const bool bad = diag_chol_inverse_block(Ar, Ai, Vr, Vi, tid, kCT);
+            const bool bad = diag_chol_inverse_block<kCT>(Ar, Ai, Vr, Vi, tid);
             __syncthreads();
             double* Lb = Lp + blk_index(kc, kc) * kLBlkDoubles;
             double* Vb = Linvp + (size_t)kc * kLBlkDoubles;
@@ -249,17 +536,31 @@
     }
 }
 
+
+constexpr int kCholTaskMaxSys = 4;
 int launch_chol_trinv(const CholArgs& a, double* Wp, const TrinvExtra& ex, cudaStream_t st) {
-    static bool attr_dev[kMaxDev] = {false};
-    bool& attr_set = attr_dev[current_device_slot()];
-    if (!attr_set) {
+    static int ctas_dev[kMaxDev] = {0};
+    int& ctas = ctas_dev[current_device_slot()];
+    if (!ctas) {
+        cudaFuncSetAttribute(k_chol_tasks, cudaFuncAttributeMaxDynamicSharedMemorySize, (int)sizeof(CholTaskSmem));
         cudaFuncSetAttribute(k_chol_w, cudaFuncAttributeMaxDynamicSharedMemorySize, (int)sizeof(CholWSmem));
-        attr_set = true;
+        int per_sm = 0, nsm = 0, dev = 0;
+        cudaGetDevice(&dev);
+        cudaDeviceGetAttribute(&nsm, cudaDevAttrMultiProcessorCount, dev);
+        cudaOccupancyMaxActiveBlocksPerMultiprocessor(&per_sm, k_chol_tasks, kTaskCT, sizeof(CholTaskSmem));
+        ctas = per_sm * nsm > 0 ? per_sm * nsm : 1;
     }
     if (a.info) cudaMemsetAsync(a.info, 0, sizeof(int) * a.nsys, st);
-    k_chol_w<<<dim3(a.nsys, 1), kCT, sizeof(CholWSmem), st>>>(a, ex, Wp, 0, 1);
+    if (a.nsys <= kCholTaskMaxSys) {
+        cudaMemsetAsync(a.sync, 0, sizeof(unsigned) * chol_sync_words(a.nblk, a.nsys), st);
+        const int ntask = a.nsys * a.nblk * a.nblk;
+        k_chol_tasks<<<ntask < ctas ? ntask : ctas, kTaskCT, sizeof(CholTaskSmem), st>>>(a, ex, Wp);
+        return 1;
+    }
+    const CholColArgs ca{a.Gp, a.lam, a.Lp, a.Linvp, a.info, a.nblk, a.n, a.N, a.nsys};
+    k_chol_w<<<dim3(a.nsys, 1), kCT, sizeof(CholWSmem), st>>>(ca, ex, Wp, 0, 1);
     if (a.nblk == 1) return 1;
-    for (int k = 0; k < a.nblk; ++k) k_chol_w<<<dim3(a.nsys, a.nblk - 1), kCT, sizeof(CholWSmem), st>>>(a, ex, Wp, k, 0);
+    for (int k = 0; k < a.nblk; ++k) k_chol_w<<<dim3(a.nsys, a.nblk - 1), kCT, sizeof(CholWSmem), st>>>(ca, ex, Wp, k, 0);
     return a.nblk + 1;
 }
 
diff --git a/hydra_pspec_b200/csrc/hp_kernels.cuh b/hydra_pspec_b200/csrc/hp_kernels.cuh
--- a/hydra_pspec_b200/csrc/hp_kernels.cuh
+++ b/hydra_pspec_b200/csrc/hp_kernels.cuh
@@ -47,9 +47,20 @@
     double* Lp;
     double* Linvp;
     int* info;
+    unsigned* sync;
     int nblk, n, N, nsys;
 };
+constexpr int kCholTimeout = 1 << 30;
+__host__ __device__ inline size_t chol_sync_words(int nblk, int nsys) { return 2 + (size_t)nsys * 2 * tri_blocks(nblk); }
 struct TrinvExtra { double* Wp1; double* Wf1; double* Wf2; const double* lam; };
+__host__ __device__ inline size_t frag1_offset(int R, int C) {
+    const int s = R >> 4, t = C >> 2;
+    return (size_t)(2 * s * (s + 1) + t) * 128 + 64 * ((R >> 3) & 1) + (4 * (R & 7) + (C & 3)) * 2;
+}
+__host__ __device__ inline size_t frag2_offset(int nblk, int R, int C) {
+    const int s = C >> 4, t = R >> 2;
+    return (size_t)(8 * nblk * s - 2 * s * (s - 1) + t - 4 * s) * 128 + 64 * ((C >> 3) & 1) + (4 * (C & 7) + (R & 3)) * 2;
+}
 int launch_chol_trinv(const CholArgs& a, double* Wp, const TrinvExtra& ex, cudaStream_t st);
 
 struct SolveArgs {
diff --git a/hydra_pspec_b200/csrc/hp_pertime.cu b/hydra_pspec_b200/csrc/hp_pertime.cu
--- a/hydra_pspec_b200/csrc/hp_pertime.cu
+++ b/hydra_pspec_b200/csrc/hp_pertime.cu
@@ -191,7 +191,7 @@
                 __syncthreads();
                 PT_T(2);
                 if (i == k) {
-                    if (diag_chol_inverse_block(Ar, Ai, Vr, Vi, tid, kPT)) bad = k + 1;
+                    if (diag_chol_inverse_block<kPT>(Ar, Ai, Vr, Vi, tid)) bad = k + 1;
                     __syncthreads();
                     PT_T(3);
                     for (int o = 8; o > 0; o >>= 1) {
diff --git a/hydra_pspec_b200/csrc/hp_testhooks.cu b/hydra_pspec_b200/csrc/hp_testhooks.cu
--- a/hydra_pspec_b200/csrc/hp_testhooks.cu
+++ b/hydra_pspec_b200/csrc/hp_testhooks.cu
@@ -30,6 +30,8 @@
     const int N = n + m, nblk = (N + 31) / 32, Np = nblk * 32, ntiles = (T + 15) / 16, Tp = ntiles * 16;
     double *dG, *dGp, *dlam, *dLp, *dLinv, *dWp, *dR, *dW = nullptr, *dX, *dS, *dP;
     int* dinfo;
+    unsigned* dsync;
+    cudaMalloc(&dsync, sizeof(unsigned) * hp::chol_sync_words(nblk, 1));
     size_t tri = hp::tri_blocks(nblk) * hp::kLBlkDoubles, trig = hp::tri_blocks(nblk) * hp::kBlkDoubles;
     cudaMalloc(&dG, 16ull * N * N); cudaMalloc(&dGp, 8 * trig); cudaMalloc(&dlam, 8ull * Np); cudaMalloc(&dLp, 8 * tri);
     cudaMalloc(&dLinv, 8ull * nblk * hp::kLBlkDoubles); cudaMalloc(&dWp, 8 * tri); cudaMalloc(&dR, 16ull * Tp * Np); cudaMalloc(&dX, 16ull * Tp * Np);
@@ -44,7 +46,7 @@
     }
     hp::launch_pack_lower(dG, N, 0, dGp, N, nblk, 1, 0);
     hp::CholArgs ca{};
-    ca.Gp = dGp; ca.lam = dlam; ca.Lp = dLp; ca.Linvp = dLinv; ca.info = dinfo; ca.nblk = nblk; ca.n = n; ca.N = N; ca.nsys = 1;
+    ca.Gp = dGp; ca.lam = dlam; ca.Lp = dLp; ca.Linvp = dLinv; ca.info = dinfo; ca.sync = dsync; ca.nblk = nblk; ca.n = n; ca.N = N; ca.nsys = 1;
     hp::launch_chol_trinv(ca, dWp, hp::TrinvExtra{nullptr, nullptr, nullptr, nullptr}, 0);
     hp::SolveArgs sa{};
     sa.Wp = dWp; sa.lam = dlam; sa.Rfix = dR; sa.wa = dW; sa.X = dX; sa.Ssc = dS; sa.Ppart = dP;
@@ -69,10 +71,61 @@
         }
     }
     cudaFree(dG); cudaFree(dGp); cudaFree(dlam); cudaFree(dLp); cudaFree(dLinv); cudaFree(dWp); cudaFree(dR); cudaFree(dW); cudaFree(dX);
-    cudaFree(dS); cudaFree(dP); cudaFree(dinfo);
-    return e == cudaSuccess ? HP_OK : HP_ERR_CUDA;
-}
-
+    cudaFree(dS); cudaFree(dP); cudaFree(dinfo); cudaFree(dsync);
+    return e == cudaSuccess ? HP_OK : HP_ERR_CUDA;
+}
+
+int hp_test_chol_batch(int n, int N, int nsys, const double* G, const double* lam, double* L, double* W, double* W1, double* W2,
+                       int* info) {
+    const int nblk = (N + 31) / 32, Np = nblk * 32;
+    const size_t tri = hp::tri_blocks(nblk) * hp::kLBlkDoubles, trig = hp::tri_blocks(nblk) * hp::kBlkDoubles;
+    const size_t wf = hp::solve3_frag_doubles(nblk), NN = (size_t)N * N;
+    double *dG, *dGp, *dlam, *dLp, *dLinv, *dWp, *dWp1, *dWf1, *dWf2;
+    int* dinfo;
+    unsigned* dsync;
+    if (cudaMalloc(&dG, 16 * NN * nsys) || cudaMalloc(&dGp, 8 * trig * nsys) || cudaMalloc(&dlam, 8ull * Np * nsys) ||
+        cudaMalloc(&dLp, 8 * tri * nsys) || cudaMalloc(&dLinv, 8ull * nblk * hp::kLBlkDoubles * nsys) || cudaMalloc(&dWp, 8 * tri * nsys) ||
+        cudaMalloc(&dWp1, 8 * tri * nsys) || cudaMalloc(&dWf1, 8 * wf * nsys) || cudaMalloc(&dWf2, 8 * wf * nsys) ||
+        cudaMalloc(&dinfo, 4ull * nsys) || cudaMalloc(&dsync, sizeof(unsigned) * hp::chol_sync_words(nblk, nsys)))
+        return HP_ERR_CUDA;
+    cudaMemset(dlam, 0, 8ull * Np * nsys);
+    cudaMemset(dWf1, 0xff, 8 * wf * nsys); cudaMemset(dWf2, 0xff, 8 * wf * nsys);
+    cudaMemcpy(dG, G, 16 * NN * nsys, cudaMemcpyHostToDevice);
+    cudaMemcpy2D(dlam, 8ull * Np, lam, 8ull * N, 8ull * N, nsys, cudaMemcpyHostToDevice);
+    hp::launch_pack_lower(dG, N, NN, dGp, N, nblk, nsys, 0);
+    hp::CholArgs ca{};
+    ca.Gp = dGp; ca.lam = dlam; ca.Lp = dLp; ca.Linvp = dLinv; ca.info = dinfo; ca.sync = dsync;
+    ca.nblk = nblk; ca.n = n; ca.N = N; ca.nsys = nsys;
+    hp::launch_chol_trinv(ca, dWp, hp::TrinvExtra{dWp1, dWf1, dWf2, dlam}, 0);
+    cudaError_t e = cudaDeviceSynchronize();
+    if (e == cudaSuccess) {
+        std::vector<double> lp(tri * nsys), wp(tri * nsys), f1(wf * nsys), f2(wf * nsys);
+        cudaMemcpy(lp.data(), dLp, 8 * lp.size(), cudaMemcpyDeviceToHost);
+        cudaMemcpy(wp.data(), dWp, 8 * wp.size(), cudaMemcpyDeviceToHost);
+        cudaMemcpy(f1.data(), dWf1, 8 * f1.size(), cudaMemcpyDeviceToHost);
+        cudaMemcpy(f2.data(), dWf2, 8 * f2.size(), cudaMemcpyDeviceToHost);
+        cudaMemcpy(info, dinfo, 4ull * nsys, cudaMemcpyDeviceToHost);
+        for (int s = 0; s < nsys; ++s)
+            for (int i = 0; i < N; ++i)
+                for (int j = 0; j < N; ++j) {
+                    const size_t o = 2 * (s * NN + (size_t)i * N + j);
+                    double v[8] = {0, 0, 0, 0, 0, 0, 0, 0};
+                    if (j <= i) {
+                        const size_t b = s * tri + hp::blk_index(i / 32, j / 32) * hp::kLBlkDoubles + (i % 32) * hp::kLdBlk + (j % 32);
+                        v[0] = lp[b]; v[1] = lp[b + hp::kLPlane];
+                        v[2] = wp[b]; v[3] = wp[b + hp::kLPlane];
+                        const double* p1 = f1.data() + s * wf + hp::frag1_offset(i, j);
+                        const double* p2 = f2.data() + s * wf + hp::frag2_offset(nblk, i, j);
+                        v[4] = p1[0]; v[5] = p1[1]; v[6] = p2[0]; v[7] = p2[1];
+                    }
+                    L[o] = v[0]; L[o + 1] = v[1]; W[o] = v[2]; W[o + 1] = v[3];
+                    W1[o] = v[4]; W1[o + 1] = v[5]; W2[o] = v[6]; W2[o + 1] = v[7];
+                }
+    }
+    cudaFree(dG); cudaFree(dGp); cudaFree(dlam); cudaFree(dLp); cudaFree(dLinv); cudaFree(dWp); cudaFree(dWp1); cudaFree(dWf1);
+    cudaFree(dWf2); cudaFree(dinfo); cudaFree(dsync);
+    return e == cudaSuccess ? HP_OK : HP_ERR_CUDA;
+}
 
 int hp_test_solve2(int n, int m, int T, int nsys, const double* G, const double* lam, const double* Rfix, const double* wa,
                    int cg_compat, int grid_limit, int variant, double* X, double* psum) {
@@ -86,6 +139,8 @@
     double *dWf1 = nullptr, *dWf2 = nullptr;
     double *dG, *dGp, *dlam, *dLp, *dLinv, *dWp, *dWp1, *dR, *dW = nullptr, *dX, *dP, *dRt;
     int* dinfo;
+    unsigned* dsync;
+    cudaMalloc(&dsync, sizeof(unsigned) * hp::chol_sync_words(nblk, 1));
     const size_t tri = hp::tri_blocks(nblk) * hp::kLBlkDoubles, trig = hp::tri_blocks(nblk) * hp::kBlkDoubles;
     const size_t rt_doubles = (size_t)nsys * ntiles * nblk * 2 * 32 * hp::kTT;
     cudaMalloc(&dG, 16ull * N * N); cudaMalloc(&dGp, 8 * trig); cudaMalloc(&dlam, 8ull * Np); cudaMalloc(&dLp, 8 * tri);
@@ -104,7 +159,7 @@
     }
     hp::launch_pack_lower(dG, N, 0, dGp, N, nblk, 1, 0);
     hp::CholArgs ca{};
-    ca.Gp = dGp; ca.lam = dlam; ca.Lp = dLp; ca.Linvp = dLinv; ca.info = dinfo; ca.nblk = nblk; ca.n = n; ca.N = N; ca.nsys = 1;
+    ca.Gp = dGp; ca.lam = dlam; ca.Lp = dLp; ca.Linvp = dLinv; ca.info = dinfo; ca.sync = dsync; ca.nblk = nblk; ca.n = n; ca.N = N; ca.nsys = 1;
     if (variant == 3) {
         cudaMalloc(&dWf1, 8 * wf * nsys); cudaMalloc(&dWf2, 8 * wf * nsys);
         cudaMemset(dWf1, 0xff, 8 * wf * nsys); cudaMemset(dWf2, 0xff, 8 * wf * nsys);
@@ -161,6 +216,7 @@
     }
     cudaFree(dG); cudaFree(dGp); cudaFree(dlam); cudaFree(dLp); cudaFree(dLinv); cudaFree(dWp); cudaFree(dWp1); cudaFree(dR);
     cudaFree(dW); cudaFree(dX); cudaFree(dP); cudaFree(dinfo); cudaFree(dRt); cudaFree(dWall); cudaFree(dW1all); cudaFree(dWf1); cudaFree(dWf2);
+    cudaFree(dsync);
     return e == cudaSuccess ? HP_OK : HP_ERR_CUDA;
 }
 
diff --git a/include/hydra_pspec_b200.h b/include/hydra_pspec_b200.h
--- a/include/hydra_pspec_b200.h
+++ b/include/hydra_pspec_b200.h
@@ -106,6 +106,9 @@
 int hp_test_solve2(int n, int m, int T, int nsys, const double* G, const double* lam, const double* Rfix, const double* wa,
                    int cg_compat, int grid_limit, int variant, double* X, double* psum);
 
+int hp_test_chol_batch(int n, int N, int nsys, const double* G, const double* lam, double* L, double* W, double* W1, double* W2,
+                       int* info);
+
 int hp_test_solve3_schedule(int nblk, unsigned char* n, unsigned char* strips, int* nwarps, int* max_per_warp);
 
 double hp_fp64_peak_tflops(int device, double seconds);
```

After: 16680, median of 6. No clear change (+0.0%).
